# Dzh-16/FLASH-Viterbi

Hardware: AMD Instinct MI355X
Metric: trellis_cells_per_sec (higher is better)
Workload: dtype f32 scores (+f64 add per cell, rounded to f32 as the reference does)

## Files before the change

flash_viterbi_amd/csrc/fv_context.hip:

```cpp
#include "fv_internal.h"
#include "flashvit_testing.h"

namespace {

template <typename F>
void parallel_rows(int rows, F &&fn)
{
    unsigned hw = std::thread::hardware_concurrency();
    int nt = (int)std::min<unsigned>(hw ? hw : 4, 16);
    if (rows < 256) nt = 1;
    if (nt <= 1) { fn(0, rows); return; }
    std::vector<std::thread> th;
    int per = (rows + nt - 1) / nt;
    for (int t = 0; t < nt; ++t) {
        int a = t * per, b = std::min(rows, a + per);
        if (a >= b) break;
        th.emplace_back([=, &fn] { fn(a, b); });
    }
    for (auto &x : th) x.join();
}

}

namespace fvi {

size_t device_bytes(const fv_ctx *c)
{
    size_t sum = 0;
    c->each_buffer([&](const auto &b) { sum += b.bytes(); });
    return sum;
}

inline size_t pack_head(int nscores) { return 2 * FV_NCOUNTERS + (size_t)std::max(4, round_up(nscores, 4)); }

static size_t pack_ints(const fv_ctx *ctx, int T, int nscores) { return pack_head(nscores) + (size_t)T * std::max(1, ctx->nranks) + (size_t)T; }

int grant(fv_ctx *ctx, const Wants &w, bool check)
{
    if (check) {
        unsigned long long grow = 0, released = 0;
        for (const Wants::Want &x : w.list)
            if (x.n > x.have) { grow += (unsigned long long)x.n * x.elem; released += (unsigned long long)x.have * x.elem; }
        if (grow) {
            size_t free_b = 0, total_b = 0;
            FV_HIP(hipMemGetInfo(&free_b, &total_b));
            if (grow > (unsigned long long)free_b + released) {
                ctx->detail = w.what + ": " + std::to_string(grow) + " bytes needed (" + w.dominant + "), " +
                              std::to_string((unsigned long long)free_b + released) + " bytes of device memory free";
                return FV_ERR_NOMEM;
            }
        }
    }
    for (const Wants::Want &x : w.list) FV_HIP(x.ensure(x.buf, x.n));
    return 0;
}

int ensure_workspace(fv_ctx *ctx, int T, size_t rows_needed, int nscores, Wants w)
{
    const size_t want_rows = rows_needed * 2 * (size_t)ctx->nrows;
    const size_t want_pack = pack_ints(ctx, T, nscores);
    const bool rows_grow = want_rows > ctx->d_rows.n;
    w.add(ctx->d_ob, (size_t)T); w.add(ctx->d_ans, (size_t)T); w.add(ctx->d_bp, (size_t)T * ctx->K);
    w.add(ctx->d_rows, want_rows); w.add(ctx->d_pack, want_pack);
    if (nscores > 1 && w.what.empty()) { w.what = "batch workspace"; w.dominant = "arg rows " + std::to_string(4ull * T * ctx->K); }
    if (int rc = grant(ctx, w, nscores > 1)) return rc;
    if (rows_grow) FV_HIP(hipMemsetAsync(ctx->d_rows.p, 0, want_rows * sizeof(float), ctx->stream));
    FV_HIP(ctx->d_score.ensure((size_t)std::max(4, nscores)));
    FV_HIP(ctx->d_counters.ensure(FV_NCOUNTERS));
    if (ctx->comm || ctx->group) FV_HIP(ctx->d_gather.ensure((size_t)T * ctx->nranks));
    if (want_pack > ctx->h_pin_n) {
        if (ctx->h_pin) { (void)hipHostFree(ctx->h_pin); ctx->h_pin = nullptr; ctx->h_pin_n = 0; }
        FV_HIP(hipHostMalloc(reinterpret_cast<void **>(&ctx->h_pin), want_pack * sizeof(int), hipHostMallocDefault));
        ctx->h_pin_n = want_pack;
    }
    return 0;
}

int ensure_flat_workspace(fv_ctx *ctx, int T, size_t passes, long long arg_rows, int chain_len)
{
    Wants w;
    const size_t want_rows = passes * 2 * (size_t)ctx->nrows;
    const bool rows_grow = want_rows > ctx->d_rows.n;
    w.add(ctx->d_rows, want_rows); w.add(ctx->d_snap, (size_t)T); w.add(ctx->d_flat_bp, (size_t)std::max(arg_rows, 1ll) * ctx->K);
    w.add(ctx->d_chain, (size_t)std::max(chain_len, 1)); w.add(ctx->d_flat, std::max(passes, (size_t)1));
    w.what = "flat generations workspace"; w.dominant = "private arg rows " + std::to_string(4ull * (unsigned long long)arg_rows * ctx->K);
    if (int rc = grant(ctx, w, true)) return rc;
    if (rows_grow) FV_HIP(hipMemsetAsync(ctx->d_rows.p, 0, want_rows * sizeof(float), ctx->stream));
    return 0;
}

__global__ void pack_result(const unsigned long long *counters, const float *score, int nscore, size_t head, const int *ans,
                            size_t nans, int *out)
{
    const size_t tid = (size_t)blockIdx.x * blockDim.x + threadIdx.x, nthr = (size_t)gridDim.x * blockDim.x;
    if (tid < 2 * FV_NCOUNTERS) out[tid] = reinterpret_cast<const int *>(counters)[tid];
    for (size_t i = tid; i < (size_t)nscore; i += nthr) out[2 * FV_NCOUNTERS + i] = __float_as_int(score[i]);
    for (size_t i = tid; i < nans; i += nthr) out[head + i] = ans[i];
}

__global__ void clear_outputs(unsigned long long *counters, int *ans, int T)
{
    const int tid = blockIdx.x * blockDim.x + threadIdx.x;
    if (tid < FV_NCOUNTERS) counters[tid] = 0ull;
    for (int i = tid; i < T; i += gridDim.x * blockDim.x) ans[i] = 0;
}

int emission_view(fv_ctx *ctx, const int *&ob, long long T)
{
    if (ob) {
        ctx->view.lb32 = ctx->LB32T.p; ctx->view.lb64 = ctx->LB64T.p; ctx->view.nsym = ctx->M;
        ctx->view.logs_nonpositive = ctx->logs_nonpositive;
        return 0;
    }
    if (ctx->emis_rows == 0) { ctx->detail = "ob == NULL: no emission scores are staged (fv_set_emissions)"; return FV_ERR_ARG; }
    if (T < 1 || T > ctx->emis_rows) {
        ctx->detail = "ob == NULL: " + std::to_string(T) + " times asked for, " + std::to_string(ctx->emis_rows) + " rows of emission scores staged";
        return FV_ERR_ARG;
    }
    try {
        for (size_t j = ctx->h_iota.size(); j < (size_t)T; ++j) ctx->h_iota.push_back((int)j);
    } catch (const std::bad_alloc &) { return FV_ERR_NOMEM; }
    ob = ctx->h_iota.data();
    ctx->view.lb32 = ctx->E32.p; ctx->view.lb64 = ctx->E64.p; ctx->view.nsym = (int)ctx->emis_rows;
    ctx->view.logs_nonpositive = ctx->logs_nonpositive && !ctx->emis_positive;
    return 0;
}

int begin_decode(fv_ctx *ctx, const int *ob, int T)
{
    ctx->h_ob.assign(ob, ob + T);
    int *stage = ctx->h_pin + (ctx->h_pin_n - (size_t)T);
    std::memcpy(stage, ob, (size_t)T * sizeof(int));
    FV_HIP(hipMemcpyAsync(ctx->d_ob.p, stage, (size_t)T * sizeof(int), hipMemcpyHostToDevice, ctx->stream));
    hipLaunchKernelGGL(clear_outputs, dim3(16), dim3(256), 0, ctx->stream, ctx->d_counters.p, ctx->d_ans.p, T);
    FV_HIP(hipGetLastError());
    return 0;
}

int batch_lengths(fv_ctx *ctx, const char *who, const int *&ob, const long long *offsets, int nseq, int n_split, int mode,
                  const int *path_out, std::vector<int> &lengths)
{
    if (!offsets || !path_out || nseq < 1 || n_split < 1) return FV_ERR_ARG;
    if (mode != FV_MODE_REFERENCE && mode != FV_MODE_SINGLE_PASS) return FV_ERR_ARG;
    const std::string w = who;
    if (offsets[0] != 0) { ctx->detail = w + ": offsets[0] must be 0"; return FV_ERR_ARG; }
    lengths.resize((size_t)nseq);
    for (int s = 0; s < nseq; ++s) {
        const long long len = offsets[s + 1] - offsets[s];
        if (len < 0) { ctx->detail = w + ": offsets decrease at sequence " + std::to_string(s); return FV_ERR_ARG; }
        if (len < 2) { ctx->detail = w + ": sequence " + std::to_string(s) + " has fewer than 2 observations"; return FV_ERR_ARG; }
        if (offsets[s + 1] > 0x7fffffffLL) { ctx->detail = w + ": more than 2^31 - 1 observations in all (at sequence " + std::to_string(s) + ")"; return FV_ERR_ARG; }
        lengths[(size_t)s] = (int)len;
    }
    if (int rc = emission_view(ctx, ob, offsets[nseq])) return rc;
    return ctx->K == 0 ? FV_ERR_STATE : 0;
}

int batch_symbols(fv_ctx *ctx, const char *who, const int *ob, const long long *offsets, int nseq)
{
    for (int s = 0; s < nseq; ++s)
        for (long long j = offsets[s]; j < offsets[s + 1]; ++j)
            if (ob[j] < 0 || ob[j] >= ctx->view.nsym) {
                ctx->detail = std::string(who) + ": sequence " + std::to_string(s) + " holds a symbol outside [0, M) at position " + std::to_string(j - offsets[s]);
                return FV_ERR_ARG;
            }
    return 0;
}

int batch_plan(fv_ctx *ctx, const char *who, const std::vector<int> &lengths, int n_split, int mode, fv::Plan &plan)
{
    int bad = -1;
    const int rc = fv::build_forest(lengths.data(), (int)lengths.size(), n_split, mode, plan, &bad);
    if (rc)
        ctx->detail = std::string(who) + ": sequence " + std::to_string(bad) + " of length " + std::to_string(lengths[(size_t)std::max(bad, 0)]) +
                      " has no plan for n_split = " + std::to_string(n_split) + " (T == 2 * n_split with n_split > 2)";
    return rc;
}

std::vector<std::vector<fv::Pass>> deal_passes(const fv_ctx *ctx, const fv::Plan &plan, size_t *most)
{
    std::vector<std::vector<fv::Pass>> gens(plan.generations());
    for (const fv::Pass &p : plan.passes)
        if (p.owner < 0 || p.owner % ctx->nranks == ctx->rank) gens[p.generation].push_back(p);
    if (most) {
        *most = 1;
        for (const auto &g : gens) *most = std::max(*most, g.size());
    }
    return gens;
}

static int read_stats(fv_ctx *ctx, const unsigned long long *counters, clk::time_point t0, size_t nprof)
{
    fv_stats &st = ctx->stats;
    st.decode_ms = ms_since(t0);
    float ms = 0.f;
    FV_HIP(hipEventElapsedTime(&ms, ctx->ev_start, ctx->ev_stop)); st.gpu_ms = ms;
    FV_HIP(hipEventElapsedTime(&ms, ctx->ev_start, ctx->ev_top)); st.top_pass_ms = ms;
    FV_HIP(hipEventElapsedTime(&ms, ctx->ev_s0, ctx->ev_s1)); st.top_steps_ms = ms;
    st.step_kernel_ms = 0;
    for (size_t i = 0; i + 1 < nprof; i += 2) {
        FV_HIP(hipEventElapsedTime(&ms, ctx->prof_events[i], ctx->prof_events[i + 1]));
        st.step_kernel_ms += ms;
    }
    st.refine_near = (long long)counters[0];
    st.refine_rescan = (long long)counters[1];
    st.beam_exact_sets = (long long)counters[2];
    st.beam_dup_cols = (long long)counters[3];
    st.beam_dup_steps = (long long)counters[4];
    st.beam_ties = (long long)counters[6];
    st.beam_cand_selects = (long long)counters[7];
    st.refine_saturated = (long long)counters[8];
    st.beam_spec_steps = (long long)counters[9];
    st.beam_reach_events = (long long)counters[10];
    st.beam_list_short = (long long)counters[11];
    st.beam_list_long = (long long)counters[12];
    st.beam_list_entries = (long long)counters[13];
    st.beam_chain_cuts = (long long)counters[14];
    if (counters[fvk::FLAT_COUNTER]) {
        st.flat_first_miss = (int)(counters[fvk::FLAT_COUNTER] >> 32);
        st.flat_missed = (int)(counters[fvk::FLAT_COUNTER] & 0xffffffffull);
    }
    if (counters[5]) { ctx->detail = "heap replay: producer/consumer hand-shake timed out"; return FV_ERR_DEVICE; }
    st.device_bytes = (long long)fvi::device_bytes(ctx);
    st.ranks = ctx->nranks;
    return 0;
}

int finish_decode(fv_ctx *ctx, const fv::Plan &plan, const long long *offsets, int nseq, int *path_out, float *score_out,
                  int *status_out, clk::time_point t0, size_t nprof, bool beam)
{
    const int T = (int)offsets[nseq];
    const bool gathered = (ctx->comm || ctx->group) && !plan.seg_L.empty();
    if (gathered)
        if (int rc = gather_answers(ctx, T)) return rc;
    FV_HIP(hipEventRecord(ctx->ev_stop, ctx->stream));
    const size_t nans = gathered ? (size_t)T * ctx->nranks : (size_t)T, head = pack_head(nseq), total = head + nans;
    hipLaunchKernelGGL(pack_result, dim3(64), dim3(256), 0, ctx->stream, ctx->d_counters.p, ctx->d_score.p, nseq, head,
                       gathered ? ctx->d_gather.p : ctx->d_ans.p, nans, ctx->d_pack.p);
    FV_HIP(hipGetLastError());
    FV_HIP(hipMemcpyAsync(ctx->h_pin, ctx->d_pack.p, total * sizeof(int), hipMemcpyDeviceToHost, ctx->stream));
    FV_HIP(hipStreamSynchronize(ctx->stream));
    for (hipGraphExec_t ge : ctx->graphs) (void)hipGraphExecDestroy(ge);
    ctx->graphs.clear();
    unsigned long long counters[FV_NCOUNTERS];
    std::memcpy(counters, ctx->h_pin, sizeof counters);
    if (gathered) {
        const std::vector<int> host(ctx->h_pin + head, ctx->h_pin + head + nans);
        merge_gathered(plan, host, T, ctx->nranks, path_out);
    } else {
        std::memcpy(path_out, ctx->h_pin + head, nans * sizeof(int));
    }
    if (score_out) std::memcpy(score_out, ctx->h_pin + 2 * FV_NCOUNTERS, (size_t)nseq * sizeof(float));
    if (int rc = read_stats(ctx, counters, t0, nprof)) return rc;
    int worst = FV_OK, warn = FV_OK;
    for (int s = 0; s < nseq; ++s) {
        bool neg = false;
        for (long long j = offsets[s]; j < offsets[s + 1]; ++j) neg |= path_out[j] < 0;
        const int st = !neg ? FV_OK : beam ? FV_WARN_BEAM_MISS : FV_ERR_NO_PRED;
        if (status_out) status_out[s] = st;
        worst = std::min(worst, st);
        warn = std::max(warn, st);
    }
    return worst < 0 ? worst : warn;
}

int drained(fv_ctx *ctx, int rc)
{
    if (rc >= 0) return rc;
    hipStreamCaptureStatus cs = hipStreamCaptureStatusNone;
    if (hipStreamIsCapturing(ctx->stream, &cs) == hipSuccess && cs != hipStreamCaptureStatusNone) {
        hipGraph_t g = nullptr;
        (void)hipStreamEndCapture(ctx->stream, &g);
        if (g) (void)hipGraphDestroy(g);
    }
    (void)hipStreamSynchronize(ctx->stream);
    for (hipStream_t a : ctx->aux) if (a) (void)hipStreamSynchronize(a);
    for (hipGraphExec_t ge : ctx->graphs) (void)hipGraphExecDestroy(ge);
    ctx->graphs.clear();
    (void)hipGetLastError();
    return rc;
}

}



extern "C" int fv_create(fv_ctx **out, int device)
{
    if (!out) return FV_ERR_ARG;
    *out = nullptr;
    int ndev = 0;
    if (hipGetDeviceCount(&ndev) != hipSuccess || device < 0 || device >= ndev) return FV_ERR_DEVICE;
    fv_ctx *ctx = new (std::nothrow) fv_ctx();
    if (!ctx) return FV_ERR_NOMEM;
    ctx->device = device;
    auto fail = [&](int rc) { fv_destroy(ctx); return rc; };
    if (hipSetDevice(device) != hipSuccess) return fail(FV_ERR_DEVICE);
    if (hipStreamCreateWithFlags(&ctx->stream, hipStreamNonBlocking) != hipSuccess) return fail(FV_ERR_DEVICE);
    for (int q = 0; q < fv_ctx::BEAM_AUX; ++q)
        if (hipStreamCreateWithFlags(&ctx->aux[q], hipStreamNonBlocking) != hipSuccess ||
            hipEventCreateWithFlags(&ctx->ev_join[q], hipEventDisableTiming) != hipSuccess) return fail(FV_ERR_DEVICE);
    if (hipEventCreateWithFlags(&ctx->ev_fork, hipEventDisableTiming) != hipSuccess) return fail(FV_ERR_DEVICE);
    {
        int cus = 0;
        if (hipDeviceGetAttribute(&cus, hipDeviceAttributeMultiprocessorCount, ctx->device) == hipSuccess && cus > 0) ctx->num_cus = cus;
    }
    if (hipEventCreate(&ctx->ev_start) != hipSuccess || hipEventCreate(&ctx->ev_stop) != hipSuccess ||
        hipEventCreate(&ctx->ev_top) != hipSuccess || hipEventCreate(&ctx->ev_s0) != hipSuccess ||
        hipEventCreate(&ctx->ev_s1) != hipSuccess)
        return fail(FV_ERR_DEVICE);
    int rc = 0;
    if ((rc = fvi::full_setup(ctx)) || (rc = fvi::beam_setup(ctx))) return fail(rc);
    *out = ctx;
    return FV_OK;
}

extern "C" void fv_destroy(fv_ctx *ctx)
{
    if (!ctx) return;
    if (ctx->group) {
        fv_group *g = ctx->group;
        if (ctx->group_rank != 0) return;
        for (fv_ctx *m : g->members) m->group = nullptr;
        for (size_t r = g->members.size(); r-- > 1;) fv_destroy(g->members[r]);
        for (hipEvent_t e : g->ans_ready) if (e) (void)hipEventDestroy(e);
        delete g;
    }
    (void)hipSetDevice(ctx->device);
    if (ctx->stream) (void)hipStreamSynchronize(ctx->stream);
    if (ctx->comm) ncclCommDestroy(ctx->comm);
    if (ctx->h_pin) { (void)hipHostFree(ctx->h_pin); ctx->h_pin = nullptr; ctx->h_pin_n = 0; }
    for (hipEvent_t e : ctx->prof_events) (void)hipEventDestroy(e);
    if (ctx->ev_start) (void)hipEventDestroy(ctx->ev_start);
    if (ctx->ev_stop) (void)hipEventDestroy(ctx->ev_stop);
    if (ctx->ev_top) (void)hipEventDestroy(ctx->ev_top);
    if (ctx->ev_s0) (void)hipEventDestroy(ctx->ev_s0);
    if (ctx->ev_s1) (void)hipEventDestroy(ctx->ev_s1);
    if (ctx->ev_fork) (void)hipEventDestroy(ctx->ev_fork);
    for (int q = 0; q < fv_ctx::BEAM_AUX; ++q) {
        if (ctx->ev_join[q]) (void)hipEventDestroy(ctx->ev_join[q]);
        if (ctx->aux[q]) (void)hipStreamDestroy(ctx->aux[q]);
    }
    if (ctx->stream) (void)hipStreamDestroy(ctx->stream);
    delete ctx;
}

namespace fvi {

static void log_emissions(const float *B, const float *Pi, int K, int M, HostTables &h, bool &ok_range, bool &any_big)
{
    h.b64.assign((size_t)M * K, 0.0); h.pi64.assign(K, 0.0);
    h.b32.assign((size_t)M * K, 0.0f);
    for (int i = 0; i < K; ++i) {
        for (int o = 0; o < M; ++o) {
            const float x = B[(size_t)i * M + o];
            if (!(x >= 0.0f) || std::isinf(x)) ok_range = false;
            if (x > 1.0f) any_big = true;
            const double l = std::log((double)x);
            h.b64[(size_t)o * K + i] = l; h.b32[(size_t)o * K + i] = (float)l;
        }
        const float x = Pi[i];
        if (!(x >= 0.0f) || std::isinf(x)) ok_range = false;
        if (x > 1.0f) any_big = true;
        h.pi64[i] = std::log((double)x);
    }
}

int build_host_tables(const float *A, const float *B, const float *Pi, int K, int M, HostTables &h, std::string &detail)
{
    h.K = K; h.M = M;
    const int nrows = h.nrows = round_up(K, fvk::ROW_ALIGN);
    const int ntiles = h.ntiles = (K + fvk::TILE_W - 1) / fvk::TILE_W;
    const bool full_ok = h.full_ok = fvk::step_lds_bytes<1>(nrows) <= 160 * 1024;
    h.u16_ok = fvk::u16_lds_bytes<1, 8>(nrows) <= 160 * 1024 && K <= 65536;

    const size_t tab = h.tab = (size_t)ntiles * nrows * fvk::TILE_W;
    std::vector<double> &h64 = h.h64;
    std::vector<float> &h32 = h.h32;
    std::vector<unsigned short> &h16 = h.h16;
    try {
        h64.assign(tab, -HUGE_VAL);
        if (full_ok) { h32.assign(tab, -HUGE_VALF); h16.assign(tab, 0xFC00u ); }
    } catch (...) { return FV_ERR_NOMEM; }
    std::vector<double> dmax_row(K, 0.0);
    bool ok_range = true;
    std::vector<char> bad(K, 0), big(K, 0);
    parallel_rows(K, [&](int a, int b) {
        for (int k = a; k < b; ++k) {
            const float *src = A + (size_t)k * K;
            for (int i = 0; i < K; ++i) {
                const float x = src[i];
                if (!(x >= 0.0f) || std::isinf(x)) bad[k] = 1;
                if (x > 1.0f) big[k] = 1;
                const double l = std::log((double)x);
// ... 411 lines not shown
                      "FV_EMIS_LOG_F32, _F64, _F16 or _BF16";
        return FV_ERR_ARG;
    }
    auto t0 = clk::now();
    hipPointerAttribute_t at{};
    bool on_device = false;
    if (hipPointerGetAttributes(&at, scores) == hipSuccess) on_device = at.type == hipMemoryTypeDevice;
    else (void)hipGetLastError();
    for (int r = 0; r < n; ++r) {
        fv_ctx *m = fvi::group_member(ctx, r);
        const bool in_place = on_device && n == 1 && at.device == m->device;
        const int rc = fvi::drained(m, fvi::stage_emissions_on(m, scores, dtype, T, ld, in_place));
        if (rc) {
            if (m != ctx) ctx->detail = m->detail;
            for (int q = 0; q < n; ++q) fvi::group_member(ctx, q)->emis_rows = 0;
            ctx->stats.device_bytes = (long long)fvi::device_bytes(ctx);
            return rc;
        }
    }
    ctx->stats.set_emissions_ms = ms_since(t0);
    ctx->stats.emission_rows = T;
    ctx->stats.device_bytes = (long long)fvi::device_bytes(ctx);
    return FV_OK;
}

extern "C" int fv_set_emission_map(fv_ctx *ctx, const int *pdf_of_state, int P)
{
    if (!ctx) return FV_ERR_ARG;
    if (ctx->K == 0) { ctx->detail = "fv_set_emission_map: no model (the map holds one entry per state of the model)"; return FV_ERR_STATE; }
    if (!pdf_of_state && P != 0) { ctx->detail = "fv_set_emission_map: pdf_of_state == NULL clears the map and takes P == 0"; return FV_ERR_ARG; }
    if (pdf_of_state) {
        if (P < 1) { ctx->detail = "fv_set_emission_map: P >= 1 score classes with a map"; return FV_ERR_ARG; }
        hipPointerAttribute_t at{};
        if (hipPointerGetAttributes(&at, pdf_of_state) != hipSuccess) (void)hipGetLastError();
        else if (at.type == hipMemoryTypeDevice) {
            ctx->detail = "fv_set_emission_map: pdf_of_state is a device pointer; the map is read on the host";
            return FV_ERR_ARG;
        }
        for (int i = 0; i < ctx->K; ++i)
            if (pdf_of_state[i] < 0 || pdf_of_state[i] >= P) {
                ctx->detail = "fv_set_emission_map: pdf_of_state[" + std::to_string(i) + "] = " + std::to_string(pdf_of_state[i]) +
                              " (state " + std::to_string(i) + ") lies outside [0, P = " + std::to_string(P) + ")";
                return FV_ERR_ARG;
            }
    }
    const int n = fvi::group_size(ctx);
    auto unset = [&] {
        for (int r = 0; r < n; ++r) {
            fv_ctx *m = fvi::group_member(ctx, r);
            m->emis_rows = 0; m->emis_positive = false; m->emis_P = 0;
        }
        ctx->stats.emission_rows = 0;
        ctx->stats.set_emissions_ms = 0.0;
    };
    unset();
    int rc = FV_OK;
    for (int r = 0; r < n && rc == FV_OK; ++r) {
        fv_ctx *m = fvi::group_member(ctx, r);
        rc = [&]() -> int {
            fv_ctx *ctx = m;
            FV_HIP(hipSetDevice(ctx->device));
            if (!pdf_of_state) { ctx->EMap.release(); return FV_OK; }
            FV_HIP(ctx->EMap.ensure((size_t)ctx->K));
            FV_HIP(hipMemcpy(ctx->EMap.p, pdf_of_state, (size_t)ctx->K * sizeof(int), hipMemcpyHostToDevice));
            ctx->emis_P = P;
            return FV_OK;
        }();
        if (rc && m != ctx) ctx->detail = m->detail;
    }
    if (rc) unset();
    ctx->stats.device_bytes = (long long)fvi::device_bytes(ctx);
    return rc;
}

extern "C" int fv_clear_emissions(fv_ctx *ctx)
{
    if (!ctx) return FV_ERR_ARG;
    const int n = fvi::group_size(ctx);
    for (int r = 0; r < n; ++r) {
        fv_ctx *m = fvi::group_member(ctx, r);
        (void)hipSetDevice(m->device);
        m->emis_rows = 0; m->emis_positive = false;
        m->E32.release(); m->E64.release();
    }
    ctx->stats.emission_rows = 0;
    ctx->stats.device_bytes = (long long)fvi::device_bytes(ctx);
    return FV_OK;
}

extern "C" int fv_test_device_alloc(fv_ctx *ctx, size_t bytes, const void *host_src, void **out)
{
    if (!ctx || !out || bytes == 0) return FV_ERR_ARG;
    *out = nullptr;
    FV_HIP(hipSetDevice(ctx->device));
    void *p = nullptr;
    FV_HIP(hipMalloc(&p, bytes));
    if (host_src) {
        hipError_t e = hipMemcpy(p, host_src, bytes, hipMemcpyHostToDevice);
        if (e != hipSuccess) { (void)hipFree(p); FV_HIP(e); }
    }
    *out = p;
    return FV_OK;
}

extern "C" int fv_test_device_free(fv_ctx *ctx, void *p)
{
    if (!ctx) return FV_ERR_ARG;
    FV_HIP(hipSetDevice(ctx->device));
    if (p) FV_HIP(hipFree(p));
    return FV_OK;
}

extern "C" int fv_test_stage_emissions_ms(fv_ctx *ctx, const void *dev_scores, int dtype, int T, long long ld, int reps, float *ms_out)
{
    if (!ctx || !ms_out || !dev_scores || T < 1 || reps < 1 || ctx->K == 0 || ld < (ctx->emis_P ? ctx->emis_P : ctx->K) ||
        ld > (1ll << 59) / T || !fvi::emis_dtype_ok(dtype) || ctx->group)
        return FV_ERR_ARG;
    hipPointerAttribute_t at{};
    if (hipPointerGetAttributes(&at, dev_scores) != hipSuccess) { (void)hipGetLastError(); return FV_ERR_ARG; }
    if (at.type != hipMemoryTypeDevice || at.device != ctx->device) return FV_ERR_ARG;
    FV_HIP(hipSetDevice(ctx->device));
    ctx->emis_rows = 0; ctx->emis_positive = false;
    ctx->stats.emission_rows = 0;
    const size_t cells = (size_t)T * (size_t)ctx->K;
    FV_HIP(ctx->E32.ensure(cells));
    FV_HIP(ctx->E64.ensure(cells));
    FV_HIP(ctx->d_emflags.ensure(2));
    FV_HIP(hipMemsetAsync(ctx->d_emflags.p, 0, sizeof(unsigned long long), ctx->stream));
    FV_HIP(hipMemsetAsync(ctx->d_emflags.p + 1, 0xFF, sizeof(unsigned long long), ctx->stream));
    hipEvent_t e0 = nullptr, e1 = nullptr;
    struct Ev { hipEvent_t &a, &b; ~Ev() { if (a) (void)hipEventDestroy(a); if (b) (void)hipEventDestroy(b); } } ev{ e0, e1 };
    FV_HIP(hipEventCreate(&e0));
    FV_HIP(hipEventCreate(&e1));
    if (int rc = fvi::launch_stage_emissions(ctx, dev_scores, dtype, ld, T, ctx->EMap.p, ctx->emis_P)) return fvi::drained(ctx, rc);
    FV_HIP(hipEventRecord(e0, ctx->stream));
    for (int r = 0; r < reps; ++r)
        if (int rc = fvi::launch_stage_emissions(ctx, dev_scores, dtype, ld, T, ctx->EMap.p, ctx->emis_P)) return fvi::drained(ctx, rc);
    FV_HIP(hipEventRecord(e1, ctx->stream));
    FV_HIP(hipStreamSynchronize(ctx->stream));
    float ms = 0.0f;
    FV_HIP(hipEventElapsedTime(&ms, e0, e1));
    *ms_out = ms / (float)reps;
    ctx->stats.device_bytes = (long long)fvi::device_bytes(ctx);
    return FV_OK;
}

extern "C" int fv_test_flat_poison(fv_ctx *ctx, int t)
{
    if (!ctx || t < -1) return FV_ERR_ARG;
    ctx->flat_poison = t;
    return FV_OK;
}

extern "C" int fv_set_option(fv_ctx *ctx, int key, long long value)
{
    if (!ctx) return FV_ERR_ARG;
    if (ctx->group && ctx->group_rank == 0) {
        for (int r = fvi::group_size(ctx) - 1; r >= 1; --r) {
            const int rc = fv_set_option(fvi::group_member(ctx, r), key, value);
            if (rc) return rc;
        }
    }
    switch (key) {
    case FV_OPT_KERNEL:
        if ((value < FV_KERNEL_AUTO || value > FV_KERNEL_U16_REFINE) && value != FV_KERNEL_CSR_F64) return FV_ERR_ARG;
        ctx->opt_kernel = (int)value; return FV_OK;
    case FV_OPT_MAX_BATCH:
        if (value < 1 || value > fvk::MAX_BATCH) return FV_ERR_ARG;
        ctx->opt_max_batch = (int)value; return FV_OK;
    case FV_OPT_PROFILE:
        ctx->opt_profile = value ? 1 : 0; return FV_OK;
    case FV_OPT_FLAT_GENERATIONS:
        if (value < 0 || value > 2) return FV_ERR_ARG;
        ctx->opt_flat = (int)value; return FV_OK;
    case FV_OPT_ROW_CODES:
        if (value < 0 || value > 4) return FV_ERR_ARG;
        ctx->opt_row_codes = (int)value; return FV_OK;
    case FV_OPT_SEL_MARGIN:
        if (value < 0 || value > 100000) return FV_ERR_ARG;
        ctx->opt_sel_margin = (float)value * 1e-3f; return FV_OK;
    case FV_OPT_SPARSE_BEAM:
        if (value != 0 && value != 1) return FV_ERR_ARG;
        ctx->opt_sparse_beam = (int)value; return FV_OK;
    case FV_OPT_DEBUG:
#ifndef FV_TIMING_BUILD
        if (value & FV_DEBUG_TIMING_ONLY) { ctx->detail = "FV_OPT_DEBUG: result-changing timing switches need the timing build"; return FV_ERR_ARG; }
#endif
        if (value < 0 || value >= (1ll << 32) || (value & ((1ll << 27) | (1ll << 30)))) return FV_ERR_ARG;
        ctx->opt_csr_mem = (int)((value >> 31) & 1);
        ctx->opt_debug = (int)(value & 0x3fffffff); return FV_OK;
    default: return FV_ERR_ARG;
    }
}

extern "C" long long fv_checkpoint_memory_bytes(int K, int T, int step)
{
    if (step <= 0) step = (int)std::floor(std::sqrt(1.0 * T));
    const long long nck = (T + step - 1) / step;
    const long long last = T - (nck - 1) * step;
    const long long tsub = nck > 1 && step + 1 > last ? step + 1 : last;
    return 4LL * K + 4LL * K * nck + 4LL * K + 4LL * (T / step + 1) + 8LL * K * tsub;
}

extern "C" int fv_last_stats(const fv_ctx *ctx, fv_stats *out)
{
    if (!ctx || !out) return FV_ERR_ARG;
    *out = ctx->stats;
    return FV_OK;
}

extern "C" const char *fv_last_error_detail(const fv_ctx *ctx) { return ctx ? ctx->detail.c_str() : ""; }

extern "C" const char *fv_strerror(int rc)
{
    switch (rc) {
    case FV_OK: return "ok";
    case FV_WARN_BEAM_MISS: return "beam miss: path holds -1 entries, as the reference prints";
    case FV_ERR_ARG: return "bad argument";
    case FV_ERR_NOMEM: return "out of memory";
    case FV_ERR_NO_PRED: return "decoded entry has no finite predecessor";
    case FV_ERR_DEVICE: return "HIP error";
    case FV_ERR_STATE: return "call out of order (no model / no communicator)";
    case FV_ERR_UNSUPPORTED: return "size or option not supported by this build";
    case FV_ERR_COMM: return "RCCL error";
    default: return "unknown flashvit error";
    }
}

extern "C" long long fv_reference_memory_bytes(int K, int T, int n_split, int beam_width)
{
    const long long N = n_split;
    const long long pool = ((40 + 48 + 8 * N + 12 + 7) / 8) * 8;
    long long mem = 0, tmp;
    const bool nway = N > 2 && T >= 2 * N;
    if (beam_width <= 0) {
        if (nway) mem = 4 * (N - 1) + 2LL * K * 4 + 2 * (N - 1) * (long long)K * 4;
        tmp = N * (2LL * K * 4 + 2LL * K * 4);
    } else {
        if (nway) mem = 4 * (N - 1) + 2 * (N - 1) * (long long)(beam_width + 1) * 12;
        tmp = N * (2LL * (beam_width + 1) * 12);
    }
    if (tmp > mem) mem = tmp;
    return mem + pool + 8;
}
```

flash_viterbi_amd/csrc/fv_full.hip:

```cpp
#include "fv_internal.h"
#include "fv_kernels.hip.inc"
#include "flashvit_testing.h"

namespace {

int pick_kernel(const fv_ctx *ctx)
{
    if (ctx->opt_kernel == FV_KERNEL_F64_STREAM) return FV_KERNEL_F64_STREAM;
    if (!ctx->view.logs_nonpositive) return FV_KERNEL_F64_STREAM;
    if (ctx->opt_kernel == FV_KERNEL_F16_REFINE || ctx->opt_kernel == FV_KERNEL_F32_REFINE ||
        ctx->opt_kernel == FV_KERNEL_Q16_REFINE || ctx->opt_kernel == FV_KERNEL_U16_REFINE)
        return ctx->opt_kernel;
    if (ctx->opt_kernel == FV_KERNEL_SPARSE_Q16) return ctx->SPdata.p ? FV_KERNEL_SPARSE_Q16 : FV_KERNEL_U16_REFINE;
    return (ctx->SPdata.p && ctx->density <= 0.35) ? FV_KERNEL_SPARSE_Q16 : FV_KERNEL_U16_REFINE;
}

constexpr int U_UP = 16, U_DB32 = 4, U_DB64 = 2, U_DB16 = 2;

constexpr int nb_slot(int NB) { return NB == 1 ? 0 : NB == 2 ? 1 : NB == 4 ? 2 : 3; }
template <typename TA> constexpr int tab_slot()
{
    return std::is_same<TA, double>::value ? 0 : std::is_same<TA, float>::value ? 1 : std::is_same<TA, fvk::half_t>::value ? 2 : 3;
}
template <typename TA, int NB, bool DB> constexpr unsigned long long step_variant()
// ... 202 lines not shown
    if (ctx->test_record) ctx->test_variants |= u16_variant<NB, DB, NWV>() | ((b.codes & 1) ? FV_TV_ROW_CODES : 0ull);
    hipLaunchKernelGGL((fvk::trellis_step_u16<NB, U, DB, NWV>), dim3(a.tiles_per_xcd * 8), dim3(NWV * 64), lds, ctx->lstream ? ctx->lstream : ctx->stream, b);
    FV_HIP(hipGetLastError());
    return 0;
}

template <int NB>
int launch_u16_nb(fv_ctx *ctx, const fvk::TaskSlot *slots, int nb, int reverse)
{
    fvk::StepArgs<NB> a;
    a.LA = ctx->LAQ16.p; a.window = ctx->windowq; a.qscale = ctx->qscale; a.vanilla = 0;
    a.LA64 = ctx->LA64.p; a.counters = ctx->d_counters.p;
    a.K = ctx->K; a.reverse = (ctx->opt_debug & 2) ? 0 : reverse; a.debug = ctx->opt_debug;
    a.nrows = ctx->nrows;
    a.ntiles = (ctx->K + fvk::TILE_W - 1) / fvk::TILE_W;
    a.tiles_per_xcd = (a.ntiles + 7) / 8;
    a.nb = nb;
    a.row_lo = 0; a.srows = ctx->nrows; a.merge = 0;
    a.codes = ctx->launch_codes;
    const fvk::CodeSlot *cs = static_cast<const fvk::CodeSlot *>(ctx->launch_code_slots);
    for (int t = 0; t < NB; ++t) { a.t[t] = slots[t < nb ? t : 0]; a.c[t] = cs[t < nb ? t : 0]; }
    const int nq = ctx->nrows / 32;
    if (ctx->opt_debug & 8192) {
        if (a.ntiles <= ctx->num_cus && (nq + 15) / 16 <= 8 && !(ctx->opt_debug & 4)) return launch_u16_variant<NB, 8, false, 16>(ctx, a);
        return launch_u16_variant<NB, U_DB16, true, 16>(ctx, a);
    }
    if (a.ntiles <= ctx->num_cus && (nq + 7) / 8 <= 16 && !(ctx->opt_debug & 4) && !ctx->forked_batches) return launch_u16_variant<NB, 16, false, 8>(ctx, a);
    return launch_u16_variant<NB, U_DB16, true, 8>(ctx, a);
}

int launch_u16(fv_ctx *ctx, const fvk::TaskSlot *slots, int nb, int reverse)
{
    if (nb <= 1) return launch_u16_nb<1>(ctx, slots, nb, reverse);
    if (nb <= 2) return launch_u16_nb<2>(ctx, slots, nb, reverse);
    if (nb <= 4) return launch_u16_nb<4>(ctx, slots, nb, reverse);
    return launch_u16_nb<8>(ctx, slots, nb, reverse);
}

constexpr int ROW_CODES_AUTO_MIN_K = 2048;
constexpr int ROW_CODES_AUTO_FAMILIES = 2;

int coded_row_index(const fv_ctx *ctx, const float *row)
{
    if (!row || row < ctx->d_rows.p || row >= ctx->d_rows.p + ctx->d_rows.n) return -1;
    const size_t off = (size_t)(row - ctx->d_rows.p);
    if (off % (size_t)ctx->nrows) return -1;
    const size_t r = off / (size_t)ctx->nrows;
    return r < ctx->row_coded.size() ? (int)r : -1;
}

int ensure_row_codes(fv_ctx *ctx, size_t pairs)
{
    if (!ctx->row_codes) { ctx->row_coded.clear(); return 0; }
    const size_t rows = pairs * 2, want = rows * (size_t)ctx->nrows;
    if (want > ctx->d_rcodes.n || want / fvk::TILE_W > ctx->d_rtmax.n) {
        if (ctx->d_rcodes.ensure(want) != hipSuccess || ctx->d_rtmax.ensure(want / fvk::TILE_W) != hipSuccess) {
            (void)hipGetLastError();
            ctx->d_rcodes.release(); ctx->d_rtmax.release();
            ctx->row_codes = 0; ctx->row_coded.clear();
            return 0;
        }
        FV_HIP(hipMemsetAsync(ctx->d_rcodes.p, 0xff, ctx->d_rcodes.bytes(), ctx->stream));
        FV_HIP(hipMemsetAsync(ctx->d_rtmax.p, 0xff, ctx->d_rtmax.bytes(), ctx->stream));
    }
    ctx->row_coded.assign(ctx->d_rcodes.n / (size_t)ctx->nrows, 0);
    return 0;
}

bool init_rows_coded(fv_ctx *ctx, int base, int n)
{
    if (!ctx->row_codes || ctx->csr || (size_t)(base + n) * 2 > ctx->row_coded.size()) return false;
    for (int q = 0; q < n; ++q) ctx->row_coded[(size_t)(base + q) * 2] = 1;
    return true;
}

int launch_step_kernel(fv_ctx *ctx, int kernel, const fvk::TaskSlot *slots, int nb, int reverse)
{
    fvk::CodeSlot cs[fvk::MAX_BATCH];
    const bool packed = kernel == FV_KERNEL_U16_REFINE && (nb <= 1 || !ctx->full_ok || (ctx->opt_debug & 16384) || ctx->forked_batches);
    bool all_in = packed && ctx->row_codes != 0, all_out = all_in;
    int rout[fvk::MAX_BATCH];
    for (int q = 0; q < nb; ++q) {
        const int rin = coded_row_index(ctx, slots[q].t1_in);
        rout[q] = coded_row_index(ctx, slots[q].t1_out);
        const size_t ntp = (size_t)ctx->nrows / fvk::TILE_W;
        cs[q].c_in = rin >= 0 ? ctx->d_rcodes.p + (size_t)rin * ctx->nrows : nullptr;
        cs[q].tmax_in = rin >= 0 ? ctx->d_rtmax.p + (size_t)rin * ntp : nullptr;
        cs[q].c_out = rout[q] >= 0 ? ctx->d_rcodes.p + (size_t)rout[q] * ctx->nrows : nullptr;
        cs[q].tmax_out = rout[q] >= 0 ? ctx->d_rtmax.p + (size_t)rout[q] * ntp : nullptr;
        all_in = all_in && rin >= 0 && ctx->row_coded[(size_t)rin];
        all_out = all_out && rout[q] >= 0;
    }
    const int family = nb <= 1 ? 1 : 2;
    const bool produce = all_out && (nb > 1 || (ctx->row_codes & 1));
    ctx->launch_codes = ((all_in && (ctx->row_codes & family)) ? 1 : 0) | (produce ? 2 : 0);
    ctx->launch_code_slots = cs;
    for (int q = 0; q < nb; ++q)
        if (rout[q] >= 0) ctx->row_coded[(size_t)rout[q]] = produce ? 1 : 0;
    switch (kernel) {
    case FV_KERNEL_U16_REFINE:
        if (nb <= 1 || !ctx->full_ok || (ctx->opt_debug & 16384) || ctx->forked_batches) return launch_u16(ctx, slots, nb, reverse);
        return launch_step<fvk::q16_t>(ctx, slots, nb, reverse);
    case FV_KERNEL_SPARSE_Q16: return launch_sparse(ctx, slots, nb);
    case FV_KERNEL_SPARSE_CSR: return launch_csr(ctx, slots, nb);
    case FV_KERNEL_CSR_F64: return launch_csr_f64(ctx, slots, nb);
    case FV_KERNEL_F64_STREAM: return launch_step<double>(ctx, slots, nb, reverse);
    case FV_KERNEL_F32_REFINE: return launch_step<float>(ctx, slots, nb, reverse);
    case FV_KERNEL_Q16_REFINE: return launch_step<fvk::q16_t>(ctx, slots, nb, reverse);
    default: return launch_step<fvk::half_t>(ctx, slots, nb, reverse);
    }
}

template <typename K>
int set_big_lds(fv_ctx *ctx, K kernel)
{
    FV_HIP(hipFuncSetAttribute(reinterpret_cast<const void *>(kernel), hipFuncAttributeMaxDynamicSharedMemorySize, 160 * 1024));
    return 0;
}

template <typename TA, int NB>
int allow_big_lds(fv_ctx *ctx)
{
    int rc = 0;
    if constexpr (std::is_same<TA, double>::value) {
        rc = set_big_lds(ctx, &fvk::trellis_step<TA, NB, U_DB64, true>);
    } else {
        constexpr int U = std::is_same<TA, float>::value ? U_DB32 : U_DB16;
        rc = set_big_lds(ctx, &fvk::trellis_step<TA, NB, U, true>);
        if constexpr (NB <= 2) { if (!rc) rc = set_big_lds(ctx, &fvk::trellis_step<TA, NB, U_UP, false>); }
    }
    return rc;
}

int max_batch_for(int nrows, bool u16_only)
{
    if (u16_only) {
        if (fvk::u16_lds_bytes<8, 8>(nrows) <= 160 * 1024) return 8;
        if (fvk::u16_lds_bytes<4, 8>(nrows) <= 160 * 1024) return 4;
        if (fvk::u16_lds_bytes<2, 8>(nrows) <= 160 * 1024) return 2;
        return 1;
    }
    int nb = fvk::MAX_BATCH;
    while (nb > 1) {
        size_t need = nb == 8 ? fvk::step_lds_bytes<8>(nrows) : nb == 4 ? fvk::step_lds_bytes<4>(nrows)
                                                                        : fvk::step_lds_bytes<2>(nrows);
        if (need <= 160 * 1024) break;
        nb >>= 1;
    }
    return nb;
}

struct ProfRange { size_t first, count; };

int prof_event(fv_ctx *ctx, size_t idx, hipEvent_t *out)
{
    while (ctx->prof_events.size() <= idx) {
        hipEvent_t e;
        FV_HIP(hipEventCreate(&e));
        ctx->prof_events.push_back(e);
    }
    *out = ctx->prof_events[idx];
    return 0;
}

enum { BATCH_NONE = 0, BATCH_SERIAL = 1, BATCH_FORK = 2 };
int run_generation_full(fv_ctx *ctx, std::vector<fv::Pass> &passes, int kernel, size_t &nprof, int batch = BATCH_NONE)
{
    const int K = ctx->K;
    const int np = (int)passes.size();
    if (np == 0) return 0;
    std::stable_sort(passes.begin(), passes.end(),
                     [](const fv::Pass &a, const fv::Pass &b) { return a.R - a.L > b.R - b.L; });
    for (int base = 0; base < np; base += fvk::PASS_CHUNK) {
        fvk::PassChunk ch;
        ch.n = std::min(fvk::PASS_CHUNK, np - base);
        for (int q = 0; q < ch.n; ++q) {
            const fv::Pass &p = passes[base + q];
            ch.p[q] = fvk::PassDesc{ p.L, p.R, p.from_pi ? 1 : 0, p.whole ? 1 : 0, (long long)(base + q) * 2 * ctx->nrows };
        }
        if (ctx->csr)
            hipLaunchKernelGGL(fvk::init_rows_csr, dim3((K + 255) / 256, ch.n), dim3(256), 0, ctx->stream, ch, ctx->CRptr.p,
                               ctx->CRcol.p, ctx->CRlog.p, ctx->view.lb64, ctx->LPi64.p, ctx->d_ob.p, ctx->d_ans.p, ctx->d_rows.p, K);
        else {
            const bool coded = init_rows_coded(ctx, base, ch.n);
            hipLaunchKernelGGL(fvk::init_rows, dim3((K + 255) / 256, ch.n), dim3(256), 0, ctx->stream, ch,
                               ctx->LA64.p, ctx->nrows, ctx->view.lb64, ctx->LPi64.p, ctx->d_ob.p, ctx->d_ans.p,
                               ctx->d_rows.p, K, coded ? ctx->d_rcodes.p : nullptr, coded ? ctx->d_rtmax.p : nullptr, -1.0f / ctx->qscale);
        }
        FV_HIP(hipGetLastError());
    }
    const int maxlen = passes[0].R - passes[0].L;
    const bool slabbed = (kernel == FV_KERNEL_F64_STREAM || kernel == FV_KERNEL_Q16_REFINE) && !ctx->full_ok;
    int cap = std::max(1, std::min(ctx->opt_max_batch, slabbed ? 4 : max_batch_for(ctx->nrows, !ctx->full_ok)));
    if (kernel == FV_KERNEL_SPARSE_CSR || kernel == FV_KERNEL_CSR_F64) cap = ctx->opt_max_batch;
    const bool whole_gen = passes[0].whole;
    constexpr int FORK_STREAMS = 3, FORK_CAP = 4;
    const bool two = ((kernel == FV_KERNEL_U16_REFINE && ctx->u16_ok) || ((kernel == FV_KERNEL_SPARSE_Q16 || kernel == FV_KERNEL_SPARSE_CSR || kernel == FV_KERNEL_CSR_F64) && maxlen >= 64)) &&
                     !(ctx->opt_debug & 262144) && (!whole_gen || batch == BATCH_FORK) && np > FORK_CAP &&
                     !ctx->opt_profile && !(ctx->opt_debug & 64);
    const int nbatches = (np + FORK_CAP - 1) / FORK_CAP;
    const int nstreams = two ? std::min(FORK_STREAMS, nbatches) : 1;
    auto fork = [&]() -> int {
        FV_HIP(hipEventRecord(ctx->ev_fork, ctx->stream));
        for (int q = 1; q < nstreams; ++q) FV_HIP(hipStreamWaitEvent(ctx->aux[q - 1], ctx->ev_fork, 0));
        return 0;
    };
    if (two) {
        cap = std::min(cap, FORK_CAP);
        if (!ctx->fork_active) {
            hipError_t qe;
            while ((qe = hipStreamQuery(ctx->stream)) == hipErrorNotReady) std::this_thread::yield();
            FV_HIP(qe);
        }
        ctx->fork_active = true;
        { int rc = fork(); if (rc) return rc; }
    }
    ctx->forked_batches = two;
    struct Unfork { fv_ctx *c; ~Unfork() { c->forked_batches = false; c->lstream = nullptr; } } unfork{ ctx };
    auto join = [&]() -> int {
        for (int q = 1; q < nstreams; ++q) {
            FV_HIP(hipEventRecord(ctx->ev_join[q - 1], ctx->aux[q - 1]));
            FV_HIP(hipStreamWaitEvent(ctx->stream, ctx->ev_join[q - 1], 0));
        }
        return 0;
    };
    const bool col_last = !(ctx->opt_debug & 8);
    const bool use_graph = (ctx->opt_debug & 64) && !ctx->opt_profile;
    if (use_graph) FV_HIP(hipStreamBeginCapture(ctx->stream, hipStreamCaptureModeThreadLocal));
    if (whole_gen && !use_graph) FV_HIP(hipEventRecord(ctx->ev_s0, ctx->stream));
    int active = np;
    for (int s = 1; s <= maxlen; ++s) {
        while (active > 0 && passes[active - 1].R - passes[active - 1].L < s) --active;
        int full = active;
        if (col_last) while (full > 0 && passes[full - 1].R - passes[full - 1].L == s && !passes[full - 1].whole) --full;
        auto row = [&](int q, int parity) { return ctx->d_rows.p + (size_t)q * 2 * ctx->nrows + (size_t)parity * ctx->nrows; };
        for (int base = 0; base < full; base += cap) {
            const int nb = std::min(cap, full - base);
            fvk::TaskSlot slots[fvk::MAX_BATCH];
            for (int q = 0; q < nb; ++q) {
                const fv::Pass &p = passes[base + q];
                slots[q].t1_in = row(base + q, (s - 1) & 1);
                slots[q].t1_out = row(base + q, s & 1);
                slots[q].tmp_row = ctx->view.lb32 + (size_t)ctx->h_ob[p.L + s] * K;
                slots[q].tmp64_row = ctx->view.lb64 + (size_t)ctx->h_ob[p.L + s] * K;
                slots[q].bp_out = ctx->d_bp.p + (size_t)(p.L + s) * K;
            }
            hipEvent_t e0 = nullptr, e1 = nullptr;
            if (ctx->opt_profile) {
                int rc = prof_event(ctx, nprof, &e0); if (rc) return rc;
                rc = prof_event(ctx, nprof + 1, &e1); if (rc) return rc;
                nprof += 2;
                FV_HIP(hipEventRecord(e0, ctx->stream));
            }
            const int other = two ? (base / cap) % nstreams : 0;
            ctx->lstream = other ? ctx->aux[other - 1] : ctx->stream;
            int rc = launch_step_kernel(ctx, kernel, slots, nb, s & 1);
            ctx->lstream = nullptr;
            if (rc) return rc;
            if (ctx->opt_profile) FV_HIP(hipEventRecord(e1, ctx->stream));
            ctx->stats.step_launches += 1;
            ctx->stats.task_steps += nb;
        }
        for (int sid = 0; sid < nstreams; ++sid) {
            fvk::ColArgs c;
            c.LA64 = ctx->LA64.p; c.ans = ctx->d_ans.p; c.K = K; c.nrows = ctx->nrows; c.n = 0;
            hipStream_t cst = sid ? ctx->aux[sid - 1] : ctx->stream;
            auto flush = [&]() -> int {
                if (c.n == 0) return 0;
                if (ctx->csr) {
                    fvk::CsrColArgs cc;
                    cc.ck = ctx->CSk.p; cc.c64 = ctx->CS64.p; cc.tile_off = ctx->CSoff.p; cc.tile_nwb = ctx->CSnwb.p;
                    cc.ans = ctx->d_ans.p; cc.K = K; cc.n = c.n;
                    std::copy(c.p, c.p + c.n, cc.p);
                    hipLaunchKernelGGL(fvk::last_column_csr, dim3(c.n), dim3(256), 0, cst, cc);
                } else
                hipLaunchKernelGGL(fvk::last_column, dim3(c.n), dim3(256), 0, cst, c);
                FV_HIP(hipGetLastError());
                ctx->stats.column_steps += c.n;
                c.n = 0;
                return 0;
            };
            for (int q = full; q < active; ++q) {
                const int owner = (two && s > 1) ? (q / cap) % nstreams : 0;
                if (owner != sid) continue;
                const fv::Pass &p = passes[q];
                c.p[c.n++] = fvk::ColJob{ row(q, (s - 1) & 1), ctx->view.lb32 + (size_t)ctx->h_ob[p.R] * K, ctx->d_bp.p + (size_t)p.R * K, p.R };
                if (c.n == fvk::COL_CHUNK) { int rc = flush(); if (rc) return rc; }
            }
            int rc = flush();
            if (rc) return rc;
        }
    }
    if (use_graph) {
        hipGraph_t g = nullptr;
        FV_HIP(hipStreamEndCapture(ctx->stream, &g));
        hipGraphExec_t ge = nullptr;
        FV_HIP(hipGraphInstantiate(&ge, g, nullptr, nullptr, 0));
        if (whole_gen) FV_HIP(hipEventRecord(ctx->ev_s0, ctx->stream));
        FV_HIP(hipGraphLaunch(ge, ctx->stream));
        ctx->graphs.push_back(ge);
        (void)hipGraphDestroy(g);
    }
    if (whole_gen && !two) FV_HIP(hipEventRecord(ctx->ev_s1, ctx->stream));
    if (two) { int rc = join(); if (rc) return rc; }
    if (whole_gen && two) FV_HIP(hipEventRecord(ctx->ev_s1, ctx->stream));
    if (batch) {
        fvk::ArgmaxArgs a;
        a.rows = ctx->d_rows.p; a.ans = ctx->d_ans.p; a.score = ctx->d_score.p; a.K = K; a.nrows = ctx->nrows; a.n = 0;
        auto flush = [&]() -> int {
            if (a.n == 0) return 0;
            hipLaunchKernelGGL(fvk::final_argmax_batch, dim3(a.n), dim3(1024), 0, ctx->stream, a);
            FV_HIP(hipGetLastError());
            a.n = 0;
            return 0;
        };
        for (int q = 0; q < np; ++q) {
            if (!passes[q].whole) continue;
            const int len = passes[q].R - passes[q].L;
            a.j[a.n++] = fvk::ArgmaxJob{ q * 2 + (len & 1), passes[q].R, passes[q].seq };
            if (a.n == fvk::ARGMAX_CHUNK) { int rc = flush(); if (rc) return rc; }
        }
        int rc = flush();
        if (rc) return rc;
    }
    for (int q = 0; q < np && !batch; ++q) {
        if (!passes[q].whole) continue;
        const int len = passes[q].R - passes[q].L;
        const float *last = ctx->d_rows.p + (size_t)q * 2 * ctx->nrows + (size_t)(len & 1) * ctx->nrows;
        hipLaunchKernelGGL(fvk::final_argmax, dim3(1), dim3(1024), 0, ctx->stream, last, K,
                           ctx->d_ans.p + passes[q].R, ctx->d_score.p);
        FV_HIP(hipGetLastError());
    }
    for (int base = 0; base < np; base += fvk::PASS_CHUNK) {
        fvk::PassChunk ch;
        ch.n = std::min(fvk::PASS_CHUNK, np - base);
        for (int q = 0; q < ch.n; ++q) {
            const fv::Pass &p = passes[base + q];
            ch.p[q] = fvk::PassDesc{ p.L, p.R, p.from_pi ? 1 : 0, p.whole ? 1 : 0, 0 };
        }
        hipLaunchKernelGGL(fvk::backtrack, dim3(ch.n), dim3(64), 0, ctx->stream, ch, ctx->d_bp.p, K, ctx->d_ans.p);
        FV_HIP(hipGetLastError());
    }
    return 0;
}

constexpr int FLAT_STREAMS = 3, FLAT_CAP = 4;
constexpr int FLAT_AUTO_MIN_K = 512, FLAT_AUTO_MAX_T = 1024;

void flat_shape(const fv_ctx *ctx, int kernel, int maxlen, int nlong, int &cap, int &nstreams)
{
    const bool slabbed = (kernel == FV_KERNEL_F64_STREAM || kernel == FV_KERNEL_Q16_REFINE) && !ctx->full_ok;
    cap = std::max(1, std::min(ctx->opt_max_batch, slabbed ? 4 : max_batch_for(ctx->nrows, !ctx->full_ok)));
    if (kernel == FV_KERNEL_SPARSE_CSR || kernel == FV_KERNEL_CSR_F64) cap = ctx->opt_max_batch;
    const bool walk = kernel == FV_KERNEL_SPARSE_Q16 || kernel == FV_KERNEL_SPARSE_CSR || kernel == FV_KERNEL_CSR_F64;
    const bool fork = ((kernel == FV_KERNEL_U16_REFINE && ctx->u16_ok) || (walk && maxlen >= 64)) && !(ctx->opt_debug & 262144) && nlong > FLAT_CAP;
    nstreams = fork ? FLAT_STREAMS : 1;
    if (fork) cap = std::min(cap, FLAT_CAP);
}

int run_flat_full(fv_ctx *ctx, int kernel, int T)
{
    const fv::FlatPlan &fp = ctx->flat_plan;
    const int K = ctx->K, np = (int)fp.passes.size(), nstreams = fp.nstreams;
    const bool two = nstreams > 1;
    hipStream_t streams[FLAT_STREAMS] = { ctx->stream, ctx->aux[0], ctx->aux[1] };
    auto row = [&](int i, int parity) { return ctx->d_rows.p + (size_t)i * 2 * ctx->nrows + (size_t)parity * ctx->nrows; };
    auto arg_rows = [&](const fv::FlatPass &p) { return p.arg_row < 0 ? ctx->d_bp.p + (size_t)(p.L + 1) * K : ctx->d_flat_bp.p + (size_t)p.arg_row * K; };
    if (ctx->flat_uploaded != ctx->d_flat.p) {
        std::vector<fvk::FlatDesc> table((size_t)np);
        for (int i = 0; i < np; ++i) table[(size_t)i] = fvk::FlatDesc{ fp.passes[i].L, fp.passes[i].R, fp.passes[i].generation, fp.passes[i].chain, fp.passes[i].arg_row };
        FV_HIP(hipMemcpyAsync(ctx->d_flat.p, table.data(), (size_t)np * sizeof(fvk::FlatDesc), hipMemcpyHostToDevice, ctx->stream));
        FV_HIP(hipStreamSynchronize(ctx->stream));
        ctx->flat_uploaded = ctx->d_flat.p;
    }
    hipLaunchKernelGGL(fvk::flat_snapshot, dim3((T + 255) / 256), dim3(256), 0, ctx->stream, ctx->d_ans.p, ctx->d_snap.p, T, ctx->flat_poison, K);
    FV_HIP(hipGetLastError());
    for (int base = 0; base < np; base += fvk::PASS_CHUNK) {
        fvk::PassChunk ch;
        ch.n = std::min(fvk::PASS_CHUNK, np - base);
        for (int q = 0; q < ch.n; ++q) ch.p[q] = fvk::PassDesc{ fp.passes[base + q].L, fp.passes[base + q].R, 0, 0, (long long)(base + q) * 2 * ctx->nrows };
        if (ctx->csr)
            hipLaunchKernelGGL(fvk::init_rows_csr, dim3((K + 255) / 256, ch.n), dim3(256), 0, ctx->stream, ch, ctx->CRptr.p,
                               ctx->CRcol.p, ctx->CRlog.p, ctx->view.lb64, ctx->LPi64.p, ctx->d_ob.p, ctx->d_snap.p, ctx->d_rows.p, K);
        else {
// ... 166 lines not shown
        hipLaunchKernelGGL(fvk::init_rows_csr, dim3((ctx->K + 255) / 256, ch.n), dim3(256), 0, ctx->stream, ch, ctx->CRptr.p,
                           ctx->CRcol.p, ctx->CRlog.p, ctx->view.lb64, ctx->LPi64.p, ctx->d_ob.p, ctx->d_ans.p, rows, ctx->K);
    else
    hipLaunchKernelGGL(fvk::init_rows, dim3((ctx->K + 255) / 256, ch.n), dim3(256), 0, ctx->stream, ch,
                       ctx->LA64.p, ctx->nrows, ctx->view.lb64, ctx->LPi64.p, ctx->d_ob.p, ctx->d_ans.p, rows, ctx->K,
                       static_cast<unsigned short *>(nullptr), static_cast<float *>(nullptr), 0.0f);
    FV_HIP(hipGetLastError());
    return 0;
}

template <typename TIN>
static void launch_stage_as(fv_ctx *ctx, const void *src, long long ld, int T, const int *map, dim3 grid)
{
    if (map)
        hipLaunchKernelGGL((fvk::stage_emissions<TIN, true>), grid, dim3(fvk::EMIS_BLOCK), 0, ctx->stream,
                           static_cast<const TIN *>(src), ld, T, ctx->K, map, ctx->E32.p, ctx->E64.p, ctx->d_emflags.p);
    else
        hipLaunchKernelGGL((fvk::stage_emissions<TIN, false>), grid, dim3(fvk::EMIS_BLOCK), 0, ctx->stream,
                           static_cast<const TIN *>(src), ld, T, ctx->K, map, ctx->E32.p, ctx->E64.p, ctx->d_emflags.p);
}

int launch_stage_emissions(fv_ctx *ctx, const void *src, int dtype, long long ld, int T, const int *map, int P)
{
    const int K = ctx->K;
    const int gx = std::min((K + fvk::EMIS_BLOCK - 1) / fvk::EMIS_BLOCK, 2048), gy = std::max(1, std::min(T, 2048 / gx));
    if (P <= 0) map = nullptr;
    switch (dtype) {
    case FV_EMIS_LOG_F64: launch_stage_as<double>(ctx, src, ld, T, map, dim3(gx, gy)); break;
    case FV_EMIS_LOG_F32: launch_stage_as<float>(ctx, src, ld, T, map, dim3(gx, gy)); break;
    case FV_EMIS_LOG_F16: launch_stage_as<_Float16>(ctx, src, ld, T, map, dim3(gx, gy)); break;
    case FV_EMIS_LOG_BF16: launch_stage_as<fvk::bf16_bits>(ctx, src, ld, T, map, dim3(gx, gy)); break;
    default: ctx->detail = "fv_set_emissions: unknown dtype"; return FV_ERR_ARG;
    }
    FV_HIP(hipGetLastError());
    return 0;
}

}

namespace {
int decode_full_impl(fv_ctx *ctx, const int *ob, int T, int n_split, int mode, int *path_out, float *score_out);
int decode_checkpoint_impl(fv_ctx *ctx, const int *ob, int T, int step, int *path_out, float *score_out);
}

extern "C" int fv_decode_full(fv_ctx *ctx, const int *ob, int T, int n_split, int mode, int *path_out, float *score_out)
{
    if (!ctx) return FV_ERR_ARG;
    if (ctx->group && ctx->group_rank == 0 && !ctx->vanilla) {
        if (!path_out || T < 2) return FV_ERR_ARG;
        return fvi::group_run(ctx, T, path_out, score_out, [&](fv_ctx *m, int *path, float *score) {
            return fvi::drained(m, decode_full_impl(m, ob, T, n_split, mode, path, score));
        });
    }
    return fvi::drained(ctx, decode_full_impl(ctx, ob, T, n_split, mode, path_out, score_out));
}

namespace {
int decode_full_batch_impl(fv_ctx *ctx, const int *ob, const long long *offsets, int nseq, int n_split, int mode, int *path_out,
                           float *score_out, int *status_out);
}

extern "C" int fv_decode_full_batch(fv_ctx *ctx, const int *ob, const long long *offsets, int nseq, int n_split, int mode,
                                    int *path_out, float *score_out, int *status_out)
{
    if (!ctx) return FV_ERR_ARG;
    if (ctx->group || ctx->comm || ctx->nranks > 1) {
        ctx->detail = "fv_decode_full_batch: one device, no communicator and no partition (sequences are not dealt to ranks)";
        return FV_ERR_UNSUPPORTED;
    }
    return fvi::drained(ctx, decode_full_batch_impl(ctx, ob, offsets, nseq, n_split, mode, path_out, score_out, status_out));
}

namespace {
int prepare_full(fv_ctx *ctx, const int *ob, int T, size_t rows_needed, int &kernel, int nscores = 1, bool auto_codes = false)
{
    ctx->row_codes = 0;
    ctx->row_coded.clear();
    if (ctx->csr) {
        const bool f64 = ctx->opt_kernel == FV_KERNEL_CSR_F64;
        if (!f64 && ctx->opt_kernel != FV_KERNEL_AUTO && ctx->opt_kernel != FV_KERNEL_SPARSE_Q16) {
            ctx->detail = "a model set by fv_set_model_sparse has no dense table: FV_KERNEL_AUTO or FV_KERNEL_SPARSE_Q16 (the filter walk), or FV_KERNEL_CSR_F64";
            return FV_ERR_UNSUPPORTED;
        }
        if (!f64 && !ctx->view.logs_nonpositive) {
            ctx->detail = "fv_set_model_sparse: the walk over the stored entries is a filter kernel and needs every model entry in [0,1] "
                          "(and every staged emission score <= 0); FV_KERNEL_CSR_F64 decodes such input";
            return FV_ERR_UNSUPPORTED;
        }
        for (int j = 0; j < T; ++j) if (ob[j] < 0 || ob[j] >= ctx->view.nsym) return FV_ERR_ARG;
        FV_HIP(hipSetDevice(ctx->device));
        kernel = f64 ? FV_KERNEL_CSR_F64 : FV_KERNEL_SPARSE_CSR;
        return fvi::ensure_workspace(ctx, T, rows_needed, nscores);
    }
    if (ctx->opt_kernel == FV_KERNEL_CSR_F64) {
        ctx->detail = "FV_KERNEL_CSR_F64 walks the stored entries of a model set by fv_set_model_sparse: this model was set by fv_set_model";
        return FV_ERR_UNSUPPORTED;
    }
    const bool wide = !ctx->full_ok;
    const bool big = wide && ctx->u16_ok && ctx->view.logs_nonpositive && !ctx->vanilla &&
                     (ctx->opt_kernel == FV_KERNEL_AUTO || ctx->opt_kernel == FV_KERNEL_U16_REFINE);
    const bool wide_q16 = wide && !big && ctx->view.logs_nonpositive && !ctx->vanilla &&
                          (ctx->opt_kernel == FV_KERNEL_AUTO || ctx->opt_kernel == FV_KERNEL_Q16_REFINE);
    if (wide && !big && !wide_q16 && !(ctx->opt_kernel == FV_KERNEL_AUTO || ctx->opt_kernel == FV_KERNEL_F64_STREAM)) {
        ctx->detail = "full-state decode of K > ~40100: FV_KERNEL_AUTO, FV_KERNEL_U16_REFINE (K <= 65536), FV_KERNEL_Q16_REFINE (both: model entries in [0,1]) or FV_KERNEL_F64_STREAM";
        return FV_ERR_UNSUPPORTED;
    }
    for (int j = 0; j < T; ++j) if (ob[j] < 0 || ob[j] >= ctx->view.nsym) return FV_ERR_ARG;
    if (ctx->opt_kernel >= FV_KERNEL_F32_REFINE && !ctx->view.logs_nonpositive) {
        ctx->detail = "the filter+refine kernels need every model entry in [0,1] (and every staged emission score <= 0)";
        return FV_ERR_UNSUPPORTED;
    }
    FV_HIP(hipSetDevice(ctx->device));
    kernel = big ? FV_KERNEL_U16_REFINE : wide_q16 ? FV_KERNEL_Q16_REFINE : wide ? FV_KERNEL_F64_STREAM : pick_kernel(ctx);
    if ((big || wide_q16) && !ctx->laq16_ready) {
        const int ntiles = (ctx->K + fvk::TILE_W - 1) / fvk::TILE_W;
        const size_t tab = (size_t)ntiles * ctx->nrows * fvk::TILE_W;
        FV_HIP(ctx->LAQ16.ensure(tab));
        FV_HIP(ctx->d_qaux.ensure(3));
        FV_HIP(hipMemsetAsync(ctx->d_qaux.p, 0, 2 * sizeof(unsigned long long), ctx->stream));
        hipLaunchKernelGGL(fvk::q16_tile_range, dim3(2048), dim3(256), 0, ctx->stream, ctx->LA64.p, tab, ctx->d_qaux.p);
        hipLaunchKernelGGL(fvk::q16_tile_codes, dim3(4096), dim3(256), 0, ctx->stream, ctx->LA64.p, ctx->LAQ16.p, ctx->K, ctx->nrows,
                           ntiles, ctx->d_qaux.p, ctx->d_qaux.p + 1);
        FV_HIP(hipGetLastError());
        unsigned long long bits[2] = { 0, 0 };
        FV_HIP(hipMemcpyAsync(bits, ctx->d_qaux.p, sizeof bits, hipMemcpyDeviceToHost, ctx->stream));
        FV_HIP(hipStreamSynchronize(ctx->stream));
        double lmax, dqmax;
        std::memcpy(&lmax, &bits[0], 8); std::memcpy(&dqmax, &bits[1], 8);
        const float stepf = lmax > 0.0 ? (float)(lmax / 65534.0) : 1.0f;
        ctx->windowq = std::nextafter((float)(2.0 * dqmax), HUGE_VALF);
        ctx->qscale = -stepf;
        ctx->laq16_ready = true;
    }
    if (int rc = fvi::ensure_workspace(ctx, T, rows_needed, nscores)) return rc;
    if (kernel == FV_KERNEL_U16_REFINE && !ctx->vanilla) {
        const int o = ctx->opt_row_codes;
        ctx->row_codes = o == 2 ? 3 : o == 3 ? 1 : o == 4 ? 2 : (o == 1 && auto_codes && ctx->K >= ROW_CODES_AUTO_MIN_K) ? ROW_CODES_AUTO_FAMILIES : 0;
    }
    return ensure_row_codes(ctx, rows_needed);
}

void start_full_stats(fv_ctx *ctx, int kernel, int generations)
{
    long long table = (long long)((ctx->K + fvk::TILE_W - 1) / fvk::TILE_W) * ctx->nrows * fvk::TILE_W * (kernel == FV_KERNEL_F64_STREAM ? 8 : kernel == FV_KERNEL_F32_REFINE ? 4 : 2);
    if (kernel == FV_KERNEL_SPARSE_Q16) table = (long long)ctx->SPdata.bytes();
    if (kernel == FV_KERNEL_SPARSE_CSR) table = (long long)(ctx->CSk.bytes() + ctx->CSq.bytes());
    if (kernel == FV_KERNEL_CSR_F64) table = (long long)(ctx->CSk.bytes() + ctx->CS64.bytes());
    ctx->start_stats(kernel, generations, table, ctx->density);
}

int decode_full_impl(fv_ctx *ctx, const int *ob, int T, int n_split, int mode, int *path_out, float *score_out)
{
    if (!ctx || !path_out || T < 2 || n_split < 1) return FV_ERR_ARG;
    int rc = fvi::emission_view(ctx, ob, T);
    if (rc) return rc;
    if (ctx->K == 0) return FV_ERR_STATE;
    auto t0 = clk::now();
    fv::Plan plan;
    rc = fv::build_plan(T, n_split, mode, ctx->nranks, plan);
    if (rc) return rc;
    size_t most = 1;
    std::vector<std::vector<fv::Pass>> gens = fvi::deal_passes(ctx, plan, &most);
    int kernel = FV_KERNEL_AUTO;
    if ((rc = prepare_full(ctx, ob, T, most, kernel, 1, true))) return rc;
    start_full_stats(ctx, kernel, plan.generations());

    bool flat = ctx->opt_flat != 0 && mode == FV_MODE_REFERENCE && plan.generations() >= 2 && plan.generations() - 1 <= fvk::FLAT_MAX_GENS &&
                !ctx->group && !ctx->comm && ctx->nranks == 1 && !ctx->opt_profile && !ctx->vanilla && !(ctx->opt_debug & 64);
    if (flat) {
        int cap = 1, nstreams = 1, maxlen = 0, nlong = 0;
        for (const fv::Pass &p : plan.passes)
            if (!p.whole) { maxlen = std::max(maxlen, p.R - p.L); nlong += p.R - p.L > 1 ? 1 : 0; }
        flat_shape(ctx, kernel, maxlen, nlong, cap, nstreams);
        if (ctx->opt_flat == 1 && !(kernel == FV_KERNEL_U16_REFINE && nstreams > 1 && ctx->K >= FLAT_AUTO_MIN_K && T <= FLAT_AUTO_MAX_T && plan.generations() >= 3)) flat = false;
        if (flat) {
            const int key[4] = { T, n_split, cap, nstreams };
            if (std::memcmp(key, ctx->flat_key, sizeof key) != 0) {
                fv::build_flat(plan, cap, nstreams, ctx->flat_plan);
                std::memcpy(ctx->flat_key, key, sizeof key);
                ctx->flat_uploaded = nullptr;
            }
            const int wrc = fvi::ensure_flat_workspace(ctx, T, ctx->flat_plan.passes.size(), ctx->flat_plan.arg_rows, ctx->flat_plan.chain_len);
            if (wrc == FV_ERR_NOMEM) { flat = false; ctx->detail.clear(); }
            else if (wrc) return wrc;
            else if ((rc = ensure_row_codes(ctx, std::max(most, ctx->flat_plan.passes.size())))) return rc;
        }
    }

    if ((rc = fvi::begin_decode(ctx, ob, T))) return rc;
    FV_HIP(hipEventRecord(ctx->ev_start, ctx->stream));
    size_t nprof = 0;
    ctx->fork_active = false;
    for (size_t g = 0; g < gens.size() && !(flat && g == 1); ++g) {
        ctx->stats.passes += (int)gens[g].size();
        if ((rc = run_generation_full(ctx, gens[g], kernel, nprof))) return rc;
        if (g == 0) FV_HIP(hipEventRecord(ctx->ev_top, ctx->stream));
    }
    if (flat && (rc = run_flat_full(ctx, kernel, T))) return rc;
    ctx->close_stats((long long)ctx->K * ctx->K, ctx->K);
    const long long whole[2] = { 0, T };
    rc = fvi::finish_decode(ctx, plan, whole, 1, path_out, score_out, nullptr, t0, nprof, false);
    if (!flat || ctx->stats.flat_first_miss < 1 || rc == FV_ERR_DEVICE) return rc;
    ctx->fork_active = false;
    for (size_t g = (size_t)ctx->stats.flat_first_miss; g < gens.size(); ++g) {
        ctx->stats.passes += (int)gens[g].size();
        if ((rc = run_generation_full(ctx, gens[g], kernel, nprof))) return rc;
    }
    ctx->close_stats((long long)ctx->K * ctx->K, ctx->K);
    return fvi::finish_decode(ctx, plan, whole, 1, path_out, score_out, nullptr, t0, nprof, false);
}

int decode_full_batch_impl(fv_ctx *ctx, const int *ob, const long long *offsets, int nseq, int n_split, int mode, int *path_out,
                           float *score_out, int *status_out)
{
    const char *who = "fv_decode_full_batch";
    std::vector<int> lengths;
    int rc = fvi::batch_lengths(ctx, who, ob, offsets, nseq, n_split, mode, path_out, lengths);
    if (rc || (rc = fvi::batch_symbols(ctx, who, ob, offsets, nseq))) return rc;
    auto t0 = clk::now();
    const int sumT = (int)offsets[nseq];
    fv::Plan plan;
    if ((rc = fvi::batch_plan(ctx, who, lengths, n_split, mode, plan))) return rc;
    size_t most = 1;
    std::vector<std::vector<fv::Pass>> gens = fvi::deal_passes(ctx, plan, &most);
    int kernel = FV_KERNEL_AUTO;
    if ((rc = prepare_full(ctx, ob, sumT, most, kernel, std::max(nseq, 2)))) return rc;
    start_full_stats(ctx, kernel, plan.generations());

    if ((rc = fvi::begin_decode(ctx, ob, sumT))) return rc;
    FV_HIP(hipEventRecord(ctx->ev_start, ctx->stream));
    size_t nprof = 0;
    ctx->fork_active = false;
    const int gen0 = (ctx->opt_debug & (1 << 28)) ? BATCH_SERIAL : BATCH_FORK;
    for (size_t g = 0; g < gens.size(); ++g) {
        ctx->stats.passes += (int)gens[g].size();
        if ((rc = run_generation_full(ctx, gens[g], kernel, nprof, gen0))) return rc;
        if (g == 0) FV_HIP(hipEventRecord(ctx->ev_top, ctx->stream));
    }
    ctx->close_stats((long long)ctx->K * ctx->K, ctx->K);
    return fvi::finish_decode(ctx, plan, offsets, nseq, path_out, score_out, status_out, t0, nprof, false);
}

int test_forward_impl(fv_ctx *ctx, const int *ob, int T, const fv_test_pass *tp, int np, float *rows_out, int *bp_out,
                      unsigned long long *variants_out)
{
    if (!tp || np < 1 || !rows_out || !bp_out || T < 2) return FV_ERR_ARG;
    if (int rv = fvi::emission_view(ctx, ob, T)) return rv;
    if (ctx->K == 0) return FV_ERR_STATE;
    const int K = ctx->K;
    std::vector<fv::Pass> gen((size_t)np);
    std::vector<int> byL((size_t)np);
    for (int q = 0; q < np; ++q) {
        const fv_test_pass &p = tp[q];
        if (p.L < 0 || p.R <= p.L || p.R >= T) { ctx->detail = "fv_test_forward: a pass needs 0 <= L < R < T"; return FV_ERR_ARG; }
        if (p.L == 0 ? p.init_state >= 0 : (p.init_state < 0 || p.init_state >= K)) {
            ctx->detail = "fv_test_forward: init_state < 0 (Pi) at L = 0 only, a state in [0, K) at L > 0";
            return FV_ERR_ARG;
        }
        gen[(size_t)q] = fv::Pass{ p.L, p.R, p.L == 0, false, 0, -1 };
        byL[(size_t)q] = q;
    }
    std::sort(byL.begin(), byL.end(), [&](int a, int b) { return tp[a].L < tp[b].L; });
    for (int q = 1; q < np; ++q)
        if (tp[byL[q]].L <= tp[byL[q - 1]].R) { ctx->detail = "fv_test_forward: passes overlap"; return FV_ERR_ARG; }
    int kernel = FV_KERNEL_AUTO;
    int rc = prepare_full(ctx, ob, T, (size_t)np, kernel);
    if (rc) return rc;
    start_full_stats(ctx, kernel, 1);
    ctx->stats.passes = np;
    if ((rc = fvi::begin_decode(ctx, ob, T))) return rc;
    int *ans = ctx->h_pin;
    std::fill(ans, ans + T, 0);
    for (int q = 0; q < np; ++q) if (tp[q].L > 0) ans[tp[q].L - 1] = tp[q].init_state;
    FV_HIP(hipMemcpyAsync(ctx->d_ans.p, ans, (size_t)T * sizeof(int), hipMemcpyHostToDevice, ctx->stream));
    struct Restore {
        fv_ctx *c; int debug;
        ~Restore() { c->opt_debug = debug; c->test_record = false; }
    } restore{ ctx, ctx->opt_debug };
    ctx->opt_debug |= 8;
    ctx->test_record = true;
    ctx->test_variants = 0;
    ctx->fork_active = false;
    size_t nprof = 0;
    if ((rc = run_generation_full(ctx, gen, kernel, nprof))) return rc;
    for (int q = 0; q < np; ++q) {
        const fv::Pass &p = gen[(size_t)q];
        int c = 0;
        while (tp[c].L != p.L) ++c;
        const float *row = ctx->d_rows.p + (size_t)q * 2 * ctx->nrows + (size_t)((p.R - p.L) & 1) * ctx->nrows;
        FV_HIP(hipMemcpyAsync(rows_out + (size_t)c * K, row, (size_t)K * sizeof(float), hipMemcpyDeviceToHost, ctx->stream));
        FV_HIP(hipMemcpyAsync(bp_out + (size_t)(p.L + 1) * K, ctx->d_bp.p + (size_t)(p.L + 1) * K,
                              (size_t)(p.R - p.L) * K * sizeof(int), hipMemcpyDeviceToHost, ctx->stream));
    }
    FV_HIP(hipStreamSynchronize(ctx->stream));
    for (hipGraphExec_t ge : ctx->graphs) (void)hipGraphExecDestroy(ge);
    ctx->graphs.clear();
    if (variants_out) *variants_out = ctx->test_variants;
    return FV_OK;
}
}

extern "C" int fv_test_forward(fv_ctx *ctx, const int *ob, int T, const fv_test_pass *passes, int npasses,
                               float *rows_out, int *bp_out, unsigned long long *variants_out)
{
    if (!ctx) return FV_ERR_ARG;
    if (fvi::group_size(ctx) > 1) { ctx->detail = "fv_test_forward: one device per context"; return FV_ERR_ARG; }
    return fvi::drained(ctx, test_forward_impl(ctx, ob, T, passes, npasses, rows_out, bp_out, variants_out));
}

extern "C" int fv_decode_vanilla(fv_ctx *ctx, const int *ob, int T, int *path_out, float *score_out)
{
    if (!ctx) return FV_ERR_ARG;
    if (ctx->csr && ctx->opt_kernel != FV_KERNEL_CSR_F64) { ctx->detail = "fv_decode_vanilla: not available on a model set by fv_set_model_sparse (its kernel reads the dense table) unless FV_KERNEL_CSR_F64 is selected"; return FV_ERR_UNSUPPORTED; }
    const int keep_kernel = ctx->opt_kernel;
    if (!ctx->csr) ctx->opt_kernel = FV_KERNEL_F64_STREAM;
    ctx->vanilla = 1;
    int rc = fv_decode_full(ctx, ob, T, 1, FV_MODE_SINGLE_PASS, path_out, score_out);
    ctx->vanilla = 0;
    ctx->opt_kernel = keep_kernel;
    return rc;
}

extern "C" int fv_decode_checkpoint(fv_ctx *ctx, const int *ob, int T, int step, int *path_out, float *score_out)
{
    if (!ctx) return FV_ERR_ARG;
    if (ctx->csr) { ctx->detail = "fv_decode_checkpoint: not available on a model set by fv_set_model_sparse (its kernel reads the dense table)"; return FV_ERR_UNSUPPORTED; }
    return fvi::drained(ctx, decode_checkpoint_impl(ctx, ob, T, step, path_out, score_out));
}

namespace {
int decode_checkpoint_impl(fv_ctx *ctx, const int *ob, int T, int step, int *path_out, float *score_out)
{
    if (!ctx || !path_out || T < 2) return FV_ERR_ARG;
    if (int rv = fvi::emission_view(ctx, ob, T)) return rv;
    if (ctx->K == 0) return FV_ERR_STATE;
    for (int j = 0; j < T; ++j) if (ob[j] < 0 || ob[j] >= ctx->view.nsym) return FV_ERR_ARG;
    if (step <= 0) step = (int)std::floor(std::sqrt(1.0 * T));
    auto t0 = clk::now();
    FV_HIP(hipSetDevice(ctx->device));
    const int K = ctx->K, nrows = ctx->nrows;
    const int nck = (T + step - 1) / step;
    fv::Plan plan;
    int rc = fv::build_plan(T, 1, FV_MODE_SINGLE_PASS, 1, plan);
    if (rc) return rc;
    if ((rc = fvi::ensure_workspace(ctx, T, (size_t)nck + 1))) return rc;
    if (ctx->d_ckpt.n < (size_t)nck * nrows) {
        FV_HIP(ctx->d_ckpt.ensure((size_t)nck * nrows));
        FV_HIP(hipMemsetAsync(ctx->d_ckpt.p, 0, (size_t)nck * nrows * sizeof(float), ctx->stream));
    }
    start_full_stats(ctx, FV_KERNEL_F64_STREAM, 2);
    ctx->stats.passes = 1 + nck;
    if ((rc = fvi::begin_decode(ctx, ob, T))) return rc;
    FV_HIP(hipEventRecord(ctx->ev_start, ctx->stream));

// ... 68 lines not shown
```

flash_viterbi_amd/csrc/fv_internal.h:

```cpp
#pragma once

#include <hip/hip_runtime.h>
#include <rccl/rccl.h>

#include <algorithm>
#include <chrono>
#include <condition_variable>
#include <functional>
#include <mutex>
#include <cmath>
#include <cstdio>
#include <cstdlib>
#include <cstring>
#include <string>
#include <thread>
#include <vector>

#include "flashvit.h"
#include "fv_layout.h"
#include "fv_schedule.h"

using clk = std::chrono::steady_clock;
inline double ms_since(clk::time_point t0) { return std::chrono::duration<double, std::milli>(clk::now() - t0).count(); }

template <typename T>
struct DevBuf {
    T *p = nullptr;
    size_t n = 0;
    DevBuf() = default;
    DevBuf(const DevBuf &) = delete;
    DevBuf &operator=(const DevBuf &) = delete;
    ~DevBuf() { release(); }
    hipError_t ensure(size_t want)
    {
        if (want <= n) return hipSuccess;
        if (p) { (void)hipFree(p); p = nullptr; n = 0; }
        hipError_t e = hipMalloc(&p, want * sizeof(T));
        if (e == hipSuccess) n = want;
        return e;
    }
    void release() { if (p) (void)hipFree(p); p = nullptr; n = 0; }
    size_t bytes() const { return n * sizeof(T); }
};

namespace fvb { struct HNode { float v; int s; }; }

struct fv_ctx {
    int device = 0;
    hipStream_t stream = nullptr;
    static constexpr int BEAM_AUX = 3;
    hipStream_t aux[BEAM_AUX] = { nullptr, nullptr, nullptr };
    hipEvent_t ev_fork = nullptr, ev_join[BEAM_AUX] = { nullptr, nullptr, nullptr };
    bool fork_active = false;
    hipStream_t lstream = nullptr;
    bool forked_batches = false;
    int num_cus = 256;
    hipEvent_t ev_start = nullptr, ev_stop = nullptr, ev_top = nullptr, ev_s0 = nullptr, ev_s1 = nullptr;
    std::string detail;

    int K = 0, M = 0, nrows = 0;
    bool full_ok = false;
    bool u16_ok = false;
    bool logs_nonpositive = false;
    DevBuf<float> LA32, LB32T;
    DevBuf<unsigned short> LA16, LAQ16;
    DevBuf<uint4> SPdata;
    DevBuf<int> SPoff, SPnwb;
    double density = 1.0;
    float window16 = 0.0f;
    float windowq = 0.0f, qscale = -1.0f;
    bool laq16_ready = false;
    DevBuf<double> LA64, LB64T, LPi64;
    bool csr = false;
    DevBuf<uint4> CSk;
    DevBuf<uint2> CSq;
    DevBuf<double> CS64;
    DevBuf<long long> CSoff;
    DevBuf<int> CSnwb;
    DevBuf<long long> CRptr;
    DevBuf<int> CRcol;
    DevBuf<double> CRlog;
    DevBuf<float> E32;
    DevBuf<double> E64;
    DevBuf<unsigned long long> d_emflags;
    long long emis_rows = 0;
    bool emis_positive = false;
    DevBuf<int> EMap;
    int emis_P = 0;
    std::vector<int> h_iota;
    struct EmisView {
        const float *lb32 = nullptr;
        const double *lb64 = nullptr;
        int nsym = 0;
        bool logs_nonpositive = false;
    } view;

    DevBuf<int> d_ob, d_ans, d_bp, d_gather;
    DevBuf<float> d_rows, d_score, d_ckpt;
    DevBuf<unsigned long long> d_counters;
    DevBuf<unsigned short> d_rcodes;
    DevBuf<float> d_rtmax;
    std::vector<unsigned char> row_coded;
    int row_codes = 0;
    int launch_codes = 0;
    const void *launch_code_slots = nullptr;
    DevBuf<int> d_snap, d_flat_bp, d_chain;
    DevBuf<fvk::FlatDesc> d_flat;
    fv::FlatPlan flat_plan;
    int flat_key[4] = { 0, 0, 0, 0 };
    const void *flat_uploaded = nullptr;
    int flat_poison = -1;
    DevBuf<int> d_pack;
    int *h_pin = nullptr;
    size_t h_pin_n = 0;
    DevBuf<float> d_hval, d_scores, d_slot_val;
    DevBuf<int> d_hstate, d_slot_state, d_flags;
    DevBuf<double> LA64R;
    DevBuf<unsigned short> LAQ16R;
    bool rowq_ready = false, beam_q16_ready = false;
    DevBuf<unsigned long long> d_qaux;
    DevBuf<int2> d_tie_list;
    DevBuf<float> d_cut;
    DevBuf<fvb::HNode> d_cand;
    DevBuf<int> d_cand_count;
    float opt_sel_margin = 0.3f;
    DevBuf<int> d_dupwin;
    DevBuf<int> d_doubt, d_doubt_count;
    DevBuf<int> d_needfull;
    DevBuf<int> d_seqof;
    std::vector<int> h_seqof;
    DevBuf<int> d_passL;
    std::vector<int> h_passL;
    DevBuf<unsigned int> d_tie_count;
    DevBuf<unsigned long long> d_csr_acc;
    DevBuf<unsigned int> d_csr_tie;
    long long csr_nnz = 0;

    int opt_sparse_beam = 0;
    int opt_kernel = FV_KERNEL_AUTO;
    int opt_max_batch = fvk::MAX_BATCH;
    int opt_profile = 0;
    int opt_flat = 1;
    int opt_row_codes = 1;
    int vanilla = 0;
    int opt_csr_mem = 0;
    int opt_debug = 0;
    std::vector<hipEvent_t> prof_events;
    std::vector<int> h_ob;
    std::vector<hipGraphExec_t> graphs;
    bool test_record = false;
    unsigned long long test_variants = 0;
    unsigned long long test_selects = 0;

    ncclComm_t comm = nullptr;
    int rank = 0, nranks = 1;
    struct fv_group *group = nullptr;
    int group_rank = 0;

    fv_stats stats{};
    void start_stats(int kernel, int generations, long long table_bytes_per_step, double density_reported)
    {
        const double model_ms = stats.set_model_ms, emis_ms = stats.set_emissions_ms;
        const long long rows = stats.emission_rows;
        stats = fv_stats{};
        stats.set_model_ms = model_ms; stats.set_emissions_ms = emis_ms; stats.emission_rows = rows;
        stats.kernel = kernel; stats.generations = generations;
        stats.table_bytes_per_step = table_bytes_per_step; stats.density = density_reported;
        stats.flat_first_miss = -1;
    }
    void close_stats(long long cells_per_task_step, long long cells_per_column_step)
    {
        stats.cells = stats.task_steps * cells_per_task_step + stats.column_steps * cells_per_column_step;
        stats.alg_bytes = 4 * stats.cells;
    }

    template <class F>
    void each_buffer(F &&f) const
    {
        f(LA32); f(LB32T); f(LA16); f(LAQ16); f(SPdata); f(SPoff); f(SPnwb); f(LA64); f(LB64T); f(LPi64);
        f(CSk); f(CSq); f(CS64); f(CSoff); f(CSnwb); f(CRptr); f(CRcol); f(CRlog);
        f(E32); f(E64); f(d_emflags); f(EMap);
        f(d_ob); f(d_ans); f(d_bp); f(d_gather); f(d_rows); f(d_rcodes); f(d_rtmax); f(d_score); f(d_ckpt); f(d_counters); f(d_pack);
        f(d_snap); f(d_flat_bp); f(d_chain); f(d_flat);
        f(d_hval); f(d_scores); f(d_slot_val); f(d_hstate); f(d_slot_state); f(d_flags); f(LA64R); f(LAQ16R); f(d_qaux);
        f(d_tie_list); f(d_cut); f(d_cand); f(d_cand_count); f(d_dupwin); f(d_doubt); f(d_doubt_count); f(d_needfull);
        f(d_seqof); f(d_passL); f(d_tie_count); f(d_csr_acc); f(d_csr_tie);
    }
};

#define FV_HIP(call)                                                                          \
    do {                                                                                      \
        hipError_t e_ = (call);                                                               \
        if (e_ != hipSuccess) {                                                               \
            ctx->detail = std::string(#call) + ": " + hipGetErrorString(e_);                  \
            return e_ == hipErrorOutOfMemory ? FV_ERR_NOMEM : FV_ERR_DEVICE;                  \
        }                                                                                     \
    } while (0)

constexpr int FV_NCOUNTERS = 16;

inline int round_up(int x, int m) { return (x + m - 1) / m * m; }
inline int fv_ldq(int K) { return round_up(K, 128); }

namespace fvi {

struct HostTables {
    int K = 0, M = 0, nrows = 0, ntiles = 0;
    size_t tab = 0;
    bool full_ok = false, u16_ok = false, any_big = false;
    std::vector<double> h64, b64, pi64;
    std::vector<float> h32, b32;
    std::vector<unsigned short> h16, hq;
    std::vector<uint4> sp;
    std::vector<int> sp_off, sp_nwb;
    float window16 = 0.0f, windowq = 0.0f, qscale = -1.0f;
    double density = 1.0;
};
int build_host_tables(const float *A, const float *B, const float *Pi, int K, int M, HostTables &h, std::string &detail);
int upload_tables(fv_ctx *ctx, const HostTables &h);

size_t device_bytes(const fv_ctx *c);
struct Wants {
    struct Want { void *buf; size_t n, have, elem; hipError_t (*ensure)(void *, size_t); };
    std::vector<Want> list;
    std::string what, dominant;
    template <typename T>
    void add(DevBuf<T> &b, size_t n)
    {
        list.push_back({ &b, n, b.n, sizeof(T), [](void *p, size_t m) { return static_cast<DevBuf<T> *>(p)->ensure(m); } });
    }
};
int grant(fv_ctx *ctx, const Wants &w, bool check);
int ensure_workspace(fv_ctx *ctx, int T, size_t rows_needed, int nscores = 1, Wants w = {});
int ensure_flat_workspace(fv_ctx *ctx, int T, size_t passes, long long arg_rows, int chain_len);
int batch_lengths(fv_ctx *ctx, const char *who, const int *&ob, const long long *offsets, int nseq, int n_split, int mode,
                  const int *path_out, std::vector<int> &lengths);
int batch_symbols(fv_ctx *ctx, const char *who, const int *ob, const long long *offsets, int nseq);
int batch_plan(fv_ctx *ctx, const char *who, const std::vector<int> &lengths, int n_split, int mode, fv::Plan &plan);
std::vector<std::vector<fv::Pass>> deal_passes(const fv_ctx *ctx, const fv::Plan &plan, size_t *most = nullptr);
int finish_decode(fv_ctx *ctx, const fv::Plan &plan, const long long *offsets, int nseq, int *path_out, float *score_out,
                  int *status_out, clk::time_point t0, size_t nprof, bool beam);
int drained(fv_ctx *ctx, int rc);
int emission_view(fv_ctx *ctx, const int *&ob, long long T);
enum { FV_EMIS_BAD = 1, FV_EMIS_POSITIVE = 2 };
int launch_stage_emissions(fv_ctx *ctx, const void *src, int dtype, long long ld, int T, const int *map, int P);
int begin_decode(fv_ctx *ctx, const int *ob, int T);
int full_setup(fv_ctx *ctx);
int beam_setup(fv_ctx *ctx);
int launch_init_rows(fv_ctx *ctx, const fvk::PassChunk &ch, float *rows);
struct fv_group_barrier {
    std::mutex mu;
    std::condition_variable cv;
    int n = 1, waiting = 0;
    unsigned generation = 0;
    bool failed = false;
    bool arrive_and_wait();
    void fail();
    void reset(int members);
};
inline int group_size(const fv_ctx *ctx);
inline fv_ctx *group_member(fv_ctx *ctx, int r);
int group_run(fv_ctx *ctx, int T, int *path_out, float *score_out, const std::function<int(fv_ctx *, int *, float *)> &fn);
int gather_answers(fv_ctx *ctx, int T);
void merge_gathered(const fv::Plan &plan, const std::vector<int> &gathered, int T, int nranks, int *path);

}

struct fv_group {
    std::vector<fv_ctx *> members;
    bool rccl = false;
    fvi::fv_group_barrier barrier;
    std::vector<hipEvent_t> ans_ready;
};

namespace fvi {
inline int group_size(const fv_ctx *ctx) { return ctx->group ? (int)ctx->group->members.size() : 1; }
inline fv_ctx *group_member(fv_ctx *ctx, int r) { return ctx->group ? ctx->group->members[(size_t)r] : ctx; }
}
```

flash_viterbi_amd/csrc/fv_kernels.hip.inc:

```
#pragma once

#include <hip/hip_runtime.h>

#include <cfloat>
#include <climits>
#include <cstdint>
#include <type_traits>

#include "fv_device_common.h"

#ifdef FV_TIMING_BUILD
#define FV_TIMING_BIT(debug, bit) (((debug) & (bit)) != 0)
#else
#define FV_TIMING_BIT(debug, bit) false
#endif

namespace fvk {


struct TaskSlot {
    const float *t1_in;
    float *t1_out;
    int *bp_out;
    const float *tmp_row;
// ... 336 lines not shown
        float thr[NB];
#pragma unroll
        for (int t = 0; t < NB; ++t) {
            const float M1 = M1v[t];
            kind[t] = 0; Lc[t] = 0.0; thr[t] = FV_NEG_INF;
            if (t < args.nb && M1 > (FACTOR ? -0.5f * FLT_MAX : FV_NEG_INF) && col < K) {
                thr[t] = FACTOR ? filter_threshold<std::is_same<TA, float>::value>(M1, tmp[t], args.window)
                                : refine_threshold(M1, args.window);
                if (FV_TIMING_BIT(args.debug, 1)) kind[t] = (m1[t] == M1 && a1[t] >= 0) ? 3 : 0;
                else if (m2[t] >= thr[t] && m2[t] > FV_NEG_INF) kind[t] = 2;
                else if (m1[t] >= thr[t] && a1[t] >= 0) {
                    kind[t] = 1;
                    if constexpr (!COARSE) Lc[t] = L64t[(size_t)(a1[t] >> 2) * (TILE_W * 4) + (a1[t] & 3)];
                }
            }
        }
        if constexpr (COARSE) {
            Vec ce[NB];
#pragma unroll
            for (int t = 0; t < NB; ++t)
                if (kind[t] == 1) ce[t] = LAt[(size_t)a1[t] * (4 * TILE_W)];
#pragma unroll
            for (int t = 0; t < NB; ++t) {
                if (kind[t] == 1) {
                    AV cv[R];
                    if constexpr (std::is_same<TA, q16_t>::value) unpack_q(ce[t], cv);
                    else unpack(ce[t], cv);
                    const int k0 = a1[t] * RBR + rg * R;
                    int found = k0;
#pragma unroll
                    for (int r = R - 1; r >= 0; --r) {
                        const float s = t1_at<NB>(T1s, k0 + r, t);
                        float y;
                        if constexpr (std::is_same<TA, q16_t>::value) y = __builtin_fmaf(cv[r], args.qscale, s);
                        else y = s + cv[r];
                        found = y == m1[t] ? k0 + r : found;
                    }
                    a1[t] = found;
                    Lc[t] = L64t[(size_t)(found >> 2) * (TILE_W * 4) + (found & 3)];
                }
            }
        }
#pragma unroll
        for (int t = 0; t < NB; ++t) {
            float r = FV_NEG_INF;
            int kb = INT_MAX;
            if (kind[t] == 1) {
                r = exact_cell(tmp[t], t1_at<NB>(T1s, a1[t], t), Lc[t]);
                kb = a1[t];
                if (m1[t] != M1v[t]) atomicAdd(&args.counters[0], 1ull);
            } else if (kind[t] == 3) {
                r = m1[t]; kb = a1[t];
            }
            rr[t] = r; rk[t] = kb;
        }
        const double *L64tile = args.LA64 + (size_t)tile * nrows * TILE_W + (size_t)(row_lo >> 2) * (TILE_W * 4);
#pragma unroll
        for (int t = 0; t < NB; ++t) {
            unsigned long long need = __ballot(kind[t] == 2);
            while (need) {
                const int L = __ffsll((long long)need) - 1;
                need &= need - 1;
                const int cL = L & (TILE_W - 1), rgL = L >> 4;
                const float tmpL = __shfl(tmp[t], L);
                float bx = FV_NEG_INF;
                int bk = INT_MAX;
                const int nlane_rows = nj * R;
                for (int e0 = 0; e0 < nlane_rows; e0 += 128) {
                    int kk[2];
                    double LL[2];
#pragma unroll
                    for (int u = 0; u < 2; ++u) {
                        const int e = e0 + 64 * u + lane;
                        const int k = (w + NWV * (e / R)) * RBR + rgL * R + (e % R);
                        kk[u] = e < nlane_rows ? k : -1;
                        const int ks = kk[u] >= 0 ? k : 0;
                        LL[u] = L64tile[(size_t)(ks >> 2) * (TILE_W * 4) + cL * 4 + (ks & 3)];
                    }
#pragma unroll
                    for (int u = 0; u < 2; ++u) {
                        if (kk[u] >= 0) {
                            const float x = exact_cell(tmpL, t1_at<NB>(T1s, kk[u], t), LL[u]);
                            if (better(x, kk[u], bx, bk)) { bx = x; bk = kk[u]; }
                        }
                    }
                }
#pragma unroll
                for (int m = 1; m < 64; m <<= 1) {
                    const float ov = __shfl_xor(bx, m);
                    const int ok = __shfl_xor(bk, m);
                    if (better(ov, ok, bx, bk)) { bx = ov; bk = ok; }
                }
                if (lane == L) { rr[t] = bx; rk[t] = bk; }
                if (lane == 0) atomicAdd(&args.counters[1], 1ull);
            }
        }
#pragma unroll
        for (int t = 0; t < NB; ++t) rk[t] = rk[t] != INT_MAX ? rk[t] + row_lo : INT_MAX;
    }

#pragma unroll
    for (int t = 0; t < NB; ++t) {
        float r = rr[t];
        int kb = rk[t];
        wave_best(r, kb);
        if (lane < TILE_W) { redR[(t * TILE_W + c) * NWV + w] = r; redK[(t * TILE_W + c) * NWV + w] = kb; }
    }
    __syncthreads();
    if (w < NB && w < args.nb) {
        const float4 fv = *reinterpret_cast<const float4 *>(redR + (w * TILE_W + c) * NWV + (rg * 4) % NWV);
        const int4 fk = *reinterpret_cast<const int4 *>(redK + (w * TILE_W + c) * NWV + (rg * 4) % NWV);
        float r = fv.x;
        int kb = fk.x;
        if (better(fv.y, fk.y, r, kb)) { r = fv.y; kb = fk.y; }
        if (better(fv.z, fk.z, r, kb)) { r = fv.z; kb = fk.z; }
        if (better(fv.w, fk.w, r, kb)) { r = fv.w; kb = fk.w; }
        wave_best(r, kb);
        if (lane < TILE_W && col < K) {
            if (args.merge) {
                const float pv = args.t[w].t1_out[col];
                const int pk = args.t[w].bp_out[col];
                if (pk >= 0 && !(r > pv)) { r = pv; kb = pk; }
            }
            const bool any = r > -FLT_MAX;
            args.t[w].t1_out[col] = any ? r : -FLT_MAX;
            args.t[w].bp_out[col] = any ? kb : -1;
        }
    }
}


typedef unsigned short fv_u16x2 __attribute__((ext_vector_type(2)));
__device__ __forceinline__ unsigned int pk_adds(unsigned int a, unsigned int b)
{
    return __builtin_bit_cast(unsigned int, __builtin_elementwise_add_sat(__builtin_bit_cast(fv_u16x2, a), __builtin_bit_cast(fv_u16x2, b)));
}
__device__ __forceinline__ unsigned int pk_minu(unsigned int a, unsigned int b)
{
    return __builtin_bit_cast(unsigned int, __builtin_elementwise_min(__builtin_bit_cast(fv_u16x2, a), __builtin_bit_cast(fv_u16x2, b)));
}
__device__ __forceinline__ unsigned int pk_maxu(unsigned int a, unsigned int b)
{
    return __builtin_bit_cast(unsigned int, __builtin_elementwise_max(__builtin_bit_cast(fv_u16x2, a), __builtin_bit_cast(fv_u16x2, b)));
}

__device__ __forceinline__ unsigned int score_code(float mx, float v, float inv_step)
{
    const float q = (mx - v) * inv_step;
    return (v > -0.5f * FLT_MAX && q < 65534.5f) ? (unsigned int)__float2uint_rn(q) : 65535u;
}

template <int NB, bool DB, int NWV> constexpr bool u16_takes_codes() { return !(NB == 8 && NWV == 16 && !DB); }

template <int NB, int U, bool DB, int NWV>
__global__ __launch_bounds__(NWV * 64) void trellis_step_u16(const StepArgs<NB> args)
{
    constexpr int R = 8, RBR = 32;
    extern __shared__ __align__(16) unsigned char smem[];
    const int nrows = args.nrows, npairs = nrows >> 1;
    unsigned int *T1c = reinterpret_cast<unsigned int *>(smem);
    unsigned int *redZ = T1c + (size_t)NB * npairs;
    float *redR = reinterpret_cast<float *>(redZ + NB * NWV * TILE_W);
    int *redK = reinterpret_cast<int *>(redR + NB * NWV * TILE_W);
    unsigned int *colZ = reinterpret_cast<unsigned int *>(redK + NB * NWV * TILE_W);

    const int tid = threadIdx.x, lane = tid & 63, w = tid >> 6;
    const int c = lane & (TILE_W - 1), rg = lane >> 4;
    const int tile = (blockIdx.x & 7) * args.tiles_per_xcd + (blockIdx.x >> 3);
    if (tile >= args.ntiles) return;
    const int col = tile * TILE_W + c;
    const int K = args.K;
    const bool rev = args.reverse != 0;
    const unsigned short *tile_base = reinterpret_cast<const unsigned short *>(args.LA) + (size_t)tile * nrows * TILE_W;
    const uint4 *LAt = reinterpret_cast<const uint4 *>(tile_base) + rg * TILE_W + c;
    const int nq = nrows / RBR;
    const int nj = nq > w ? (nq - w + NWV - 1) / NWV : 0;
    auto block_of = [&](int p) { return w + NWV * (rev ? nj - 1 - p : p); };

    float Mx[NB], tmp[NB];
    const float step = -args.qscale, inv_step = 1.0f / step;
    const int nq4 = nrows >> 2;
    constexpr int QPT = 1024 / (NWV * 64);
    uint4 cur[U], nxt[DB ? U : 1];
    auto request_table = [&]() {
        __builtin_amdgcn_sched_barrier(0);
#pragma unroll
        for (int u = 0; u < U; ++u)
            if (u < nj) cur[u] = LAt[(size_t)block_of(u) * (4 * TILE_W)];
        __builtin_amdgcn_sched_barrier(0);
#pragma unroll
        for (int t = 0; t < NB; ++t) tmp[t] = args.t[t].tmp_row[min(col, K - 1)];
        __builtin_amdgcn_sched_barrier(0);
    };
    const bool coded = u16_takes_codes<NB, DB, NWV>() && (args.codes & 1) != 0;
    const int nch = nrows >> 3;
    if (coded) {
        uint4 cv[NB];
        float tw[NB], tm[NB][4];
        const int ch = min(tid, nch - 1);
#pragma unroll
        for (int t = 0; t < NB; ++t) cv[t] = reinterpret_cast<const uint4 *>(args.c[t].c_in)[ch];
        auto request_maxima = [&]() {
#pragma unroll
            for (int t = 0; t < NB; ++t) {
                tw[t] = args.c[t].tmax_in[ch >> 1];
#pragma unroll
                for (int j = 0; j < 4; ++j) tm[t][j] = args.c[t].tmax_in[min(lane + 64 * j, args.ntiles - 1)];
            }
        };
        if constexpr (NB < 8) request_maxima();
        request_table();
        if constexpr (NB >= 8) request_maxima();
#pragma unroll
        for (int t = 0; t < NB; ++t) {
            float x = fmaxf(fmaxf(tm[t][0], tm[t][1]), fmaxf(tm[t][2], tm[t][3]));
            for (int i = 256 + lane; i < args.ntiles; i += 64) x = fmaxf(x, args.c[t].tmax_in[i]);
#pragma unroll
            for (int m = 1; m < 64; m <<= 1) x = fmaxf(x, __shfl_xor(x, m));
            Mx[t] = x;
        }
        auto put = [&](int ch, int t, const uint4 &p, float tmax_w) {
            const unsigned int d = score_code(Mx[t], tmax_w, inv_step), dd = d | (d << 16);
            *reinterpret_cast<uint4 *>(T1c + (size_t)t * npairs + 4 * ch) = make_uint4(pk_adds(p.x, dd), pk_adds(p.y, dd), pk_adds(p.z, dd), pk_adds(p.w, dd));
        };
        if (tid < nch) {
#pragma unroll
            for (int t = 0; t < NB; ++t) put(tid, t, cv[t], tw[t]);
        }
        for (int ch = NWV * 64 + tid; ch < nch; ch += NWV * 64) {
#pragma unroll
            for (int t = 0; t < NB; ++t) put(ch, t, reinterpret_cast<const uint4 *>(args.c[t].c_in)[ch], args.c[t].tmax_in[ch >> 1]);
        }
    } else {
        float4 v0[QPT][NB];
#pragma unroll
        for (int h = 0; h < QPT; ++h) {
            const int q = min(h * (NWV * 64) + tid, nq4 - 1);
#pragma unroll
            for (int t = 0; t < NB; ++t) v0[h][t] = reinterpret_cast<const float4 *>(args.t[t].t1_in)[q];
        }
        request_table();
        float *redM = reinterpret_cast<float *>(redZ);
        float pm[NB];
        auto fold = [&](int q, const float4 &v, float &m) {
            const int r0 = 4 * q;
            m = r0 < K ? fmaxf(m, v.x) : m;
            m = r0 + 1 < K ? fmaxf(m, v.y) : m;
            m = r0 + 2 < K ? fmaxf(m, v.z) : m;
            m = r0 + 3 < K ? fmaxf(m, v.w) : m;
        };
#pragma unroll
        for (int t = 0; t < NB; ++t) {
            pm[t] = FV_NEG_INF;
#pragma unroll
            for (int h = 0; h < QPT; ++h)
                if (h * (NWV * 64) + tid < nq4) fold(h * (NWV * 64) + tid, v0[h][t], pm[t]);
        }
        for (int q = 1024 + tid; q < nq4; q += NWV * 64) {
#pragma unroll
            for (int t = 0; t < NB; ++t) fold(q, reinterpret_cast<const float4 *>(args.t[t].t1_in)[q], pm[t]);
        }
#pragma unroll
        for (int t = 0; t < NB; ++t) {
#pragma unroll
            for (int m = 1; m < 64; m <<= 1) pm[t] = fmaxf(pm[t], __shfl_xor(pm[t], m));
            if (lane == 0) redM[t * NWV + w] = pm[t];
        }
        __syncthreads();
#pragma unroll
        for (int t = 0; t < NB; ++t) {
            float x = redM[t * NWV + (lane & (NWV - 1))];
#pragma unroll
            for (int m = 1; m < NWV; m <<= 1) x = fmaxf(x, __shfl_xor(x, m));
            Mx[t] = x;
        }
        auto put = [&](int q, int t, const float4 &v) {
            uint2 wd;
            wd.x = score_code(Mx[t], v.x, inv_step) | (score_code(Mx[t], v.y, inv_step) << 16);
            wd.y = score_code(Mx[t], v.z, inv_step) | (score_code(Mx[t], v.w, inv_step) << 16);
            *reinterpret_cast<uint2 *>(T1c + (size_t)t * npairs + 2 * q) = wd;
        };
#pragma unroll
        for (int h = 0; h < QPT; ++h)
            if (h * (NWV * 64) + tid < nq4) {
#pragma unroll
                for (int t = 0; t < NB; ++t) put(h * (NWV * 64) + tid, t, v0[h][t]);
            }
        for (int q = 1024 + tid; q < nq4; q += NWV * 64) {
#pragma unroll
            for (int t = 0; t < NB; ++t) put(q, t, reinterpret_cast<const float4 *>(args.t[t].t1_in)[q]);
        }
    }
    __syncthreads();

    unsigned int m1p[NB], m2p[NB];
    int alo[NB], ahi[NB];
#pragma unroll
    for (int t = 0; t < NB; ++t) { m1p[t] = 0xffffffffu; m2p[t] = 0xffffffffu; alo[t] = -1; ahi[t] = -1; }

    for (int p0 = 0; p0 < (FV_TIMING_BIT(args.debug, 2048) ? 0 : (DB ? nj : 1)); p0 += U) {
        if constexpr (DB) {
            if (p0 + U < nj) {
#pragma unroll
                for (int u = 0; u < U; ++u)
                    if (p0 + U + u < nj) nxt[u] = LAt[(size_t)block_of(p0 + U + u) * (4 * TILE_W)];
            }
        }
#pragma unroll
        for (int u = 0; u < U; ++u) {
            if (p0 + u < nj) {
                const int qb = block_of(p0 + u);
                const unsigned int ca[4] = { cur[u].x, cur[u].y, cur[u].z, cur[u].w };
                const int pb = qb * (RBR / 2) + rg * (R / 2);
#pragma unroll
                for (int t = 0; t < NB; ++t) {
                    const uint4 ct4 = *reinterpret_cast<const uint4 *>(T1c + (size_t)t * npairs + pb);
                    const unsigned int ct[4] = { ct4.x, ct4.y, ct4.z, ct4.w };
                    const unsigned int old = m1p[t];
#pragma unroll
                    for (int i = 0; i < 4; ++i) {
                        const unsigned int z = pk_adds(ca[i], ct[i]);
                        m2p[t] = pk_minu(m2p[t], pk_maxu(z, m1p[t]));
                        m1p[t] = pk_minu(m1p[t], z);
                    }
                    const unsigned int x = m1p[t] ^ old;
                    alo[t] = (x & 0xffffu) ? qb : alo[t];
                    ahi[t] = (x >> 16) ? qb : ahi[t];
                }
            }
        }
        if constexpr (DB) {
#pragma unroll
            for (int u = 0; u < U; ++u) cur[u] = nxt[u];
        }
    }

    unsigned int m1[NB], m2[NB];
    int a1[NB], par[NB];
#pragma unroll
    for (int t = 0; t < NB; ++t) {
        const unsigned int lo = m1p[t] & 0xffffu, hi = m1p[t] >> 16;
        par[t] = hi < lo ? 1 : 0;
        m1[t] = par[t] ? hi : lo;
        a1[t] = par[t] ? ahi[t] : alo[t];
        m2[t] = min(max(lo, hi), min(m2p[t] & 0xffffu, m2p[t] >> 16));
    }

    constexpr bool SPEC = !DB && NB <= 2;
    double Lc[NB];
    float tv[NB];
    const double *L64t = args.LA64 + (size_t)tile * nrows * TILE_W + c * 4;
    const int blk0 = nj > 0 ? block_of(0) : 0;
    auto locate = [&](int t, int blk, const uint4 &ce) -> int {
        const unsigned int ca[4] = { ce.x, ce.y, ce.z, ce.w };
        const uint4 ct4 = *reinterpret_cast<const uint4 *>(T1c + (size_t)t * npairs + blk * (RBR / 2) + rg * (R / 2));
        const unsigned int ct[4] = { ct4.x, ct4.y, ct4.z, ct4.w };
        const int k0 = blk * RBR + rg * R;
        int found = k0 + par[t];
#pragma unroll
        for (int i = 3; i >= 0; --i) {
            const unsigned int z = pk_adds(ca[i], ct[i]);
            const unsigned int zh = par[t] ? (z >> 16) : (z & 0xffffu);
            found = zh == m1[t] ? k0 + 2 * i + par[t] : found;
        }
        return found;
    };
    if constexpr (SPEC) {
#pragma unroll
        for (int t = 0; t < NB; ++t) {
            const int blk = a1[t] >= 0 ? a1[t] : blk0;
            const int jj = (blk - w) / NWV;
            const int pos = rev ? nj - 1 - jj : jj;
            uint4 ce = cur[0];
#pragma unroll
            for (int u = 1; u < U; ++u) {
                const bool hit = u == pos;
                ce.x = hit ? cur[u].x : ce.x; ce.y = hit ? cur[u].y : ce.y; ce.z = hit ? cur[u].z : ce.z; ce.w = hit ? cur[u].w : ce.w;
            }
            const int found = locate(t, blk, ce);
            a1[t] = a1[t] >= 0 ? found : -1;
        }
    }

    unsigned int Zc[NB];
#pragma unroll
    for (int t = 0; t < NB; ++t) {
        unsigned int v = m1[t];
        v = min(v, (unsigned int)__shfl_xor((int)v, 16));
        v = min(v, (unsigned int)__shfl_xor((int)v, 32));
        if (lane < TILE_W) redZ[(t * TILE_W + c) * NWV + w] = v;
    }
    __syncthreads();
    if constexpr (NB <= 2) {
#pragma unroll
        for (int t = 0; t < NB; ++t) {
            const uint4 *q = reinterpret_cast<const uint4 *>(redZ + (t * TILE_W + c) * NWV);
            unsigned int v = 0xffffffffu;
#pragma unroll
            for (int x = 0; x < NWV / 4; ++x) {
                const uint4 f = q[x];
                v = min(min(v, min(f.x, f.y)), min(f.z, f.w));
            }
            Zc[t] = v;
        }
    } else {
        if (w < NB) {
            const uint4 f = *reinterpret_cast<const uint4 *>(redZ + (w * TILE_W + c) * NWV + (rg * 4) % NWV);
            unsigned int v = min(min(f.x, f.y), min(f.z, f.w));
            v = min(v, (unsigned int)__shfl_xor((int)v, 16));
            v = min(v, (unsigned int)__shfl_xor((int)v, 32));
            if (lane < TILE_W) colZ[w * TILE_W + c] = v;
        }
        __syncthreads();
#pragma unroll
        for (int t = 0; t < NB; ++t) Zc[t] = colZ[t * TILE_W + c];
    }

    float rr[NB];
    int rk[NB];
    {
        int kind[NB];
#pragma unroll
        for (int t = 0; t < NB; ++t) {
            kind[t] = 0;
            if (t < args.nb && col < K && !FV_TIMING_BIT(args.debug, 4096)) {
                const float zz = fabsf(Mx[t] + tmp[t]) + 65536.0f * step + 1.0f;
                const unsigned int eb = __float_as_uint(zz) & 0x7f800000u;
                const float Uf = (eb > (24u << 23) && eb < 0x7f800000u) ? __uint_as_float(eb - (23u << 23)) : (eb >= 0x7f800000u ? 0.0f : FLT_MIN);
                const float wf = (2.0f * Uf + args.window) * inv_step + (coded ? 4.2f : 3.1f);
                const unsigned int W = wf < 65535.0f ? (unsigned int)wf + 1u : 65535u;
                const unsigned int thr = Zc[t] + W;
                if (thr >= 65535u) {
                    kind[t] = 2;
                    if (w == 0 && rg == 0) atomicAdd(&args.counters[8], 1ull);
                }
                else if (m2[t] <= thr) kind[t] = 2;
                else if (m1[t] <= thr && a1[t] >= 0) kind[t] = 1;
            }
        }
        if constexpr (SPEC) {
#pragma unroll
            for (int t = 0; t < NB; ++t) {
                Lc[t] = 0.0; tv[t] = 0.0f;
                if (kind[t] == 1) {
                    Lc[t] = L64t[(size_t)(a1[t] >> 2) * (TILE_W * 4) + (a1[t] & 3)];
                    tv[t] = args.t[t].t1_in[a1[t]];
                }
            }
        } else {
            uint4 ce[NB];
#pragma unroll
            for (int t = 0; t < NB; ++t) ce[t] = LAt[(size_t)(kind[t] == 1 ? a1[t] : blk0) * (4 * TILE_W)];
#pragma unroll
            for (int t = 0; t < NB; ++t) {
                const int found = locate(t, kind[t] == 1 ? a1[t] : blk0, ce[t]);
                a1[t] = found;
                Lc[t] = L64t[(size_t)(found >> 2) * (TILE_W * 4) + (found & 3)];
                tv[t] = args.t[t].t1_in[found];
            }
        }
#pragma unroll
        for (int t = 0; t < NB; ++t) {
            float r = FV_NEG_INF;
            int kb = INT_MAX;
            if (kind[t] == 1) {
                r = exact_cell(tmp[t], tv[t], Lc[t]);
                kb = a1[t];
                if (m1[t] != Zc[t]) atomicAdd(&args.counters[0], 1ull);
            }
            rr[t] = r; rk[t] = kb;
        }
        const double *L64tile = args.LA64 + (size_t)tile * nrows * TILE_W;
#pragma unroll
        for (int t = 0; t < NB; ++t) {
            unsigned long long need = __ballot(kind[t] == 2);
            while (need) {
                const int L = __ffsll((long long)need) - 1;
                need &= need - 1;
                const int cL = L & (TILE_W - 1), rgL = L >> 4;
                const float tmpL = __shfl(tmp[t], L);
                const float *t1g = args.t[t].t1_in;
                float bx = FV_NEG_INF;
                int bk = INT_MAX;
                const int nlane_rows = nj * R;
                for (int e0 = 0; e0 < nlane_rows; e0 += 128) {
                    int kk[2];
                    float tt[2];
                    double LL[2];
#pragma unroll
                    for (int u = 0; u < 2; ++u) {
                        const int e = e0 + 64 * u + lane;
                        const int k = (w + NWV * (e / R)) * RBR + rgL * R + (e % R);
                        kk[u] = (e < nlane_rows && k < K) ? k : -1;
                        const int ks = kk[u] >= 0 ? k : 0;
                        tt[u] = t1g[ks];
                        LL[u] = L64tile[(size_t)(ks >> 2) * (TILE_W * 4) + cL * 4 + (ks & 3)];
                    }
#pragma unroll
                    for (int u = 0; u < 2; ++u) {
                        if (kk[u] >= 0) {
                            const float x = exact_cell(tmpL, tt[u], LL[u]);
                            if (better(x, kk[u], bx, bk)) { bx = x; bk = kk[u]; }
                        }
                    }
                }
#pragma unroll
                for (int m = 1; m < 64; m <<= 1) {
                    const float ov = __shfl_xor(bx, m);
                    const int ok = __shfl_xor(bk, m);
                    if (better(ov, ok, bx, bk)) { bx = ov; bk = ok; }
                }
                if (lane == L) { rr[t] = bx; rk[t] = bk; }
                if (lane == 0) atomicAdd(&args.counters[1], 1ull);
            }
        }
    }

#pragma unroll
    for (int t = 0; t < NB; ++t) {
        float r = rr[t];
        int kb = rk[t];
        wave_best(r, kb);
        if (lane < TILE_W) { redR[(t * TILE_W + c) * NWV + w] = r; redK[(t * TILE_W + c) * NWV + w] = kb; }
    }
    __syncthreads();
    if (w < NB && w < args.nb) {
        const float4 fv = *reinterpret_cast<const float4 *>(redR + (w * TILE_W + c) * NWV + (rg * 4) % NWV);
        const int4 fk = *reinterpret_cast<const int4 *>(redK + (w * TILE_W + c) * NWV + (rg * 4) % NWV);
        float r = fv.x;
        int kb = fk.x;
        if (better(fv.y, fk.y, r, kb)) { r = fv.y; kb = fk.y; }
        if (better(fv.z, fk.z, r, kb)) { r = fv.z; kb = fk.z; }
        if (better(fv.w, fk.w, r, kb)) { r = fv.w; kb = fk.w; }
        wave_best(r, kb);
        const bool any = r > -FLT_MAX;
        if (lane < TILE_W && col < K) {
            args.t[w].t1_out[col] = any ? r : -FLT_MAX;
            args.t[w].bp_out[col] = any ? kb : -1;
        }
        if (args.codes & 2) {
            const float val = (col < K && any) ? r : -FLT_MAX;
            float tmx = val;
#pragma unroll
            for (int m = 1; m < TILE_W; m <<= 1) tmx = fmaxf(tmx, __shfl_xor(tmx, m));
            if (lane < TILE_W) {
                args.c[w].c_out[col] = (unsigned short)score_code(tmx, val, inv_step);
                if (lane == 0) args.c[w].tmax_out[tile] = tmx;
            }
        }
    }
}

__global__ void q16_tile_range(const double *t4, size_t n, unsigned long long *lmax_bits)
{
    double m = 0.0;
    for (size_t e = (size_t)blockIdx.x * blockDim.x + threadIdx.x; e < n; e += (size_t)gridDim.x * blockDim.x) {
        const double l = t4[e];
        if (l > -__builtin_huge_val() && -l > m) m = -l;
    }
#pragma unroll
    for (int k = 1; k < 64; k <<= 1) { const double o = __shfl_xor(m, k); m = o > m ? o : m; }
    if ((threadIdx.x & 63) == 0 && m > 0.0) atomicMax(lmax_bits, (unsigned long long)__double_as_longlong(m));
}

__global__ void q16_tile_codes(const double *t4, unsigned short *q8, int K, int nrows, int ntiles,
                               const unsigned long long *lmax_bits, unsigned long long *dmax_bits)
{
    const double lmax = __longlong_as_double((long long)*lmax_bits);
    const float stepf = lmax > 0.0 ? (float)(lmax / 65534.0) : 1.0f;
    const double stepd = (double)stepf;
    const size_t n = (size_t)ntiles * nrows * TILE_W;
    double dm = 0.0;
    for (size_t e = (size_t)blockIdx.x * blockDim.x + threadIdx.x; e < n; e += (size_t)gridDim.x * blockDim.x) {
        const int tile = (int)(e / ((size_t)nrows * TILE_W));
        const int rem = (int)(e % ((size_t)nrows * TILE_W));
        const int k = rem / TILE_W, col = tile * TILE_W + rem % TILE_W;
        unsigned short code = 0xFFFFu;
        const double l = t4[tab_index<4>(k, col, nrows)];
        if (k < K && col < K && l > -__builtin_huge_val()) {
            double c = nearbyint(-l / stepd);
            c = c < 0.0 ? 0.0 : (c > 65534.0 ? 65534.0 : c);
            code = (unsigned short)c;
            const double d = fabs(-c * stepd - l);
            dm = d > dm ? d : dm;
        }
        q8[tab_index<8>(k, col, nrows)] = code;
    }
#pragma unroll
    for (int k = 1; k < 64; k <<= 1) { const double o = __shfl_xor(dm, k); dm = o > dm ? o : dm; }
    if ((threadIdx.x & 63) == 0 && dm > 0.0) atomicMax(dmax_bits, (unsigned long long)__double_as_longlong(dm));
}


constexpr int SP_WAVES = 8;
constexpr int SP_BLOCK = SP_WAVES * 64;

template <int NB>
struct SparseArgs {
    const uint4 *data;
    const int *tile_off;
    const int *tile_nwb;
    const double *LA64;
    unsigned long long *counters;
    int K, nrows, ntiles, tiles_per_xcd, nb, debug;
    float window, qscale;
    TaskSlot t[NB];
};

template <int NB>
__global__ __launch_bounds__(SP_BLOCK) void trellis_step_sparse(const SparseArgs<NB> args)
{
    extern __shared__ __align__(16) unsigned char smem[];
    const int nrows = args.nrows;
    float *T1s = reinterpret_cast<float *>(smem);
    float *redV = T1s + (size_t)nrows * NB;
    float *redR = redV + NB * SP_WAVES * TILE_W;
    int *redK = reinterpret_cast<int *>(redR + NB * SP_WAVES * TILE_W);

    const int tid = threadIdx.x, lane = tid & 63, w = tid >> 6;
    const int c = lane & (TILE_W - 1), rg = lane >> 4;
    const int tile = (blockIdx.x & 7) * args.tiles_per_xcd + (blockIdx.x >> 3);
    if (tile >= args.ntiles) return;
    if (FV_TIMING_BIT(args.debug, 16)) return;
    const int col = tile * TILE_W + c;
    const int K = args.K;
    const uint4 *base = args.data + args.tile_off[tile] + rg * TILE_W + c;
    const int nwb = args.tile_nwb[tile];
    const int nj = nwb > w ? (nwb - w + SP_WAVES - 1) / SP_WAVES : 0;
    constexpr int U = 4;
    uint4 cur[U];
#pragma unroll
    for (int u = 0; u < U; ++u)
        if (u < nj) cur[u] = base[(size_t)(w + SP_WAVES * u) * (4 * TILE_W)];

    float tmp[NB];
    if (!FV_TIMING_BIT(args.debug, 32)) stage_rows<NB, SP_BLOCK>(T1s, args.t, nrows, tid);
#pragma unroll
    for (int t = 0; t < NB; ++t) tmp[t] = (t < args.nb && col < K) ? args.t[t].tmp_row[col] : 0.0f;
    __syncthreads();

    float m1[NB], m2[NB];
    int a1[NB];
#pragma unroll
    for (int t = 0; t < NB; ++t) { m1[t] = FV_NEG_INF; m2[t] = FV_NEG_INF; a1[t] = -1; }

    auto visit = [&](unsigned int word) {
        const int k = (int)(word >> 16);
        const float qf = q2f(word & 0xffffu);
        float tv[NB];
        load_t1<NB>(T1s, k, tv);
#pragma unroll
        for (int t = 0; t < NB; ++t) {
            const float y = __builtin_fmaf(qf, args.qscale, tmp[t] + tv[t]);
            const bool gt = y > m1[t];
            m2[t] = __builtin_amdgcn_fmed3f(y, m1[t], m2[t]);
            m1[t] = gt ? y : m1[t];
            a1[t] = gt ? k : a1[t];
        }
    };
    for (int p0 = 0; p0 < nj; p0 += U) {
#pragma unroll
        for (int u = 0; u < U; ++u) {
            if (p0 + u < nj) {
                const uint4 e = cur[u];
                visit(e.x); visit(e.y); visit(e.z); visit(e.w);
            }
        }
        if (p0 + U < nj) {
#pragma unroll
            for (int u = 0; u < U; ++u)
                if (p0 + U + u < nj) cur[u] = base[(size_t)(w + SP_WAVES * (p0 + U + u)) * (4 * TILE_W)];
        }
    }

    float M1v[NB];
#pragma unroll
    for (int t = 0; t < NB; ++t) {
        float v = m1[t];
        v = fmaxf(v, __shfl_xor(v, 16));
        v = fmaxf(v, __shfl_xor(v, 32));
        if (lane < TILE_W) redV[(t * TILE_W + c) * SP_WAVES + w] = v;
    }
    __syncthreads();
#pragma unroll
    for (int t = 0; t < NB; ++t) {
        const float4 *q = reinterpret_cast<const float4 *>(redV + (t * TILE_W + c) * SP_WAVES);
        const float4 f0 = q[0], f1 = q[1];
        M1v[t] = fmaxf(fmaxf(fmaxf(f0.x, f0.y), fmaxf(f0.z, f0.w)), fmaxf(fmaxf(f1.x, f1.y), fmaxf(f1.z, f1.w)));
    }

    const double *L64t = args.LA64 + (size_t)tile * nrows * TILE_W + c * 4;
    float rr[NB];
    int rk[NB];
    double Lc[NB];
    int kind[NB];
    float thr[NB];
#pragma unroll
    for (int t = 0; t < NB; ++t) {
        const float M1 = M1v[t];
        kind[t] = 0; Lc[t] = 0.0; thr[t] = FV_NEG_INF;
        if (t < args.nb && M1 > FV_NEG_INF && col < K) {
            thr[t] = refine_threshold(M1, args.window);
// ... 738 lines not shown
```

flash_viterbi_amd/csrc/fv_layout.h:

```cpp
#pragma once

#include <hip/hip_runtime.h>

#include <cstddef>

namespace fvk {

constexpr int TILE_W = 16;
constexpr int ROWG = 64 / TILE_W;
constexpr int NWAVES = 16;
constexpr int BLOCK = NWAVES * 64;
constexpr int ROW_ALIGN = 32;
constexpr int MAX_BATCH = 8;

template <int R>
__host__ __device__ inline size_t tab_index(int k, int col, int nrows)
{
    return (size_t)(col >> 4) * nrows * TILE_W + ((size_t)(k / R) * TILE_W + (col & 15)) * R + (k % R);
}
constexpr int BT_WARMUP = 32, BT_MIN_PARALLEL = 128;
struct PassDesc { int L, R, from_pi, whole; long long row_off; };
constexpr int PASS_CHUNK = 64;
struct PassChunk { int n; PassDesc p[PASS_CHUNK]; };
struct FlatDesc { int L, R, generation, chain; long long arg_row; };
constexpr int FLAT_MAX_GENS = 40;
struct FlatGens { int ngen; int begin[FLAT_MAX_GENS + 1]; };
constexpr int FLAT_COUNTER = 15;

template <int NB>
static inline size_t step_lds_bytes(int nrows)
{
    return (size_t)nrows * NB * 4 + (size_t)NB * NWAVES * TILE_W * 12 + (size_t)NB * TILE_W * 4;
}

template <int NB, int NWV>
static inline size_t u16_lds_bytes(int nrows)
{
    return (size_t)nrows * NB * 2 + (size_t)NB * NWV * TILE_W * 12 + (size_t)NB * TILE_W * 4;
}

}
```

flash_viterbi_amd/decoder.py:

```python
import ctypes
import os

import numpy as np

from . import build as _build

MODE_REFERENCE = 0
MODE_SINGLE_PASS = 1
KERNEL_AUTO, KERNEL_F64_STREAM, KERNEL_F32_REFINE, KERNEL_F16_REFINE, KERNEL_Q16_REFINE, KERNEL_SPARSE_Q16 = 0, 1, 2, 3, 4, 5
KERNEL_U16_REFINE = 6
KERNEL_SPARSE_CSR = 7
KERNEL_CSR_F64 = 8
OPT_KERNEL, OPT_MAX_BATCH, OPT_PROFILE, OPT_SEL_MARGIN, OPT_DEBUG = 1, 2, 3, 4, 100
OPT_FLAT_GENERATIONS = 5
OPT_ROW_CODES = 6
OPT_SPARSE_BEAM = 7
FLAT_OFF, FLAT_AUTO, FLAT_ON = 0, 1, 2
DEBUG_TIMING_ONLY = (1 << 0) | (1 << 4) | (1 << 5) | (1 << 11) | (1 << 12)
DEBUG_BATCH_GEN0_SERIAL = 1 << 28
DEBUG_BEAM_BATCH_GEN0_OTHER = 1 << 29
DEBUG_CSR_ROWS_IN_MEMORY = 1 << 31
TV_CSR64_NB = (1 << 58, 1 << 59, 1 << 60, 1 << 61)
TV_CSR64_MEM = 1 << 62
TV_BEAM_CSR = (1 << 46) | (1 << 47)
TV_ROW_CODES = 1 << 63
WARN_BEAM_MISS = 1
ERR_ARG, ERR_NOMEM, ERR_NO_PRED, ERR_DEVICE, ERR_STATE, ERR_UNSUPPORTED = -1, -2, -3, -4, -5, -6
UNIQUE_ID_BYTES = 128
EMIS_LOG_F32, EMIS_LOG_F64 = 0, 1
EMIS_LOG_F16, EMIS_LOG_BF16 = 2, 3
_EMIS_OF_NUMPY = {np.dtype(np.float32): EMIS_LOG_F32, np.dtype(np.float64): EMIS_LOG_F64, np.dtype(np.float16): EMIS_LOG_F16}


class Stats(ctypes.Structure):
    _fields_ = [("set_model_ms", ctypes.c_double), ("decode_ms", ctypes.c_double), ("gpu_ms", ctypes.c_double),
                ("top_pass_ms", ctypes.c_double), ("top_steps_ms", ctypes.c_double),
                ("step_kernel_ms", ctypes.c_double),
                ("step_launches", ctypes.c_longlong), ("task_steps", ctypes.c_longlong),
                ("column_steps", ctypes.c_longlong),
                ("cells", ctypes.c_longlong), ("alg_bytes", ctypes.c_longlong),
                ("table_bytes_per_step", ctypes.c_longlong), ("device_bytes", ctypes.c_longlong),
                ("refine_near", ctypes.c_longlong), ("refine_rescan", ctypes.c_longlong),
                ("beam_exact_sets", ctypes.c_longlong), ("beam_ties", ctypes.c_longlong),
                ("beam_dup_cols", ctypes.c_longlong), ("beam_dup_steps", ctypes.c_longlong),
                ("beam_cand_selects", ctypes.c_longlong), ("density", ctypes.c_double),
                ("passes", ctypes.c_int), ("generations", ctypes.c_int), ("kernel", ctypes.c_int),
                ("ranks", ctypes.c_int), ("refine_saturated", ctypes.c_longlong),
                ("beam_spec_steps", ctypes.c_longlong), ("beam_reach_events", ctypes.c_longlong),
                ("beam_list_short", ctypes.c_longlong), ("beam_list_long", ctypes.c_longlong), ("beam_list_entries", ctypes.c_longlong),
                ("beam_chain_cuts", ctypes.c_longlong),
                ("flat_passes", ctypes.c_int), ("flat_missed", ctypes.c_int), ("flat_first_miss", ctypes.c_int),
                ("set_emissions_ms", ctypes.c_double), ("emission_rows", ctypes.c_longlong)]

    def as_dict(self):
        return {k: getattr(self, k) for k, _ in self._fields_}


class FlatInfo(ctypes.Structure):
    _fields_ = [("L", ctypes.c_int), ("R", ctypes.c_int), ("generation", ctypes.c_int), ("batch", ctypes.c_int),
                ("stream", ctypes.c_int), ("chain", ctypes.c_int), ("arg_row", ctypes.c_longlong)]


class PassInfo(ctypes.Structure):
    _fields_ = [("L", ctypes.c_int), ("R", ctypes.c_int), ("generation", ctypes.c_int), ("owner", ctypes.c_int)]


EXPORTS = ["fv_create", "fv_destroy", "fv_set_model", "fv_set_option", "fv_decode_full", "fv_decode_beam",
           "fv_decode_vanilla", "fv_decode_checkpoint", "fv_checkpoint_memory_bytes",
           "fv_last_stats", "fv_strerror", "fv_last_error_detail", "fv_reference_memory_bytes",
           "fv_comm_unique_id", "fv_comm_init", "fv_plan_passes", "fv_merge_paths", "fv_set_partition",
           "fv_create_multi", "fv_device_count", "fv_decode_full_batch", "fv_plan_passes_batch", "fv_decode_beam_batch",
           "fv_set_model_sparse", "fv_set_emissions", "fv_clear_emissions", "fv_plan_flat", "fv_set_emission_map"]
TEST_EXPORTS = ["fv_test_forward", "fv_test_beam_step", "fv_test_beam_select", "fv_test_device_alloc", "fv_test_device_free",
                "fv_test_stage_emissions_ms", "fv_test_flat_poison"]
TIE_TAG = 1 << 30
TS_BITS = {"topb_select<4,listed>": 1 << 0, "topb_select<4,derived>": 1 << 1, "topb_select<16,listed>": 1 << 2,
           "topb_select<16,derived>": 1 << 3, "topb_select<64,listed>": 1 << 4, "topb_select<64,derived>": 1 << 5,
           "topb_select_cand<8,listed>": 1 << 6, "topb_select_cand<8,derived>": 1 << 7, "topb_select_cand<16,listed>": 1 << 8,
           "topb_select_cand<16,derived>": 1 << 9, "heap_build_all": 1 << 10}
TS_ALL = (1 << 11) - 1
CUT_THETA, CUT_STATE, CUT_NEXT, CUT_LIST, CUT_N, CUT_MARGIN, CUT_W = 0, 1, 2, 3, 4, 5, 8
BEAM_EXTRA = 32
SELECT_COUNTERS = (2, 5, 7, 9, 10, 11, 12, 13)


class ForwardPass(ctypes.Structure):
    _fields_ = [("L", ctypes.c_int), ("R", ctypes.c_int), ("init_state", ctypes.c_int)]


class SelectSet(ctypes.Structure):
    _fields_ = [("scores", ctypes.c_void_p), ("cand", ctypes.c_void_p), ("cand_count", ctypes.c_int)]


class BeamSet(ctypes.Structure):
    _fields_ = [("val", ctypes.c_void_p), ("state", ctypes.c_void_p), ("n", ctypes.c_int)]

_lib = None


def load_library():
    global _lib
    if _lib is not None:
        return _lib
    path = _build.HIP_TIMING_LIB if os.environ.get("FLASHVIT_TIMING_BUILD") == "1" else _build.HIP_LIB
    if not os.path.isfile(path):
        raise RuntimeError(f"{path} is missing: run `python -c 'import __graft_entry__ as g; g.build()'` "
                           "(hipcc --offload-arch=gfx950); there is no CPU fallback")
    L = ctypes.CDLL(path)
    vp, ci, cll = ctypes.c_void_p, ctypes.c_int, ctypes.c_longlong
    L.fv_create.argtypes = [ctypes.POINTER(vp), ci]
    L.fv_create_multi.argtypes = [ctypes.POINTER(vp), vp, ci]
    L.fv_device_count.argtypes = []
    L.fv_destroy.argtypes = [vp]
    L.fv_destroy.restype = None
    L.fv_set_model.argtypes = [vp, vp, vp, vp, ci, ci]
    L.fv_set_model_sparse.argtypes = [vp, vp, vp, vp, vp, vp, ci, ci]
    L.fv_set_option.argtypes = [vp, ci, cll]
    L.fv_set_emissions.argtypes = [vp, vp, ci, ci, cll]
    L.fv_clear_emissions.argtypes = [vp]
    L.fv_set_emission_map.argtypes = [vp, vp, ci]
    L.fv_test_device_alloc.argtypes = [vp, ctypes.c_size_t, vp, ctypes.POINTER(vp)]
    L.fv_test_device_free.argtypes = [vp, vp]
    L.fv_test_stage_emissions_ms.argtypes = [vp, vp, ctypes.c_int, ctypes.c_int, ctypes.c_longlong, ctypes.c_int, ctypes.POINTER(ctypes.c_float)]
    L.fv_decode_full.argtypes = [vp, vp, ci, ci, ci, vp, vp]
    L.fv_decode_beam.argtypes = [vp, vp, ci, ci, ci, ci, vp, vp]
    L.fv_decode_full_batch.argtypes = [vp, vp, vp, ci, ci, ci, vp, vp, vp]
    L.fv_decode_beam_batch.argtypes = [vp, vp, vp, ci, ci, ci, ci, vp, vp, vp]
    L.fv_plan_passes_batch.argtypes = [vp, ci, ci, ci, ctypes.POINTER(PassInfo), ci]
    L.fv_decode_vanilla.argtypes = [vp, vp, ci, vp, vp]
    L.fv_decode_checkpoint.argtypes = [vp, vp, ci, ci, vp, vp]
    L.fv_checkpoint_memory_bytes.argtypes = [ci, ci, ci]
    L.fv_checkpoint_memory_bytes.restype = ctypes.c_longlong
    L.fv_last_stats.argtypes = [vp, ctypes.POINTER(Stats)]
    L.fv_strerror.argtypes = [ci]
    L.fv_strerror.restype = ctypes.c_char_p
    L.fv_last_error_detail.argtypes = [vp]
    L.fv_last_error_detail.restype = ctypes.c_char_p
    L.fv_reference_memory_bytes.argtypes = [ci, ci, ci, ci]
    L.fv_reference_memory_bytes.restype = cll
    L.fv_comm_unique_id.argtypes = [vp]
    L.fv_comm_init.argtypes = [vp, ci, ci, vp]
    L.fv_set_partition.argtypes = [vp, ci, ci]
    L.fv_plan_passes.argtypes = [ci, ci, ci, ci, ctypes.POINTER(PassInfo), ci]
    L.fv_merge_paths.argtypes = [ci, ci, ci, vp, vp]
    L.fv_plan_flat.argtypes = [ci, ci, ci, ci, ctypes.POINTER(FlatInfo), ci]
    L.fv_test_flat_poison.argtypes = [vp, ci]
    L.fv_test_forward.argtypes = [vp, vp, ci, ctypes.POINTER(ForwardPass), ci, vp, vp, ctypes.POINTER(ctypes.c_ulonglong)]
    cf = ctypes.c_float
    L.fv_test_beam_step.argtypes = [vp, ci, ctypes.POINTER(BeamSet), ci, vp, ci, cf, cf, ci, vp, vp, vp, ctypes.POINTER(ci),
                                    vp, vp, vp, vp, ctypes.POINTER(ctypes.c_ulonglong)]
    L.fv_test_beam_select.argtypes = [vp, ci, ci, ci, ctypes.POINTER(SelectSet), ci, cf, cf, vp, ci, ctypes.POINTER(ci), vp,
                                      vp, vp, vp, vp, vp, ctypes.POINTER(ctypes.c_ulonglong)]
    _lib = L
    return L


class FlashVitError(RuntimeError):
    def __init__(self, rc, detail=""):
        msg = load_library().fv_strerror(rc).decode()
        super().__init__(f"flashvit: {msg} ({rc})" + (f": {detail}" if detail else ""))
        self.rc = rc


def plan_passes(T, n_split, mode=MODE_REFERENCE, nranks=1):
    L = load_library()
    n = L.fv_plan_passes(T, n_split, mode, nranks, None, 0)
    if n < 0:
        raise FlashVitError(n)
    buf = (PassInfo * n)()
    L.fv_plan_passes(T, n_split, mode, nranks, buf, n)
    return [(p.L, p.R, p.generation, p.owner) for p in buf]


def plan_flat(T, n_split, batch_cap=4, nstreams=3):
    L = load_library()
    n = L.fv_plan_flat(T, n_split, batch_cap, nstreams, None, 0)
    if n < 0:
        raise FlashVitError(n)
    buf = (FlatInfo * max(n, 1))()
    L.fv_plan_flat(T, n_split, batch_cap, nstreams, buf, n)
    return [{k: getattr(buf[i], k) for k, _ in FlatInfo._fields_} for i in range(n)]


def plan_passes_batch(lengths, n_split, mode=MODE_REFERENCE):
    L = load_library()
    lens = np.ascontiguousarray(lengths, dtype=np.int32)
    n = L.fv_plan_passes_batch(_p(lens), lens.size, n_split, mode, None, 0)
    if n < 0:
        raise FlashVitError(n)
    buf = (PassInfo * n)()
    L.fv_plan_passes_batch(_p(lens), lens.size, n_split, mode, buf, n)
    return [(p.L, p.R, p.generation, p.owner) for p in buf]


def merge_paths(T, n_split, nranks, gathered):
    g = np.ascontiguousarray(gathered, dtype=np.int32).reshape(nranks * T)
    out = np.empty(T, dtype=np.int32)
    rc = load_library().fv_merge_paths(T, n_split, nranks, _p(g), _p(out))
    if rc < 0:
        raise FlashVitError(rc)
    return out


def reference_memory_bytes(K, T, n_split, beam=0):
    return int(load_library().fv_reference_memory_bytes(K, T, n_split, beam))


def checkpoint_memory_bytes(K, T, step=0):
    return int(load_library().fv_checkpoint_memory_bytes(K, T, step))


def _p(a):
    return a.ctypes.data_as(ctypes.c_void_p)


def _is_torch_tensor(x):
    return type(x).__module__.split(".")[0] == "torch" and hasattr(x, "data_ptr")


def _ob_arg(ob, T):
    if ob is None:
        if T is None:
            raise ValueError("ob=None decodes the staged emission scores: give T, the number of times")
        return None, None, int(T)
    ob = np.ascontiguousarray(ob, dtype=np.int32)
    if T is not None and int(T) != ob.size:
        raise ValueError("T differs from the length of ob")
    return ob, _p(ob), ob.size


def _batch_arg(obs, lengths):
    if obs is None:
        if lengths is None:
            raise ValueError("obs=None decodes the staged emission scores: give lengths")
        sizes, ob, ptr = [int(n) for n in lengths], None, None
    else:
        if lengths is not None:
            raise ValueError("lengths goes with obs=None")
        seqs = [np.ascontiguousarray(o, dtype=np.int32).reshape(-1) for o in obs]
        sizes = [o.size for o in seqs]
        ob = np.concatenate(seqs) if seqs else np.zeros(0, dtype=np.int32)
        ptr = _p(ob)
    offsets = np.zeros(len(sizes) + 1, dtype=np.int64)
    if sizes:
        offsets[1:] = np.cumsum(sizes)
    return ob, ptr, offsets


def dense_to_csr(A):
    A = np.ascontiguousarray(A, dtype=np.float32)
    assert A.ndim == 2 and A.shape[0] == A.shape[1]
    rows, cols = np.nonzero(A != 0)
    indptr = np.zeros(A.shape[0] + 1, dtype=np.int64)
    np.cumsum(np.bincount(rows, minlength=A.shape[0]), out=indptr[1:])
    return indptr, cols.astype(np.int32), A[rows, cols]


class FlashViterbi:

    def __init__(self, device=0):
        self._L = load_library()
        h = ctypes.c_void_p()
        if isinstance(device, (list, tuple)):
            devs = np.ascontiguousarray(device, dtype=np.int32)
            rc = self._L.fv_create_multi(ctypes.byref(h), _p(devs), devs.size)
        else:
            rc = self._L.fv_create(ctypes.byref(h), device)
        if rc != 0:
            raise FlashVitError(rc, "fv_create (is a GPU visible? there is no CPU fallback)")
        self._h = h
        self.K = self.M = 0
        self.P = 0

    def close(self):
        if getattr(self, "_h", None):
            self._L.fv_destroy(self._h)
            self._h = None

    def __del__(self):
        self.close()

    def _check(self, rc):
        if rc < 0:
            raise FlashVitError(rc, self._L.fv_last_error_detail(self._h).decode())
        return rc

    def set_option(self, key, value):
        self._check(self._L.fv_set_option(self._h, key, int(value)))

    def set_model(self, A, B, Pi):
        A = np.ascontiguousarray(A, dtype=np.float32)
        B = np.ascontiguousarray(B, dtype=np.float32)
        Pi = np.ascontiguousarray(Pi, dtype=np.float32)
        K, M = B.shape
        assert A.shape == (K, K) and Pi.shape == (K,)
        self._check(self._L.fv_set_model(self._h, _p(A), _p(B), _p(Pi), K, M))
        self.K, self.M, self.P = K, M, 0

    def set_model_sparse(self, indptr, indices, data, B, Pi):
        indptr = np.ascontiguousarray(indptr, dtype=np.int64)
        indices = np.ascontiguousarray(indices, dtype=np.int32)
        data = np.ascontiguousarray(data, dtype=np.float32)
        B = np.ascontiguousarray(B, dtype=np.float32)
        Pi = np.ascontiguousarray(Pi, dtype=np.float32)
        K, M = B.shape
        assert indptr.shape == (K + 1,) and Pi.shape == (K,) and indices.shape == data.shape and indices.ndim == 1
        assert indptr[-1] <= indices.size, "indptr[K] exceeds the number of stored entries"
        self._check(self._L.fv_set_model_sparse(self._h, _p(indptr), _p(indices), _p(data), _p(B), _p(Pi), K, M))
        self.K, self.M, self.P = K, M, 0

    def set_emission_map(self, pdf_of_state, P=None):
        if pdf_of_state is None:
            self._check(self._L.fv_set_emission_map(self._h, None, 0))
            self.P = 0
            return
        m = np.ascontiguousarray(pdf_of_state, dtype=np.int32)
        if m.shape != (self.K,):
            raise ValueError("set_emission_map: one entry per state of the model")
        P = int(m.max()) + 1 if P is None else int(P)
        self._check(self._L.fv_set_emission_map(self._h, _p(m), P))
        self.P = P

    def set_emissions(self, scores, ld=None):
        if isinstance(scores, tuple):
            ptr, dtype, T, pitch = scores
            if ld is not None:
                pitch = ld
            if isinstance(dtype, (type, np.dtype, str)):
                dtype = _EMIS_OF_NUMPY.get(np.dtype(dtype), -1)
            self._check(self._L.fv_set_emissions(self._h, ctypes.c_void_p(int(ptr)), int(dtype), int(T), int(pitch)))
            return
        if _is_torch_tensor(scores):
            import torch
            codes = {torch.float16: EMIS_LOG_F16, torch.bfloat16: EMIS_LOG_BF16, torch.float32: EMIS_LOG_F32, torch.float64: EMIS_LOG_F64}
            if scores.dim() != 2 or scores.dtype not in codes or scores.stride(1) != 1 or scores.shape[0] < 1 or scores.shape[1] < 1:
                raise TypeError("set_emissions: a torch tensor must be 2-D, float16 / bfloat16 / float32 / float64, with stride(1) == 1")
            pitch = scores.stride(0) if ld is None else int(ld)
            if scores.shape[0] == 1:
                pitch = max(pitch, scores.shape[1])
            if scores.is_cuda:
                torch.cuda.current_stream(scores.device).synchronize()
            self._check(self._L.fv_set_emissions(self._h, ctypes.c_void_p(scores.data_ptr()), codes[scores.dtype],
                                                 scores.shape[0], pitch))
            return
        a = np.asarray(scores)
        if a.ndim != 2 or a.dtype not in _EMIS_OF_NUMPY:
            raise TypeError("set_emissions: a 2-D float16, float32 or float64 array, a torch tensor, or (device_pointer, dtype, T, ld)")
        a = np.ascontiguousarray(a)
        pitch = a.shape[1] if ld is None else int(ld)
        if pitch > a.shape[1] and a.shape[0] > 1:
            raise ValueError("set_emissions: ld exceeds the row length of the array")
        self._check(self._L.fv_set_emissions(self._h, _p(a), _EMIS_OF_NUMPY[a.dtype], a.shape[0], pitch))

    def clear_emissions(self):
        self._check(self._L.fv_clear_emissions(self._h))

    def decode_full(self, ob, n_split=1, mode=MODE_REFERENCE, T=None):
        ob, ptr, T = _ob_arg(ob, T)
        path = np.empty(T, dtype=np.int32)
        score = ctypes.c_float(0)
        rc = self._check(self._L.fv_decode_full(self._h, ptr, T, n_split, mode, _p(path), ctypes.byref(score)))
        return path, np.float32(score.value), rc

    def decode_full_batch(self, obs, n_split=1, mode=MODE_REFERENCE, lengths=None):
        ob, ptr, offsets = _batch_arg(obs, lengths)
        nseq = offsets.size - 1
        path = np.empty(max(int(offsets[-1]), 1), dtype=np.int32)
        scores = np.zeros(nseq, dtype=np.float32)
        statuses = np.zeros(nseq, dtype=np.int32)
        rc = self._L.fv_decode_full_batch(self._h, ptr, _p(offsets), nseq, n_split, mode, _p(path), _p(scores), _p(statuses))
        if rc != ERR_NO_PRED:
            self._check(rc)
        return [path[offsets[s]:offsets[s + 1]].copy() for s in range(nseq)], scores, statuses

    def decode_beam(self, ob, n_split, beam, mode=MODE_REFERENCE, T=None):
        ob, ptr, T = _ob_arg(ob, T)
        path = np.empty(T, dtype=np.int32)
        score = ctypes.c_float(0)
        rc = self._check(self._L.fv_decode_beam(self._h, ptr, T, n_split, beam, mode, _p(path), ctypes.byref(score)))
        return path, np.float32(score.value), rc

    def decode_beam_batch(self, obs, n_split, beam, mode=MODE_REFERENCE, lengths=None):
        ob, ptr, offsets = _batch_arg(obs, lengths)
        nseq = offsets.size - 1
        path = np.empty(max(int(offsets[-1]), 1), dtype=np.int32)
        scores = np.zeros(nseq, dtype=np.float32)
        statuses = np.zeros(nseq, dtype=np.int32)
        self._check(self._L.fv_decode_beam_batch(self._h, ptr, _p(offsets), nseq, n_split, beam, mode, _p(path),
                                                 _p(scores), _p(statuses)))
        return [path[offsets[s]:offsets[s + 1]].copy() for s in range(nseq)], scores, statuses

    def decode_vanilla(self, ob, T=None):
        ob, ptr, T = _ob_arg(ob, T)
        path = np.empty(T, dtype=np.int32)
        score = ctypes.c_float(0)
        rc = self._check(self._L.fv_decode_vanilla(self._h, ptr, T, _p(path), ctypes.byref(score)))
        return path, np.float32(score.value), rc

    def decode_checkpoint(self, ob, step=0, T=None):
        ob, ptr, T = _ob_arg(ob, T)
        path = np.empty(T, dtype=np.int32)
        score = ctypes.c_float(0)
        rc = self._check(self._L.fv_decode_checkpoint(self._h, ptr, T, step, _p(path), ctypes.byref(score)))
        return path, np.float32(score.value), rc

    def test_flat_poison(self, t):
        self._check(self._L.fv_test_flat_poison(self._h, int(t)))

    def test_device_alloc(self, host_array):
        a = np.ascontiguousarray(host_array)
        out = ctypes.c_void_p()
        self._check(self._L.fv_test_device_alloc(self._h, a.nbytes, _p(a), ctypes.byref(out)))
        return int(out.value)

    def test_device_free(self, ptr):
        self._check(self._L.fv_test_device_free(self._h, ctypes.c_void_p(int(ptr))))

    def test_stage_emissions_ms(self, ptr, dtype, T, ld, reps):
        ms = ctypes.c_float(0)
        code = dtype if isinstance(dtype, int) else _EMIS_OF_NUMPY.get(np.dtype(dtype), -1)
        self._check(self._L.fv_test_stage_emissions_ms(self._h, ctypes.c_void_p(int(ptr)), int(code), int(T), int(ld), int(reps), ctypes.byref(ms)))
        return float(ms.value)

    def test_forward(self, ob, passes, bp_fill=-2, T=None):
        ob, ptr, T = _ob_arg(ob, T)
        pa = (ForwardPass * len(passes))(*[ForwardPass(int(L), int(R), int(s)) for L, R, s in passes])
        rows = np.empty((len(passes), self.K), dtype=np.float32)
        bp = np.full((T, self.K), bp_fill, dtype=np.int32)
        variants = ctypes.c_ulonglong(0)
        self._check(self._L.fv_test_forward(self._h, ptr, T, pa, len(passes), _p(rows), _p(bp), ctypes.byref(variants)))
        return rows, bp, int(variants.value)

    def test_beam_step(self, beam, sets, syms, speculative=False, theta=0.0, next_bound=float("inf"), cand_cap=0):
        K = self.K
        vals = [np.ascontiguousarray(v, dtype=np.float32) for v, _ in sets]
        sts = [np.ascontiguousarray(s, dtype=np.int32) for _, s in sets]
        arr = (BeamSet * len(sets))(*[BeamSet(_p(v).value, _p(s).value, v.size) for v, s in zip(vals, sts)])
        syms = np.ascontiguousarray(syms, dtype=np.int32)
        n = len(sets)
        scores = np.empty((n, K), dtype=np.float32)
        bp = np.empty((n, K), dtype=np.int32)
        ties = np.empty((n * K, 2), dtype=np.int32)
        nties = ctypes.c_int(0)
        doubt = np.empty((n, 1024), dtype=np.int32)
        doubt_counts = np.empty(n, dtype=np.int32)
        cand = np.empty((n, max(cand_cap, 1), 2), dtype=np.int32)
        cand_counts = np.zeros(n, dtype=np.int32)
        variants = ctypes.c_ulonglong(0)
        self._check(self._L.fv_test_beam_step(self._h, int(beam), arr, n, _p(syms), 1 if speculative else 0, float(theta),
                                              float(next_bound), int(cand_cap), _p(scores), _p(bp), _p(ties), ctypes.byref(nties),
                                              _p(doubt), _p(doubt_counts), _p(cand), _p(cand_counts), ctypes.byref(variants)))
        out_cand = []
        for q in range(n):
            c = int(cand_counts[q])
            rows = cand[q, :min(c, cand_cap)]
            out_cand.append((c, [(rows[i, 0:1].view(np.float32)[0], int(rows[i, 1])) for i in range(rows.shape[0])]))
        return dict(scores=scores, bp=bp, ties={(int(a), int(b)) for a, b in ties[:nties.value]},
                    doubt=[(int(doubt_counts[q]), doubt[q, :min(int(doubt_counts[q]), 1024)].tolist()) for q in range(n)],
                    cand=out_cand, variants=int(variants.value))

    def select_cand_cap(self, K, beam):
        cap = ctypes.c_int(-1)
        self._check(self._L.fv_test_beam_select(self._h, int(K), int(beam), 0, None, 0, 0.0, 0.0, None, 0, ctypes.byref(cap),
                                                None, None, None, None, None, None, None))
        return int(cap.value)

    def test_beam_select(self, beam, rows, s=0, lists=None, prev_theta=0.0, prev_margin=0.0, seed=None, want_layout=True):
        rows = np.ascontiguousarray(rows, dtype=np.float32)
        n, K = rows.shape
        BP = beam + BEAM_EXTRA
        keep = []
        arr = (SelectSet * n)()
        for q in range(n):
            arr[q].scores = rows[q:q + 1].ctypes.data
            if lists is not None and lists[q] is not None:
                count, vals, states = lists[q]
                rec = np.empty((len(vals), 2), dtype=np.int32)
                rec[:, 0] = np.ascontiguousarray(vals, dtype=np.float32).view(np.int32)
                rec[:, 1] = states
                keep.append(rec)
                arr[q].cand = rec.ctypes.data
                arr[q].cand_count = int(count)
        cap = ctypes.c_int(-1)
        cut = np.empty((n, CUT_W), dtype=np.float32)
        mval = np.empty((n, BP), dtype=np.float32)
        mstate = np.empty((n, BP), dtype=np.int32)
        counters = np.zeros(len(SELECT_COUNTERS), dtype=np.uint64)
        sval = np.empty((n, beam), dtype=np.float32)
        sstate = np.empty((n, beam), dtype=np.int32)
        selects = ctypes.c_ulonglong(0)
        sd = None if seed is None else np.ascontiguousarray(seed, dtype=np.float32)
        self._check(self._L.fv_test_beam_select(self._h, K, int(beam), int(s), arr, n, float(prev_theta), float(prev_margin),
                                                None if sd is None else _p(sd), 1 if want_layout else 0, ctypes.byref(cap),
                                                _p(cut), _p(mval), _p(mstate), _p(counters), _p(sval), _p(sstate),
                                                ctypes.byref(selects)))
        members = []
        for q in range(n):
            cn = int(cut[q, CUT_N]) if np.isfinite(cut[q, CUT_N]) else 0
            cn = max(0, min(cn, BP))
            members.append((mval[q, :cn].copy(), mstate[q, :cn].copy()))
        out = dict(cut=cut, members=members, raw_val=mval, raw_state=mstate,
                   counters={c: int(v) for c, v in zip(SELECT_COUNTERS, counters)}, selects=int(selects.value),
                   cand_cap=int(cap.value))
        if want_layout:
            out["slot_val"], out["slot_state"] = sval, sstate
        return out

    def stats(self):
        s = Stats()
        self._check(self._L.fv_last_stats(self._h, ctypes.byref(s)))
        return s.as_dict()

    def set_partition(self, rank, nranks):
        self._check(self._L.fv_set_partition(self._h, rank, nranks))

    def comm_init(self, rank, nranks, unique_id):
        buf = ctypes.create_string_buffer(bytes(unique_id), UNIQUE_ID_BYTES)
        self._check(self._L.fv_comm_init(self._h, rank, nranks, buf))


def device_count():
    return int(load_library().fv_device_count())


def comm_unique_id():
    buf = ctypes.create_string_buffer(UNIQUE_ID_BYTES)
    rc = load_library().fv_comm_unique_id(buf)
    if rc != 0:
        raise FlashVitError(rc)
    return buf.raw
```

include/flashvit.h:

```cpp
#ifndef FLASHVIT_H
#define FLASHVIT_H

#include <stddef.h>

#ifdef __cplusplus
extern "C" {
#endif

typedef struct fv_ctx fv_ctx;

enum {
    FV_OK = 0,
    FV_WARN_BEAM_MISS = 1,
    FV_ERR_ARG = -1,
    FV_ERR_NOMEM = -2,
    FV_ERR_NO_PRED = -3,
    FV_ERR_DEVICE = -4,
    FV_ERR_STATE = -5,
    FV_ERR_UNSUPPORTED = -6,
    FV_ERR_COMM = -7,
};

enum {
    FV_MODE_REFERENCE = 0,
    FV_MODE_SINGLE_PASS = 1,
};

enum {
    FV_OPT_KERNEL = 1,
    FV_OPT_MAX_BATCH = 2,
    FV_OPT_PROFILE = 3,
    FV_OPT_SEL_MARGIN = 4,
    FV_OPT_FLAT_GENERATIONS = 5,
    FV_OPT_ROW_CODES = 6,
    FV_OPT_SPARSE_BEAM = 7,
    FV_OPT_DEBUG = 100,
};
#define FV_DEBUG_TIMING_ONLY ((1 << 0) | (1 << 4) | (1 << 5) | (1 << 11) | (1 << 12))
enum {
    FV_KERNEL_AUTO = 0,
    FV_KERNEL_F64_STREAM = 1,
    FV_KERNEL_F32_REFINE = 2,
    FV_KERNEL_F16_REFINE = 3,
    FV_KERNEL_Q16_REFINE = 4,
    FV_KERNEL_U16_REFINE = 6,
    FV_KERNEL_SPARSE_Q16 = 5,
    FV_KERNEL_SPARSE_CSR = 7,
    FV_KERNEL_CSR_F64 = 8,
};

typedef struct {
    double set_model_ms;
    double decode_ms;
    double gpu_ms;
    double top_pass_ms;
    double top_steps_ms;
    double step_kernel_ms;
    long long step_launches;
    long long task_steps;
    long long column_steps;
    long long cells;
    long long alg_bytes;
    long long table_bytes_per_step;
    long long device_bytes;
    long long refine_near;
    long long refine_rescan;
    long long beam_exact_sets;
    long long beam_ties;
    long long beam_dup_cols;
    long long beam_dup_steps;
    long long beam_cand_selects;
    double density;
    int passes;
    int generations;
    int kernel;
    int ranks;
    long long refine_saturated;
    long long beam_spec_steps;
    long long beam_reach_events;
    long long beam_list_short;
    long long beam_list_long;
    long long beam_list_entries;
    long long beam_chain_cuts;
    int flat_passes;
    int flat_missed;
    int flat_first_miss;
    double set_emissions_ms;
    long long emission_rows;
} fv_stats;

int fv_create(fv_ctx **out, int device);
void fv_destroy(fv_ctx *ctx);

int fv_create_multi(fv_ctx **out, const int *devices, int ndev);
int fv_device_count(void);

int fv_set_model(fv_ctx *ctx, const float *A, const float *B, const float *Pi, int K, int M);

int fv_set_model_sparse(fv_ctx *ctx, const long long *row_ptr, const int *col, const float *val,
                        const float *B, const float *Pi, int K, int M);

enum { FV_EMIS_LOG_F32 = 0, FV_EMIS_LOG_F64 = 1 };
int fv_set_emissions(fv_ctx *ctx, const void *scores, int dtype, int T, long long ld);
int fv_clear_emissions(fv_ctx *ctx);
enum { FV_EMIS_LOG_F16 = 2, FV_EMIS_LOG_BF16 = 3 };
int fv_set_emission_map(fv_ctx *ctx, const int *pdf_of_state, int P);

int fv_set_option(fv_ctx *ctx, int key, long long value);

int fv_decode_full(fv_ctx *ctx, const int *ob, int T, int n_split, int mode,
                   int *path_out, float *score_out);

int fv_decode_full_batch(fv_ctx *ctx, const int *ob, const long long *offsets, int nseq, int n_split, int mode,
                         int *path_out, float *score_out, int *status_out);

int fv_decode_beam(fv_ctx *ctx, const int *ob, int T, int n_split, int beam_width, int mode,
                   int *path_out, float *score_out);

int fv_decode_beam_batch(fv_ctx *ctx, const int *ob, const long long *offsets, int nseq, int n_split,
                         int beam_width, int mode, int *path_out, float *score_out, int *status_out);

int fv_decode_vanilla(fv_ctx *ctx, const int *ob, int T, int *path_out, float *score_out);

int fv_decode_checkpoint(fv_ctx *ctx, const int *ob, int T, int step, int *path_out, float *score_out);
long long fv_checkpoint_memory_bytes(int K, int T, int step);

int fv_last_stats(const fv_ctx *ctx, fv_stats *out);
const char *fv_strerror(int rc);
const char *fv_last_error_detail(const fv_ctx *ctx);

long long fv_reference_memory_bytes(int K, int T, int n_split, int beam_width);

#define FV_UNIQUE_ID_BYTES 128
int fv_comm_unique_id(void *id_out);
int fv_comm_init(fv_ctx *ctx, int rank, int nranks, const void *id);

int fv_set_partition(fv_ctx *ctx, int rank, int nranks);

int fv_merge_paths(int T, int n_split, int nranks, const int *gathered, int *path_out);

typedef struct { int L, R, generation, owner; } fv_pass_info;
int fv_plan_passes(int T, int n_split, int mode, int nranks, fv_pass_info *out, int cap);

typedef struct { int L, R, generation, batch, stream, chain; long long arg_row; } fv_flat_info;
int fv_plan_flat(int T, int n_split, int batch_cap, int nstreams, fv_flat_info *out, int cap);

int fv_plan_passes_batch(const int *lengths, int nseq, int n_split, int mode, fv_pass_info *out, int cap);

#ifdef __cplusplus
}
#endif
#endif
```

include/flashvit_testing.h:

```cpp
#ifndef FLASHVIT_TESTING_H
#define FLASHVIT_TESTING_H

#include "flashvit.h"

#ifdef __cplusplus
extern "C" {
#endif

typedef struct { int L, R, init_state; } fv_test_pass;

int fv_test_forward(fv_ctx *ctx, const int *ob, int T, const fv_test_pass *passes, int npasses,
                    float *rows_out, int *bp_out, unsigned long long *variants_out);

int fv_test_flat_poison(fv_ctx *ctx, int t);

int fv_test_device_alloc(fv_ctx *ctx, size_t bytes, const void *host_src, void **out);
int fv_test_device_free(fv_ctx *ctx, void *p);

int fv_test_stage_emissions_ms(fv_ctx *ctx, const void *dev_scores, int dtype, int T, long long ld, int reps, float *ms_out);

typedef struct { const float *val; const int *state; int n; } fv_test_beam_set;
typedef struct { float value; int state; } fv_test_cand;

#define FV_TEST_TIE_TAG (1 << 30)
int fv_test_beam_step(fv_ctx *ctx, int beam, const fv_test_beam_set *sets, int nsets, const int *sym, int speculative,
                      float theta, float next_bound, int cand_cap, float *scores_out, int *bp_out, int *ties_out,
                      int *tie_count_out, int *doubt_out, int *doubt_counts, fv_test_cand *cand_out, int *cand_counts,
                      unsigned long long *variants_out);

typedef struct { const float *scores; const fv_test_cand *cand; int cand_count; } fv_test_select_set;

int fv_test_beam_select(fv_ctx *ctx, int K, int beam, int s, const fv_test_select_set *sets, int nsets, float prev_theta,
                        float prev_margin, const float *seed, int want_layout, int *cand_cap_out, float *cut_out,
                        float *member_val_out, int *member_state_out, unsigned long long *counters_out, float *slot_val_out,
                        int *slot_state_out, unsigned long long *selects_out);

#define FV_TS_SEL4_LISTED     (1ull << 0)
#define FV_TS_SEL4_DERIVED    (1ull << 1)
#define FV_TS_SEL16_LISTED    (1ull << 2)
#define FV_TS_SEL16_DERIVED   (1ull << 3)
#define FV_TS_SEL64_LISTED    (1ull << 4)
#define FV_TS_SEL64_DERIVED   (1ull << 5)
#define FV_TS_CAND8_LISTED    (1ull << 6)
#define FV_TS_CAND8_DERIVED   (1ull << 7)
#define FV_TS_CAND16_LISTED   (1ull << 8)
#define FV_TS_CAND16_DERIVED  (1ull << 9)
#define FV_TS_HEAP_BUILD_ALL  (1ull << 10)
#define FV_TS_ALL             ((1ull << 11) - 1)

#define FV_TV_F64_NB1        (1ull << 0)
#define FV_TV_F64_NB2        (1ull << 1)
#define FV_TV_F64_NB4        (1ull << 2)
#define FV_TV_F64_NB8        (1ull << 3)
#define FV_TV_F32_NB1        (1ull << 4)
#define FV_TV_F32_NB2        (1ull << 5)
#define FV_TV_F32_NB4        (1ull << 6)
#define FV_TV_F32_NB8        (1ull << 7)
#define FV_TV_F32_UP_NB1     (1ull << 8)
#define FV_TV_F32_UP_NB2     (1ull << 9)
#define FV_TV_F16_NB1        (1ull << 10)
#define FV_TV_F16_NB2        (1ull << 11)
#define FV_TV_F16_NB4        (1ull << 12)
#define FV_TV_F16_NB8        (1ull << 13)
#define FV_TV_F16_UP_NB1     (1ull << 14)
#define FV_TV_F16_UP_NB2     (1ull << 15)
#define FV_TV_Q16_NB1        (1ull << 16)
#define FV_TV_Q16_NB2        (1ull << 17)
#define FV_TV_Q16_NB4        (1ull << 18)
#define FV_TV_Q16_NB8        (1ull << 19)
#define FV_TV_Q16_UP_NB1     (1ull << 20)
#define FV_TV_Q16_UP_NB2     (1ull << 21)
#define FV_TV_SLAB_F64       (1ull << 22)
#define FV_TV_SLAB_F32       (1ull << 23)
#define FV_TV_SLAB_F16       (1ull << 24)
#define FV_TV_SLAB_Q16       (1ull << 25)
#define FV_TV_U16_W16_UP_NB1 (1ull << 26)
#define FV_TV_U16_W16_UP_NB2 (1ull << 27)
#define FV_TV_U16_W16_UP_NB4 (1ull << 28)
#define FV_TV_U16_W16_UP_NB8 (1ull << 29)
#define FV_TV_U16_W16_NB1    (1ull << 30)
#define FV_TV_U16_W16_NB2    (1ull << 31)
#define FV_TV_U16_W16_NB4    (1ull << 32)
#define FV_TV_U16_W16_NB8    (1ull << 33)
#define FV_TV_U16_W8_UP_NB1  (1ull << 34)
#define FV_TV_U16_W8_UP_NB2  (1ull << 35)
#define FV_TV_U16_W8_UP_NB4  (1ull << 36)
#define FV_TV_U16_W8_UP_NB8  (1ull << 37)
#define FV_TV_U16_W8_NB1     (1ull << 38)
#define FV_TV_U16_W8_NB2     (1ull << 39)
#define FV_TV_U16_W8_NB4     (1ull << 40)
#define FV_TV_U16_W8_NB8     (1ull << 41)
#define FV_TV_SPARSE_NB1     (1ull << 42)
#define FV_TV_SPARSE_NB2     (1ull << 43)
#define FV_TV_SPARSE_NB4     (1ull << 44)
#define FV_TV_SPARSE_NB8     (1ull << 45)
#define FV_TV_BEAM_W4        (1ull << 46)
#define FV_TV_BEAM_W16       (1ull << 47)
#define FV_TV_BEAM_Q16_W8    (1ull << 48)
#define FV_TV_BEAM_Q16_W16   (1ull << 49)
#define FV_TV_BEAM_CSR       (FV_TV_BEAM_W4 | FV_TV_BEAM_W16)
#define FV_TV_CSR_SHIFT      50
#define FV_TV_CSR_LDS_NB1    (1ull << (FV_TV_CSR_SHIFT + 0))
#define FV_TV_CSR_LDS_NB2    (1ull << (FV_TV_CSR_SHIFT + 1))
#define FV_TV_CSR_LDS_NB4    (1ull << (FV_TV_CSR_SHIFT + 2))
#define FV_TV_CSR_LDS_NB8    (1ull << (FV_TV_CSR_SHIFT + 3))
#define FV_TV_CSR_MEM_NB1    (1ull << (FV_TV_CSR_SHIFT + 4))
#define FV_TV_CSR_MEM_NB2    (1ull << (FV_TV_CSR_SHIFT + 5))
#define FV_TV_CSR_MEM_NB4    (1ull << (FV_TV_CSR_SHIFT + 6))
#define FV_TV_CSR_MEM_NB8    (1ull << (FV_TV_CSR_SHIFT + 7))
#define FV_TV_CSR64_SHIFT    58
#define FV_TV_CSR64_NB1      (1ull << (FV_TV_CSR64_SHIFT + 0))
#define FV_TV_CSR64_NB2      (1ull << (FV_TV_CSR64_SHIFT + 1))
#define FV_TV_CSR64_NB4      (1ull << (FV_TV_CSR64_SHIFT + 2))
#define FV_TV_CSR64_NB8      (1ull << (FV_TV_CSR64_SHIFT + 3))
#define FV_TV_CSR64_MEM      (1ull << (FV_TV_CSR64_SHIFT + 4))
#define FV_TV_ROW_CODES_SHIFT 63
#define FV_TV_ROW_CODES      (1ull << FV_TV_ROW_CODES_SHIFT)

#ifdef __cplusplus
}
#endif
#endif
```

Baseline: 1135 billion.

## Add persistent resident pass kernel with tagged cross-block row exchange

Adds a persistent trellis_pass_u16 kernel that runs every step of a single whole pass in one launch. Blocks exchange each step's row through epoch/step-tagged 64-bit words in global memory and spin-poll until the tags match, which removes the per-step kernel launches and their implicit grid-wide syncs. A timeout/abort word lets the host detect a stall and re-run the decode on the old per-step path. It is enabled by default for the u16 refine kernel when K >= 512 and T <= 4096, and it relies on every tile block being co-resident (ntiles <= num CUs). The backpointer buffers are also zeroed once when first allocated or when K changes.

Result: faster. 1178 billion, median of 6 (+3.8%).

```diff
diff --git a/flash_viterbi_amd/csrc/fv_context.hip b/flash_viterbi_amd/csrc/fv_context.hip
--- a/flash_viterbi_amd/csrc/fv_context.hip
+++ b/flash_viterbi_amd/csrc/fv_context.hip
@@ -60,11 +60,17 @@
     const size_t want_rows = rows_needed * 2 * (size_t)ctx->nrows;
     const size_t want_pack = pack_ints(ctx, T, nscores);
     const bool rows_grow = want_rows > ctx->d_rows.n;
-    w.add(ctx->d_ob, (size_t)T); w.add(ctx->d_ans, (size_t)T); w.add(ctx->d_bp, (size_t)T * ctx->K);
+    const size_t want_bp = (size_t)T * ctx->K;
+    const bool bp_fresh = want_bp > ctx->d_bp.n || ctx->bp_zero_K != ctx->K;
+    w.add(ctx->d_ob, (size_t)T); w.add(ctx->d_ans, (size_t)T); w.add(ctx->d_bp, want_bp);
     w.add(ctx->d_rows, want_rows); w.add(ctx->d_pack, want_pack);
     if (nscores > 1 && w.what.empty()) { w.what = "batch workspace"; w.dominant = "arg rows " + std::to_string(4ull * T * ctx->K); }
     if (int rc = grant(ctx, w, nscores > 1)) return rc;
     if (rows_grow) FV_HIP(hipMemsetAsync(ctx->d_rows.p, 0, want_rows * sizeof(float), ctx->stream));
+    if (bp_fresh) {
+        FV_HIP(hipMemsetAsync(ctx->d_bp.p, 0, ctx->d_bp.bytes(), ctx->stream));
+        ctx->bp_zero_K = ctx->K;
+    }
     FV_HIP(ctx->d_score.ensure((size_t)std::max(4, nscores)));
     FV_HIP(ctx->d_counters.ensure(FV_NCOUNTERS));
     if (ctx->comm || ctx->group) FV_HIP(ctx->d_gather.ensure((size_t)T * ctx->nranks));
@@ -81,19 +87,26 @@
     Wants w;
     const size_t want_rows = passes * 2 * (size_t)ctx->nrows;
     const bool rows_grow = want_rows > ctx->d_rows.n;
-    w.add(ctx->d_rows, want_rows); w.add(ctx->d_snap, (size_t)T); w.add(ctx->d_flat_bp, (size_t)std::max(arg_rows, 1ll) * ctx->K);
+    const size_t want_fbp = (size_t)std::max(arg_rows, 1ll) * ctx->K;
+    const bool fbp_fresh = want_fbp > ctx->d_flat_bp.n || ctx->flat_bp_zero_K != ctx->K;
+    w.add(ctx->d_rows, want_rows); w.add(ctx->d_snap, (size_t)T); w.add(ctx->d_flat_bp, want_fbp);
     w.add(ctx->d_chain, (size_t)std::max(chain_len, 1)); w.add(ctx->d_flat, std::max(passes, (size_t)1));
     w.what = "flat generations workspace"; w.dominant = "private arg rows " + std::to_string(4ull * (unsigned long long)arg_rows * ctx->K);
     if (int rc = grant(ctx, w, true)) return rc;
     if (rows_grow) FV_HIP(hipMemsetAsync(ctx->d_rows.p, 0, want_rows * sizeof(float), ctx->stream));
+    if (fbp_fresh) {
+        FV_HIP(hipMemsetAsync(ctx->d_flat_bp.p, 0, ctx->d_flat_bp.bytes(), ctx->stream));
+        ctx->flat_bp_zero_K = ctx->K;
+    }
     return 0;
 }
 
 __global__ void pack_result(const unsigned long long *counters, const float *score, int nscore, size_t head, const int *ans,
-                            size_t nans, int *out)
+                            size_t nans, int *out, const unsigned long long *status)
 {
     const size_t tid = (size_t)blockIdx.x * blockDim.x + threadIdx.x, nthr = (size_t)gridDim.x * blockDim.x;
     if (tid < 2 * FV_NCOUNTERS) out[tid] = reinterpret_cast<const int *>(counters)[tid];
+    if (status && tid < fvk::PASS_STATUS_WORDS) out[2 * FV_NCOUNTERS + 1 + tid] = (int)status[tid];
     for (size_t i = tid; i < (size_t)nscore; i += nthr) out[2 * FV_NCOUNTERS + i] = __float_as_int(score[i]);
     for (size_t i = tid; i < nans; i += nthr) out[head + i] = ans[i];
 }
@@ -129,6 +142,8 @@
 int begin_decode(fv_ctx *ctx, const int *ob, int T)
 {
     ctx->h_ob.assign(ob, ob + T);
+    ctx->pass_launched = false;
+    ctx->pack_copied = false;
     int *stage = ctx->h_pin + (ctx->h_pin_n - (size_t)T);
     std::memcpy(stage, ob, (size_t)T * sizeof(int));
     FV_HIP(hipMemcpyAsync(ctx->d_ob.p, stage, (size_t)T * sizeof(int), hipMemcpyHostToDevice, ctx->stream));
@@ -236,10 +251,12 @@
     FV_HIP(hipEventRecord(ctx->ev_stop, ctx->stream));
     const size_t nans = gathered ? (size_t)T * ctx->nranks : (size_t)T, head = pack_head(nseq), total = head + nans;
     hipLaunchKernelGGL(pack_result, dim3(64), dim3(256), 0, ctx->stream, ctx->d_counters.p, ctx->d_score.p, nseq, head,
-                       gathered ? ctx->d_gather.p : ctx->d_ans.p, nans, ctx->d_pack.p);
+                       gathered ? ctx->d_gather.p : ctx->d_ans.p, nans, ctx->d_pack.p,
+                       (ctx->pass_launched && nseq == 1 && !beam) ? ctx->d_xch.p + 2 * (size_t)ctx->xch_nrows : nullptr);
     FV_HIP(hipGetLastError());
     FV_HIP(hipMemcpyAsync(ctx->h_pin, ctx->d_pack.p, total * sizeof(int), hipMemcpyDeviceToHost, ctx->stream));
     FV_HIP(hipStreamSynchronize(ctx->stream));
+    ctx->pack_copied = true;
     for (hipGraphExec_t ge : ctx->graphs) (void)hipGraphExecDestroy(ge);
     ctx->graphs.clear();
     unsigned long long counters[FV_NCOUNTERS];
@@ -957,6 +974,31 @@
     return FV_OK;
 }
 
+extern "C" int fv_test_pass_status(const fv_ctx *ctx, int *pass_kernel, int *pass_fallbacks, long long *pass_timeouts)
+{
+    if (!ctx) return FV_ERR_ARG;
+    if (pass_kernel) *pass_kernel = ctx->pass_kernel;
+    if (pass_fallbacks) *pass_fallbacks = ctx->pass_fallbacks;
+    if (pass_timeouts) *pass_timeouts = ctx->pass_timeouts;
+    return FV_OK;
+}
+
+extern "C" int fv_test_pass_abort(fv_ctx *ctx, int s)
+{
+    if (!ctx || s < -1) return FV_ERR_ARG;
+    ctx->pass_abort_step = s;
+    return FV_OK;
+}
+
+extern "C" int fv_test_read_bp(fv_ctx *ctx, int T, int *out)
+{
+    if (!ctx || !out || T < 1 || ctx->K == 0 || (size_t)T * ctx->K > ctx->d_bp.n) return FV_ERR_ARG;
+    FV_HIP(hipSetDevice(ctx->device));
+    FV_HIP(hipStreamSynchronize(ctx->stream));
+    FV_HIP(hipMemcpy(out, ctx->d_bp.p, (size_t)T * ctx->K * sizeof(int), hipMemcpyDeviceToHost));
+    return FV_OK;
+}
+
 extern "C" int fv_set_option(fv_ctx *ctx, int key, long long value)
 {
     if (!ctx) return FV_ERR_ARG;
@@ -978,6 +1020,9 @@
     case FV_OPT_FLAT_GENERATIONS:
         if (value < 0 || value > 2) return FV_ERR_ARG;
         ctx->opt_flat = (int)value; return FV_OK;
+    case FV_OPT_PASS_KERNEL:
+        if (value < 0 || value > 2) return FV_ERR_ARG;
+        ctx->opt_pass_kernel = (int)value; return FV_OK;
     case FV_OPT_ROW_CODES:
         if (value < 0 || value > 4) return FV_ERR_ARG;
         ctx->opt_row_codes = (int)value; return FV_OK;
diff --git a/flash_viterbi_amd/csrc/fv_full.hip b/flash_viterbi_amd/csrc/fv_full.hip
--- a/flash_viterbi_amd/csrc/fv_full.hip
+++ b/flash_viterbi_amd/csrc/fv_full.hip
@@ -378,6 +378,76 @@
 
 struct ProfRange { size_t first, count; };
 
+enum { BATCH_NONE = 0, BATCH_SERIAL = 1, BATCH_FORK = 2 };
+
+constexpr int PASS_AUTO_MIN_K = 512, PASS_AUTO_MAX_T = 4096;
+constexpr int PASS_DEBUG_DECLINES = 1 | 4 | 16 | 32 | 64 | 8192;
+
+bool pass_kernel_eligible(fv_ctx *ctx, const std::vector<fv::Pass> &passes, int kernel, int batch)
+{
+    if (!ctx->pass_allowed || ctx->pass_retry || ctx->opt_pass_kernel == 0 || batch != BATCH_NONE) return false;
+    if (passes.size() != 1 || !passes[0].whole) return false;
+    const int steps = passes[0].R - passes[0].L;
+    if (kernel != FV_KERNEL_U16_REFINE || !ctx->u16_ok || !ctx->full_ok || ctx->csr || ctx->vanilla) return false;
+    if (ctx->nrows > 4096 || steps < 2 || steps > fvk::PASS_MAX_STEPS) return false;
+    if (ctx->group || ctx->comm || ctx->nranks > 1) return false;
+    if (ctx->opt_profile || (ctx->opt_debug & PASS_DEBUG_DECLINES)) return false;
+    if (ctx->row_codes & 1) return false;
+    const int ntiles = (ctx->K + fvk::TILE_W - 1) / fvk::TILE_W;
+    if (ntiles > ctx->num_cus) return false;
+    if (ctx->opt_pass_kernel == 1 && !(ctx->K >= PASS_AUTO_MIN_K && steps + 1 <= PASS_AUTO_MAX_T)) return false;
+    if (ctx->pass_occ_nrows != ctx->nrows) {
+        int per_cu = 0;
+        if (hipOccupancyMaxActiveBlocksPerMultiprocessor(&per_cu, fvk::trellis_pass_u16, 8 * 64, fvk::u16_lds_bytes<1, 8>(ctx->nrows)) != hipSuccess) {
+            (void)hipGetLastError();
+            per_cu = 0;
+        }
+        ctx->pass_occ = per_cu; ctx->pass_occ_nrows = ctx->nrows;
+    }
+    if (ctx->pass_occ < 1) return false;
+    const size_t want = 2 * (size_t)ctx->nrows + fvk::PASS_STATUS_WORDS;
+    if (want > ctx->d_xch.n || ctx->xch_nrows != ctx->nrows) {
+        if (ctx->d_xch.ensure(want) != hipSuccess) { (void)hipGetLastError(); ctx->xch_nrows = 0; ctx->pass_launched = false; return false; }
+        ctx->xch_nrows = ctx->nrows;
+        ctx->pass_epoch = 0;
+    }
+    return true;
+}
+
+int launch_pass_kernel(fv_ctx *ctx, const fv::Pass &p)
+{
+    const int K = ctx->K;
+    fvk::PassArgs a;
+    std::memset(&a, 0, sizeof a);
+    a.st.LA = ctx->LAQ16.p; a.st.window = ctx->windowq; a.st.qscale = ctx->qscale; a.st.vanilla = 0;
+    a.st.LA64 = ctx->LA64.p; a.st.counters = ctx->d_counters.p;
+    a.st.K = K; a.st.reverse = 0; a.st.debug = ctx->opt_debug;
+    a.st.nrows = ctx->nrows;
+    a.st.ntiles = (K + fvk::TILE_W - 1) / fvk::TILE_W;
+    a.st.tiles_per_xcd = (a.st.ntiles + 7) / 8;
+    a.st.nb = 1; a.st.row_lo = 0; a.st.srows = ctx->nrows; a.st.merge = 0; a.st.codes = 0;
+    a.lb32 = ctx->view.lb32;
+    a.ob = ctx->d_ob.p + p.L;
+    a.bp = ctx->d_bp.p + (size_t)p.L * K;
+    a.row[0] = ctx->d_rows.p; a.row[1] = ctx->d_rows.p + ctx->nrows;
+    a.xch[0] = ctx->d_xch.p; a.xch[1] = ctx->d_xch.p + ctx->nrows;
+    a.first = 1; a.last = p.R - p.L;
+    ctx->pass_epoch = fvk::pass_next_epoch(ctx->pass_epoch);
+    if (ctx->pass_epoch == 1) {
+        FV_HIP(hipMemsetAsync(ctx->d_xch.p, 0, ctx->d_xch.bytes(), ctx->stream));
+        ctx->pass_timeouts_seen = 0;
+    }
+    a.epoch = ctx->pass_epoch;
+    unsigned long long *status = ctx->d_xch.p + 2 * (size_t)ctx->nrows;
+    a.abort_word = reinterpret_cast<unsigned int *>(status + fvk::PASS_ABORT_WORD);
+    a.timeouts = status + fvk::PASS_TIMEOUT_COUNTER;
+    a.test_abort_step = ctx->pass_abort_step;
+    const size_t lds = fvk::u16_lds_bytes<1, 8>(ctx->nrows);
+    hipLaunchKernelGGL(fvk::trellis_pass_u16, dim3(a.st.tiles_per_xcd * 8), dim3(8 * 64), lds, ctx->stream, a);
+    FV_HIP(hipGetLastError());
+    return 0;
+}
+
 int prof_event(fv_ctx *ctx, size_t idx, hipEvent_t *out)
 {
     while (ctx->prof_events.size() <= idx) {
@@ -389,7 +459,6 @@
     return 0;
 }
 
-enum { BATCH_NONE = 0, BATCH_SERIAL = 1, BATCH_FORK = 2 };
 int run_generation_full(fv_ctx *ctx, std::vector<fv::Pass> &passes, int kernel, size_t &nprof, int batch = BATCH_NONE)
 {
     const int K = ctx->K;
@@ -454,8 +523,15 @@
     const bool use_graph = (ctx->opt_debug & 64) && !ctx->opt_profile;
     if (use_graph) FV_HIP(hipStreamBeginCapture(ctx->stream, hipStreamCaptureModeThreadLocal));
     if (whole_gen && !use_graph) FV_HIP(hipEventRecord(ctx->ev_s0, ctx->stream));
+    const bool resident = pass_kernel_eligible(ctx, passes, kernel, batch);
+    if (resident) {
+        if (int rc = launch_pass_kernel(ctx, passes[0])) return rc;
+        ctx->pass_launched = true;
+        ctx->stats.step_launches += 1;
+        ctx->stats.task_steps += maxlen;
+    }
     int active = np;
-    for (int s = 1; s <= maxlen; ++s) {
+    for (int s = 1; s <= maxlen && !resident; ++s) {
         while (active > 0 && passes[active - 1].R - passes[active - 1].L < s) --active;
         int full = active;
         if (col_last) while (full > 0 && passes[full - 1].R - passes[full - 1].L == s && !passes[full - 1].whole) --full;
@@ -928,6 +1004,7 @@
 int decode_full_impl(fv_ctx *ctx, const int *ob, int T, int n_split, int mode, int *path_out, float *score_out)
 {
     if (!ctx || !path_out || T < 2 || n_split < 1) return FV_ERR_ARG;
+    const int *const ob_arg = ob;
     int rc = fvi::emission_view(ctx, ob, T);
     if (rc) return rc;
     if (ctx->K == 0) return FV_ERR_STATE;
@@ -967,6 +1044,9 @@
     FV_HIP(hipEventRecord(ctx->ev_start, ctx->stream));
     size_t nprof = 0;
     ctx->fork_active = false;
+    ctx->pass_launched = false;
+    ctx->pass_allowed = true;
+    struct PassScope { fv_ctx *c; ~PassScope() { c->pass_allowed = false; } } pass_scope{ ctx };
     for (size_t g = 0; g < gens.size() && !(flat && g == 1); ++g) {
         ctx->stats.passes += (int)gens[g].size();
         if ((rc = run_generation_full(ctx, gens[g], kernel, nprof))) return rc;
@@ -976,6 +1056,21 @@
     ctx->close_stats((long long)ctx->K * ctx->K, ctx->K);
     const long long whole[2] = { 0, T };
     rc = fvi::finish_decode(ctx, plan, whole, 1, path_out, score_out, nullptr, t0, nprof, false);
+    if (ctx->pass_launched && ctx->pack_copied) {
+        const unsigned int *status = reinterpret_cast<const unsigned int *>(ctx->h_pin) + 2 * FV_NCOUNTERS + 1;
+        const bool aborted = status[fvk::PASS_ABORT_WORD] == ctx->pass_epoch;
+        const long long counted = (long long)status[fvk::PASS_TIMEOUT_COUNTER], timeouts = counted - ctx->pass_timeouts_seen;
+        ctx->pass_timeouts_seen = counted;
+        if (!aborted) ctx->pass_kernel = 1;
+        else if (rc != FV_ERR_DEVICE) {
+            ctx->pass_retry = true;
+            rc = decode_full_impl(ctx, ob_arg, T, n_split, mode, path_out, score_out);
+            ctx->pass_retry = false;
+            ctx->pass_fallbacks = 1;
+            ctx->pass_timeouts = timeouts;
+            return rc;
+        }
+    }
     if (!flat || ctx->stats.flat_first_miss < 1 || rc == FV_ERR_DEVICE) return rc;
     ctx->fork_active = false;
     for (size_t g = (size_t)ctx->stats.flat_first_miss; g < gens.size(); ++g) {
diff --git a/flash_viterbi_amd/csrc/fv_internal.h b/flash_viterbi_amd/csrc/fv_internal.h
--- a/flash_viterbi_amd/csrc/fv_internal.h
+++ b/flash_viterbi_amd/csrc/fv_internal.h
@@ -110,6 +110,19 @@
     int flat_key[4] = { 0, 0, 0, 0 };
     const void *flat_uploaded = nullptr;
     int flat_poison = -1;
+    DevBuf<unsigned long long> d_xch;
+    unsigned int pass_epoch = 0;
+    int xch_nrows = 0;
+    long long pass_timeouts_seen = 0;
+    int pass_kernel = 0, pass_fallbacks = 0;
+    long long pass_timeouts = 0;
+    bool pass_allowed = false;
+    bool pass_retry = false;
+    bool pack_copied = false;
+    bool pass_launched = false;
+    int pass_abort_step = -1;
+    int pass_occ_nrows = -1, pass_occ = 0;
+    int bp_zero_K = 0, flat_bp_zero_K = 0;
     DevBuf<int> d_pack;
     int *h_pin = nullptr;
     size_t h_pin_n = 0;
@@ -141,6 +154,7 @@
     int opt_max_batch = fvk::MAX_BATCH;
     int opt_profile = 0;
     int opt_flat = 1;
+    int opt_pass_kernel = 1;
     int opt_row_codes = 1;
     int vanilla = 0;
     int opt_csr_mem = 0;
@@ -167,6 +181,7 @@
         stats.kernel = kernel; stats.generations = generations;
         stats.table_bytes_per_step = table_bytes_per_step; stats.density = density_reported;
         stats.flat_first_miss = -1;
+        if (!pass_retry) { pass_kernel = 0; pass_fallbacks = 0; pass_timeouts = 0; }
     }
     void close_stats(long long cells_per_task_step, long long cells_per_column_step)
     {
@@ -181,7 +196,7 @@
         f(CSk); f(CSq); f(CS64); f(CSoff); f(CSnwb); f(CRptr); f(CRcol); f(CRlog);
         f(E32); f(E64); f(d_emflags); f(EMap);
         f(d_ob); f(d_ans); f(d_bp); f(d_gather); f(d_rows); f(d_rcodes); f(d_rtmax); f(d_score); f(d_ckpt); f(d_counters); f(d_pack);
-        f(d_snap); f(d_flat_bp); f(d_chain); f(d_flat);
+        f(d_snap); f(d_flat_bp); f(d_chain); f(d_flat); f(d_xch);
         f(d_hval); f(d_scores); f(d_slot_val); f(d_hstate); f(d_slot_state); f(d_flags); f(LA64R); f(LAQ16R); f(d_qaux);
         f(d_tie_list); f(d_cut); f(d_cand); f(d_cand_count); f(d_dupwin); f(d_doubt); f(d_doubt_count); f(d_needfull);
         f(d_seqof); f(d_passL); f(d_tie_count); f(d_csr_acc); f(d_csr_tie);
diff --git a/flash_viterbi_amd/csrc/fv_kernels.hip.inc b/flash_viterbi_amd/csrc/fv_kernels.hip.inc
--- a/flash_viterbi_amd/csrc/fv_kernels.hip.inc
+++ b/flash_viterbi_amd/csrc/fv_kernels.hip.inc
@@ -512,17 +512,38 @@
 
 template <int NB, bool DB, int NWV> constexpr bool u16_takes_codes() { return !(NB == 8 && NWV == 16 && !DB); }
 
+template <int NB, int NWV>
+struct U16Lds {
+    unsigned int *T1c;
+    unsigned int *redZ;
+    float *redR;
+    int *redK;
+    unsigned int *colZ;
+    __device__ __forceinline__ U16Lds(unsigned char *smem, int npairs)
+    {
+        T1c = reinterpret_cast<unsigned int *>(smem);
+        redZ = T1c + (size_t)NB * npairs;
+        redR = reinterpret_cast<float *>(redZ + NB * NWV * TILE_W);
+        redK = reinterpret_cast<int *>(redR + NB * NWV * TILE_W);
+        colZ = reinterpret_cast<unsigned int *>(redK + NB * NWV * TILE_W);
+    }
+};
+
+template <int NB, int NWV>
+__device__ __forceinline__ void u16_stage_floats(const float4 (&v0)[1024 / (NWV * 64)][NB], const float *const (&t1_in)[NB], int K, int nrows,
+                                                 float inv_step, const U16Lds<NB, NWV> &S, float (&Mx)[NB]);
+template <int NB, int U, bool DB, int NWV, class RowIn, class Out>
+__device__ __forceinline__ void u16_step_tail(const StepArgs<NB> &args, const U16Lds<NB, NWV> &S, uint4 (&cur)[U], const uint4 *LAt, int tile,
+                                              bool rev, bool coded, const float (&Mx)[NB], const float (&tmp)[NB], float step, float inv_step, int nj, RowIn rowin, Out out);
+
 template <int NB, int U, bool DB, int NWV>
 __global__ __launch_bounds__(NWV * 64) void trellis_step_u16(const StepArgs<NB> args)
 {
-    constexpr int R = 8, RBR = 32;
+    constexpr int RBR = 32;
     extern __shared__ __align__(16) unsigned char smem[];
     const int nrows = args.nrows, npairs = nrows >> 1;
-    unsigned int *T1c = reinterpret_cast<unsigned int *>(smem);
-    unsigned int *redZ = T1c + (size_t)NB * npairs;
-    float *redR = reinterpret_cast<float *>(redZ + NB * NWV * TILE_W);
-    int *redK = reinterpret_cast<int *>(redR + NB * NWV * TILE_W);
-    unsigned int *colZ = reinterpret_cast<unsigned int *>(redK + NB * NWV * TILE_W);
+    const U16Lds<NB, NWV> S(smem, npairs);
+    unsigned int *T1c = S.T1c;
 
     const int tid = threadIdx.x, lane = tid & 63, w = tid >> 6;
     const int c = lane & (TILE_W - 1), rg = lane >> 4;
@@ -541,7 +562,7 @@
     const float step = -args.qscale, inv_step = 1.0f / step;
     const int nq4 = nrows >> 2;
     constexpr int QPT = 1024 / (NWV * 64);
-    uint4 cur[U], nxt[DB ? U : 1];
+    uint4 cur[U];
     auto request_table = [&]() {
         __builtin_amdgcn_sched_barrier(0);
 #pragma unroll
@@ -600,7 +621,29 @@
             for (int t = 0; t < NB; ++t) v0[h][t] = reinterpret_cast<const float4 *>(args.t[t].t1_in)[q];
         }
         request_table();
-        float *redM = reinterpret_cast<float *>(redZ);
+        const float *rows_in[NB];
+#pragma unroll
+        for (int t = 0; t < NB; ++t) rows_in[t] = args.t[t].t1_in;
+        u16_stage_floats<NB, NWV>(v0, rows_in, K, nrows, inv_step, S, Mx);
+    }
+    __syncthreads();
+    u16_step_tail<NB, U, DB, NWV>(args, S, cur, LAt, tile, rev, coded, Mx, tmp, step, inv_step, nj,
+        [&](int t, int k) { return args.t[t].t1_in[k]; },
+        [&](int t, int col_, bool real, float r, int kb) {
+            if (real) { args.t[t].t1_out[col_] = r; args.t[t].bp_out[col_] = kb; }
+        });
+}
+
+template <int NB, int NWV>
+__device__ __forceinline__ void u16_stage_floats(const float4 (&v0)[1024 / (NWV * 64)][NB], const float *const (&t1_in)[NB], int K, int nrows,
+                                                 float inv_step, const U16Lds<NB, NWV> &S, float (&Mx)[NB])
+{
+    constexpr int QPT = 1024 / (NWV * 64);
+    const int tid = threadIdx.x, lane = tid & 63, w = tid >> 6;
+    const int npairs = nrows >> 1, nq4 = nrows >> 2;
+    unsigned int *T1c = S.T1c;
+    {
+        float *redM = reinterpret_cast<float *>(S.redZ);
         float pm[NB];
         auto fold = [&](int q, const float4 &v, float &m) {
             const int r0 = 4 * q;
@@ -618,7 +661,7 @@
         }
         for (int q = 1024 + tid; q < nq4; q += NWV * 64) {
 #pragma unroll
-            for (int t = 0; t < NB; ++t) fold(q, reinterpret_cast<const float4 *>(args.t[t].t1_in)[q], pm[t]);
+            for (int t = 0; t < NB; ++t) fold(q, reinterpret_cast<const float4 *>(t1_in[t])[q], pm[t]);
         }
 #pragma unroll
         for (int t = 0; t < NB; ++t) {
@@ -648,10 +691,25 @@
             }
         for (int q = 1024 + tid; q < nq4; q += NWV * 64) {
 #pragma unroll
-            for (int t = 0; t < NB; ++t) put(q, t, reinterpret_cast<const float4 *>(args.t[t].t1_in)[q]);
-        }
-    }
-    __syncthreads();
+            for (int t = 0; t < NB; ++t) put(q, t, reinterpret_cast<const float4 *>(t1_in[t])[q]);
+        }
+    }
+}
+
+template <int NB, int U, bool DB, int NWV, class RowIn, class Out>
+__device__ __forceinline__ void u16_step_tail(const StepArgs<NB> &args, const U16Lds<NB, NWV> &S, uint4 (&cur)[U], const uint4 *LAt, int tile,
+                                              bool rev, bool coded, const float (&Mx)[NB], const float (&tmp)[NB], float step, float inv_step, int nj, RowIn rowin, Out out)
+{
+    constexpr int R = 8, RBR = 32;
+    const int nrows = args.nrows, npairs = nrows >> 1, K = args.K;
+    unsigned int *T1c = S.T1c, *redZ = S.redZ, *colZ = S.colZ;
+    float *redR = S.redR;
+    int *redK = S.redK;
+    const int tid = threadIdx.x, lane = tid & 63, w = tid >> 6;
+    const int c = lane & (TILE_W - 1), rg = lane >> 4;
+    const int col = tile * TILE_W + c;
+    auto block_of = [&](int p) { return w + NWV * (rev ? nj - 1 - p : p); };
+    uint4 nxt[DB ? U : 1];
 
     unsigned int m1p[NB], m2p[NB];
     int alo[NB], ahi[NB];
@@ -804,7 +862,7 @@
                 Lc[t] = 0.0; tv[t] = 0.0f;
                 if (kind[t] == 1) {
                     Lc[t] = L64t[(size_t)(a1[t] >> 2) * (TILE_W * 4) + (a1[t] & 3)];
-                    tv[t] = args.t[t].t1_in[a1[t]];
+                    tv[t] = rowin(t, a1[t]);
                 }
             }
         } else {
@@ -816,7 +874,7 @@
                 const int found = locate(t, kind[t] == 1 ? a1[t] : blk0, ce[t]);
                 a1[t] = found;
                 Lc[t] = L64t[(size_t)(found >> 2) * (TILE_W * 4) + (found & 3)];
-                tv[t] = args.t[t].t1_in[found];
+                tv[t] = rowin(t, found);
             }
         }
 #pragma unroll
@@ -839,7 +897,6 @@
                 need &= need - 1;
                 const int cL = L & (TILE_W - 1), rgL = L >> 4;
                 const float tmpL = __shfl(tmp[t], L);
-                const float *t1g = args.t[t].t1_in;
                 float bx = FV_NEG_INF;
                 int bk = INT_MAX;
                 const int nlane_rows = nj * R;
@@ -853,7 +910,7 @@
                         const int k = (w + NWV * (e / R)) * RBR + rgL * R + (e % R);
                         kk[u] = (e < nlane_rows && k < K) ? k : -1;
                         const int ks = kk[u] >= 0 ? k : 0;
-                        tt[u] = t1g[ks];
+                        tt[u] = rowin(t, ks);
                         LL[u] = L64tile[(size_t)(ks >> 2) * (TILE_W * 4) + cL * 4 + (ks & 3)];
                     }
 #pragma unroll
@@ -894,10 +951,7 @@
         if (better(fv.w, fk.w, r, kb)) { r = fv.w; kb = fk.w; }
         wave_best(r, kb);
         const bool any = r > -FLT_MAX;
-        if (lane < TILE_W && col < K) {
-            args.t[w].t1_out[col] = any ? r : -FLT_MAX;
-            args.t[w].bp_out[col] = any ? kb : -1;
-        }
+        if (lane < TILE_W) out(w, col, col < K, any ? r : -FLT_MAX, any ? kb : -1);
         if (args.codes & 2) {
             const float val = (col < K && any) ? r : -FLT_MAX;
             float tmx = val;
@@ -908,6 +962,120 @@
                 if (lane == 0) args.c[w].tmax_out[tile] = tmx;
             }
         }
+    }
+}
+
+struct PassArgs {
+    StepArgs<1> st;
+    const float *lb32;
+    const int *ob;
+    int *bp;
+    float *row[2];
+    unsigned long long *xch[2];
+    int first, last;
+    unsigned int epoch;
+    unsigned int *abort_word;
+    unsigned long long *timeouts;
+    int test_abort_step;
+};
+
+__device__ __forceinline__ unsigned long long xch_load(const unsigned long long *p) { return __hip_atomic_load(p, __ATOMIC_RELAXED, __HIP_MEMORY_SCOPE_AGENT); }
+
+__global__ __launch_bounds__(8 * 64) void trellis_pass_u16(const PassArgs a)
+{
+    constexpr int NWV = 8, U = 16, RBR = 32, QPT = 1024 / (NWV * 64);
+    extern __shared__ __align__(16) unsigned char smem[];
+    __shared__ int s_leave;
+    const StepArgs<1> &args = a.st;
+    const int nrows = args.nrows, npairs = nrows >> 1, K = args.K;
+    const U16Lds<1, NWV> S(smem, npairs);
+    const int tid = threadIdx.x, lane = tid & 63, w = tid >> 6;
+    const int c = lane & (TILE_W - 1), rg = lane >> 4;
+    const int tile = (blockIdx.x & 7) * args.tiles_per_xcd + (blockIdx.x >> 3);
+    if (tile >= args.ntiles) return;
+    const int col = tile * TILE_W + c;
+    const uint4 *LAt = reinterpret_cast<const uint4 *>(reinterpret_cast<const unsigned short *>(args.LA) + (size_t)tile * nrows * TILE_W) + rg * TILE_W + c;
+    const int nq = nrows / RBR, nq4 = nrows >> 2;
+    const int nj = nq > w ? (nq - w + NWV - 1) / NWV : 0;
+    const int live4 = args.ntiles * (TILE_W / 4);
+    const float inv_step = 1.0f / -args.qscale;
+    if (tid == 0) s_leave = 0;
+    uint4 cur[U];
+#pragma unroll
+    for (int u = 0; u < U; ++u)
+        if (u < nj) cur[u] = LAt[(size_t)(w + NWV * u) * (4 * TILE_W)];
+    int sym = a.ob[a.first];
+    __syncthreads();
+    for (int s = a.first; s <= a.last; ++s) {
+        float Mx[1], tmp[1];
+        tmp[0] = a.lb32[(size_t)sym * K + min(col, K - 1)];
+        if (s < a.last) sym = a.ob[s + 1];
+        const float *rin = a.row[(s - 1) & 1];
+        const unsigned long long *xin = a.xch[(s - 1) & 1];
+        const bool plain = s == a.first;
+        float4 v0[QPT][1];
+        bool leave = false;
+        if (plain) {
+#pragma unroll
+            for (int h = 0; h < QPT; ++h) v0[h][0] = reinterpret_cast<const float4 *>(rin)[min(h * (NWV * 64) + tid, nq4 - 1)];
+        } else {
+            const unsigned int want = pass_tag(a.epoch, s - 1);
+            const unsigned long long t0 = __builtin_amdgcn_s_memrealtime();
+            for (unsigned int polls = 1;; ++polls) {
+                bool ok = true;
+#pragma unroll
+                for (int h = 0; h < QPT; ++h) {
+                    const int q = min(h * (NWV * 64) + tid, nq4 - 1);
+                    unsigned int x[4] = { 0u, 0u, 0u, 0u };
+                    if (q < live4) {
+#pragma unroll
+                        for (int e = 0; e < 4; ++e) {
+                            const unsigned long long g = xch_load(xin + 4 * q + e);
+                            x[e] = (unsigned int)g;
+                            ok = ok && (unsigned int)(g >> 32) == want;
+                        }
+                    }
+                    v0[h][0] = make_float4(__uint_as_float(x[0]), __uint_as_float(x[1]), __uint_as_float(x[2]), __uint_as_float(x[3]));
+                }
+                if (__all(ok)) break;
+                if ((polls & 7u) == 0u) {
+                    bool gone = __hip_atomic_load(a.abort_word, __ATOMIC_RELAXED, __HIP_MEMORY_SCOPE_AGENT) == a.epoch;
+                    if (!gone && __builtin_amdgcn_s_memrealtime() - t0 > PASS_WAIT_TICKS) {
+                        if (lane == 0) {
+                            __hip_atomic_store(a.abort_word, a.epoch, __ATOMIC_RELAXED, __HIP_MEMORY_SCOPE_AGENT);
+                            atomicAdd(a.timeouts, 1ull);
+                        }
+                        gone = true;
+                    }
+                    if (__any(gone)) { leave = true; break; }
+                }
+                __builtin_amdgcn_s_sleep(1);
+            }
+        }
+        if (a.test_abort_step == s && blockIdx.x == 0) {
+            if (tid == 0) __hip_atomic_store(a.abort_word, a.epoch, __ATOMIC_RELAXED, __HIP_MEMORY_SCOPE_AGENT);
+            leave = true;
+        }
+        if (leave) s_leave = 1;
+        __syncthreads();
+        if (*static_cast<volatile int *>(&s_leave)) return;
+        const float *rows_in[1] = { rin };
+        u16_stage_floats<1, NWV>(v0, rows_in, K, nrows, inv_step, S, Mx);
+        __syncthreads();
+        float *rout = a.row[s & 1];
+        int *bps = a.bp + (size_t)s * K;
+        unsigned long long *xout = a.xch[s & 1];
+        const unsigned long long tag = (unsigned long long)pass_tag(a.epoch, s) << 32;
+        const bool publish = s < a.last;
+        u16_step_tail<1, U, false, NWV>(args, S, cur, LAt, tile, false, false, Mx, tmp, -args.qscale, inv_step, nj,
+            [&](int, int k) {
+                return plain ? rin[k]
+                             : __uint_as_float(__hip_atomic_load(reinterpret_cast<const unsigned int *>(xin) + 2 * k, __ATOMIC_RELAXED, __HIP_MEMORY_SCOPE_AGENT));
+            },
+            [&](int, int col_, bool real, float r, int kb) {
+                if (real) { rout[col_] = r; bps[col_] = kb; }
+                if (publish) __hip_atomic_store(xout + col_, tag | __float_as_uint(real ? r : 0.0f), __ATOMIC_RELAXED, __HIP_MEMORY_SCOPE_AGENT);
+            });
     }
 }
 
diff --git a/flash_viterbi_amd/csrc/fv_layout.h b/flash_viterbi_amd/csrc/fv_layout.h
--- a/flash_viterbi_amd/csrc/fv_layout.h
+++ b/flash_viterbi_amd/csrc/fv_layout.h
@@ -27,6 +27,14 @@
 struct FlatGens { int ngen; int begin[FLAT_MAX_GENS + 1]; };
 constexpr int FLAT_COUNTER = 15;
 
+constexpr int PASS_ABORT_WORD = 0;
+constexpr int PASS_TIMEOUT_COUNTER = 1;
+constexpr int PASS_STATUS_WORDS = 2;
+constexpr unsigned long long PASS_WAIT_TICKS = 20000000ull;
+constexpr int PASS_MAX_STEPS = 65535;
+__host__ __device__ inline unsigned int pass_tag(unsigned int epoch, int s) { return (epoch << 16) | ((unsigned int)s & 0xffffu); }
+inline unsigned int pass_next_epoch(unsigned int epoch) { return epoch >= 65535u ? 1u : epoch + 1u; }
+
 template <int NB>
 static inline size_t step_lds_bytes(int nrows)
 {
diff --git a/flash_viterbi_amd/decoder.py b/flash_viterbi_amd/decoder.py
--- a/flash_viterbi_amd/decoder.py
+++ b/flash_viterbi_amd/decoder.py
@@ -14,6 +14,7 @@
 OPT_KERNEL, OPT_MAX_BATCH, OPT_PROFILE, OPT_SEL_MARGIN, OPT_DEBUG = 1, 2, 3, 4, 100
 OPT_FLAT_GENERATIONS = 5
 OPT_ROW_CODES = 6
+OPT_PASS_KERNEL = 8
 OPT_SPARSE_BEAM = 7
 FLAT_OFF, FLAT_AUTO, FLAT_ON = 0, 1, 2
 DEBUG_TIMING_ONLY = (1 << 0) | (1 << 4) | (1 << 5) | (1 << 11) | (1 << 12)
@@ -72,7 +73,7 @@
            "fv_create_multi", "fv_device_count", "fv_decode_full_batch", "fv_plan_passes_batch", "fv_decode_beam_batch",
            "fv_set_model_sparse", "fv_set_emissions", "fv_clear_emissions", "fv_plan_flat", "fv_set_emission_map"]
 TEST_EXPORTS = ["fv_test_forward", "fv_test_beam_step", "fv_test_beam_select", "fv_test_device_alloc", "fv_test_device_free",
-                "fv_test_stage_emissions_ms", "fv_test_flat_poison"]
+                "fv_test_stage_emissions_ms", "fv_test_flat_poison", "fv_test_pass_abort", "fv_test_read_bp", "fv_test_pass_status"]
 TIE_TAG = 1 << 30
 TS_BITS = {"topb_select<4,listed>": 1 << 0, "topb_select<4,derived>": 1 << 1, "topb_select<16,listed>": 1 << 2,
            "topb_select<16,derived>": 1 << 3, "topb_select<64,listed>": 1 << 4, "topb_select<64,derived>": 1 << 5,
@@ -145,6 +146,9 @@
     L.fv_merge_paths.argtypes = [ci, ci, ci, vp, vp]
     L.fv_plan_flat.argtypes = [ci, ci, ci, ci, ctypes.POINTER(FlatInfo), ci]
     L.fv_test_flat_poison.argtypes = [vp, ci]
+    L.fv_test_pass_abort.argtypes = [vp, ci]
+    L.fv_test_read_bp.argtypes = [vp, ci, vp]
+    L.fv_test_pass_status.argtypes = [vp, ctypes.POINTER(ci), ctypes.POINTER(ci), ctypes.POINTER(cll)]
     L.fv_test_forward.argtypes = [vp, vp, ci, ctypes.POINTER(ForwardPass), ci, vp, vp, ctypes.POINTER(ctypes.c_ulonglong)]
     cf = ctypes.c_float
     L.fv_test_beam_step.argtypes = [vp, ci, ctypes.POINTER(BeamSet), ci, vp, ci, cf, cf, ci, vp, vp, vp, ctypes.POINTER(ci),
@@ -406,6 +410,19 @@
 
     def test_flat_poison(self, t):
         self._check(self._L.fv_test_flat_poison(self._h, int(t)))
+
+    def test_pass_abort(self, s):
+        self._check(self._L.fv_test_pass_abort(self._h, int(s)))
+
+    def test_pass_status(self):
+        k, f, t = ctypes.c_int(0), ctypes.c_int(0), ctypes.c_longlong(0)
+        self._check(self._L.fv_test_pass_status(self._h, ctypes.byref(k), ctypes.byref(f), ctypes.byref(t)))
+        return {"pass_kernel": k.value, "pass_fallbacks": f.value, "pass_timeouts": t.value}
+
+    def test_read_bp(self, T, K):
+        out = np.empty((int(T), int(K)), dtype=np.int32)
+        self._check(self._L.fv_test_read_bp(self._h, int(T), _p(out)))
+        return out
 
     def test_device_alloc(self, host_array):
         a = np.ascontiguousarray(host_array)
diff --git a/include/flashvit.h b/include/flashvit.h
--- a/include/flashvit.h
+++ b/include/flashvit.h
@@ -37,6 +37,7 @@
     FV_OPT_DEBUG = 100,
 };
 #define FV_DEBUG_TIMING_ONLY ((1 << 0) | (1 << 4) | (1 << 5) | (1 << 11) | (1 << 12))
+#define FV_OPT_PASS_KERNEL 8
 enum {
     FV_KERNEL_AUTO = 0,
     FV_KERNEL_F64_STREAM = 1,
diff --git a/include/flashvit_testing.h b/include/flashvit_testing.h
--- a/include/flashvit_testing.h
+++ b/include/flashvit_testing.h
@@ -13,6 +13,10 @@
                     float *rows_out, int *bp_out, unsigned long long *variants_out);
 
 int fv_test_flat_poison(fv_ctx *ctx, int t);
+
+int fv_test_pass_abort(fv_ctx *ctx, int s);
+int fv_test_pass_status(const fv_ctx *ctx, int *pass_kernel, int *pass_fallbacks, long long *pass_timeouts);
+int fv_test_read_bp(fv_ctx *ctx, int T, int *out);
 
 int fv_test_device_alloc(fv_ctx *ctx, size_t bytes, const void *host_src, void **out);
 int fv_test_device_free(fv_ctx *ctx, void *p);
```
